# bupt-ai-cz/HIAST

Measured on AMD Instinct MI355X. Metric: self-training images/sec (fwd+bwd+pseudo-label) at 1024x512, higher is better.
Workload: dtype fp16

## Files before the change

### hiast_amd/_lib.py

```python
import ctypes
import os

import torch

_HERE = os.path.dirname(os.path.abspath(__file__))
LIB_PATH = os.environ.get("HIAST_LIB") or os.path.join(_HERE, "csrc", "libhiast_hip.so")

c_int, c_i64, c_f32, c_sz, c_vp = (ctypes.c_int, ctypes.c_int64, ctypes.c_float, ctypes.c_size_t,
                                   ctypes.c_void_p)

SIGNATURES = {
    "hiast_version": (c_int, []),
    "hiast_error_string": (ctypes.c_char_p, [c_int]),
    "hiast_upsample_bilinear_ac_fwd": (c_int, [c_vp, c_vp] + [c_int] * 6 + [c_vp]),
    "hiast_upsample_bilinear_ac_bwd": (c_int, [c_vp, c_vp] + [c_int] * 6 + [c_vp]),
    "hiast_plabel_pass1_workspace_bytes": (c_sz, [c_int]),
    "hiast_plabel_pass1": (c_int, [c_vp] + [c_int] * 6 + [c_vp, c_vp, c_vp, c_vp, c_sz, c_vp]),
    "hiast_plabel_pass2": (c_int, [c_vp, c_vp, c_vp, c_int, c_int, c_i64, c_vp, c_vp, c_vp, c_vp]),
    "hiast_plabel_strided_hist_workspace_bytes": (c_sz, [c_i64, c_int]),
    "hiast_plabel_strided_hist": (c_int, [c_vp, c_vp, c_i64, c_int, c_int, c_vp, c_vp, c_vp, c_vp, c_sz, c_vp]),
    "hiast_tta_fused": (c_int, [c_vp] * 6 + [c_int] * 5 + [c_vp, c_vp, c_vp]),
    "hiast_dinput_fwd": (c_int, [c_vp, c_int, c_vp] + [c_int] * 6 + [c_vp]),
    "hiast_dinput_bwd": (c_int, [c_vp, c_int, c_vp, c_vp, c_vp] + [c_int] * 6 + [c_vp]),
    "hiast_st_loss_workspace_bytes": (c_sz, [c_int] * 6),
    "hiast_st_loss_fwd": (c_int, [c_vp, c_vp, c_vp] + [c_int] * 8 + [c_vp, c_vp, c_sz, c_vp]),
    "hiast_st_loss_bwd": (c_int, [c_vp, c_vp, c_vp] + [c_int] * 8 + [c_vp, c_vp, c_vp, c_vp, c_sz, c_vp]),
    "hiast_st_loss_cst_fwd": (c_int, [c_vp, c_vp, c_vp] + [c_int] * 9 + [c_vp, c_vp, c_sz, c_vp]),
    "hiast_st_loss_cst_bwd": (c_int, [c_vp, c_vp, c_vp] + [c_int] * 9 + [c_vp, c_vp, c_vp, c_vp, c_sz, c_vp]),
    "hiast_aspp_wpack_bytes": (c_sz, [c_int, c_int]),
    "hiast_aspp_workspace_bytes": (c_sz, [c_int] * 5),
    "hiast_aspp_pack_weights": (c_int, [c_vp] * 8 + [c_int, c_int, c_vp, c_vp]),
    "hiast_aspp_fwd": (c_int, [c_vp, c_vp, c_vp] + [c_int] * 5 + [c_vp, c_vp, c_sz, c_vp]),
    "hiast_aspp_bwd_data": (c_int, [c_vp, c_vp, c_vp] + [c_int] * 5 + [c_vp, c_vp]),
    "hiast_aspp_bwd_weight": (c_int, [c_vp] * 7 + [c_int] * 5 + [c_vp, c_vp, c_sz, c_vp]),
    "hiast_aspp2_np": (c_int, [c_int]),
    "hiast_aspp2_workspace_bytes": (c_sz, [c_int] * 6),
    "hiast_aspp2_pack_weights": (c_int, [c_vp] * 8 + [c_int, c_int, c_vp, c_vp, c_vp, c_vp]),
    "hiast_aspp2_fwd": (c_int, [c_vp, c_int, c_vp, c_vp, c_vp] + [c_int] * 5 + [c_vp, c_vp, c_sz, c_vp]),
    "hiast_aspp2_bwd": (c_int, [c_vp] * 9 + [c_int] * 5 + [c_vp, c_int, c_vp, c_sz, c_vp]),
    "hiast_bn_workspace_bytes": (c_sz, [c_int, c_int]),
    "hiast_bn_stats": (c_int, [c_vp, c_int, c_int, c_i64, c_int, c_vp, c_vp]),
    "hiast_bn_act_apply": (c_int, [c_vp] * 8 + [c_int, ctypes.c_double, c_f32, c_f32, c_int, c_vp, c_vp,
                                   c_int, c_int, c_i64, c_int, c_vp]),
    "hiast_bn_act_bwd_stats": (c_int, [c_vp] * 5 + [c_int, c_int, c_int, c_i64, c_int, c_vp, c_vp]),
    "hiast_bn_act_bwd_apply": (c_int, [c_vp] * 7 + [c_int, ctypes.c_double, c_int, c_vp, c_vp, c_vp, c_vp,
                                       c_int, c_int, c_i64, c_int, c_vp]),
    "hiast_bn_act_nhwc_infer": (c_int, [c_vp] * 6 + [c_f32, c_int, c_i64, c_int, c_int, c_vp]),
    "hiast_igemm_bn_act": (c_int, [c_vp] * 6 + [c_f32, c_vp, c_int, c_vp] + [c_int] * 10 + [c_vp, c_int, c_vp, c_int, c_vp]),
    "hiast_igemm_set_cosched": (c_int, [c_int]),
    "hiast_igemm_set_half": (c_int, [c_int]),
    "hiast_device_cus": (c_int, []),
    "hiast_set_reserve_cus": (c_int, [c_int]),
    "hiast_get_reserve_cus": (c_int, []),
    "hiast_stream_create_reserved": (c_int, [c_vp, c_int]),
    "hiast_stream_destroy": (c_int, [c_vp]),
    "hiast_igemm_stats_rows": (c_int, [c_i64, c_int, c_int, c_int, c_int]),
    "hiast_igemm_dgrad_bn_stats": (c_int, [c_vp, c_vp, c_vp] + [c_int] * 7 + [c_vp] * 6 + [c_int, c_int, c_vp]),
    "hiast_xconv_dgrad_gated_bn_stats_rows": (c_int, [c_i64, c_int, c_int]),
    "hiast_xconv_dgrad_gated_bn_stats": (c_int, [c_vp] * 10 + [c_i64, c_int, c_int, c_int, c_vp]),
    "hiast_igemm_dgrad_s2": (c_int, [c_vp, c_vp, c_vp] + [c_int] * 6 + [c_vp]),
    "hiast_igemm_dgrad_bn_stats_rows": (c_int, [c_i64, c_int, c_int, c_int]),
    "hiast_bn_nhwc_stats_from_partial": (c_int, [c_vp, c_int, c_int, c_vp, c_vp]),
    "hiast_conv_wgrad_workspace_bytes": (c_sz, [c_int] * 6),
    "hiast_conv_wgrad_nhwc": (c_int, [c_vp, c_vp, c_vp] + [c_int] * 9 + [c_vp, c_sz, c_vp]),
    "hiast_conv_wgrad_group_workspace_bytes": (c_sz, [c_vp, c_int]),
    "hiast_conv_wgrad_group_nhwc": (c_int, [c_vp, c_int, c_int, c_vp, c_sz, c_vp]),
    "hiast_conv_wgrad_small_workspace_bytes": (c_sz, [c_int] * 6),
    "hiast_conv_wgrad_small_nhwc": (c_int, [c_vp, c_vp, c_vp] + [c_int] * 9 + [c_vp, c_sz, c_vp]),
    "hiast_pack_conv_weight": (c_int, [c_vp, c_int, c_int, c_int, c_int, c_int, c_vp, c_vp, c_vp]),
    "hiast_bn_nhwc_workspace_bytes": (c_sz, [c_int]),
    "hiast_bn_nhwc_stats": (c_int, [c_vp, c_i64, c_int, c_vp, c_vp, c_sz, c_int, c_vp]),
    "hiast_bn_nhwc_apply": (c_int, [c_vp] * 8 + [ctypes.c_double, c_f32, c_f32, c_int, c_vp, c_vp, c_i64, c_int, c_vp,
                                    c_int, c_vp]),
    "hiast_bn_nhwc_apply_partial": (c_int, [c_vp] * 8 + [c_int, ctypes.c_double, c_f32, c_f32, c_int, c_vp, c_vp, c_i64,
                                            c_int, c_vp, c_int, c_vp]),
    "hiast_bn_nhwc_bwd_stats": (c_int, [c_vp] * 7 + [c_int, c_i64, c_int, c_vp, c_vp, c_sz, c_int, c_vp]),
    "hiast_bn_nhwc_bwd_apply": (c_int, [c_vp] * 8 + [ctypes.c_double, c_int, c_vp, c_vp, c_vp, c_vp, c_i64, c_int, c_int,
                                        c_vp]),
    "hiast_pack_conv_weight_multi": (c_int, [c_vp, c_vp, c_vp, c_int, c_int, c_vp]),
    "hiast_split_planes": (c_int, [c_vp, c_vp, c_i64, c_int, c_int, c_vp]),
    "hiast_stem_tail": (c_int, [c_vp, c_int, c_vp, c_vp, c_vp, c_vp, c_f32, c_vp, c_int, c_int, c_int, c_int, c_int, c_vp]),
    "hiast_stem_eval": (c_int, [c_vp] * 6 + [c_f32, c_vp, c_int, c_int, c_int, c_int, c_vp]),
    "hiast_stem_train_blocks": (c_int, [c_int] * 3),
    "hiast_stem_train_fwd": (c_int, [c_vp, c_vp, c_vp, c_vp, c_int, c_int, c_int, c_int, c_vp]),
    "hiast_stem_wgrad_workspace_bytes": (c_sz, [c_int] * 3),
    "hiast_stem_wgrad": (c_int, [c_vp, c_vp, c_vp, c_int, c_int, c_int, c_int, c_vp, c_sz, c_vp]),
    "hiast_ema_update": (c_int, [c_vp, c_vp, c_vp, c_int, c_f32, c_f32, c_vp]),
    "hiast_normalize_u8": (c_int, [c_vp, c_vp, c_int, c_i64, c_vp, c_vp, c_vp]),
    "hiast_maxpool3x3s2_nhwc_fwd": (c_int, [c_vp, c_vp, c_vp, c_int, c_int, c_int, c_int, c_int, c_vp]),
    "hiast_maxpool3x3s2_nhwc_bwd": (c_int, [c_vp, c_vp, c_vp, c_int, c_int, c_int, c_int, c_int, c_vp]),
    "hiast_multi_copy": (c_int, [c_vp, c_int, c_vp]),
    "hiast_aug_geometry_u8": (c_int, [c_vp] * 6 + [c_int] * 4 + [c_vp]),
    "hiast_aug_hist_u8": (c_int, [c_vp] * 5 + [c_int, c_i64, c_vp]),
    "hiast_aug_colour_u8": (c_int, [c_vp] * 5 + [c_int, c_i64, c_vp]),
    "hiast_aug2_table_u8": (c_int, [c_vp] * 6 + [c_int, c_i64, c_vp]),
    "hiast_aug2_colour_u8": (c_int, [c_vp] * 6 + [c_int, c_i64, c_vp]),
    "hiast_aug2_blur_u8": (c_int, [c_vp] * 5 + [c_int] * 3 + [c_vp]),
    "hiast_adam_prepare": (c_int, [c_vp, c_vp, c_vp, c_vp]),
    "hiast_adam_step": (c_int, [c_vp, c_vp, c_vp, c_int, ctypes.c_double, ctypes.c_double, c_f32, c_f32, c_vp, c_vp]),
    "hiast_sgd_step": (c_int, [c_vp, c_vp, c_vp, c_int, c_f32, c_f32, c_vp, c_vp]),
    "hiast_adamw_step": (c_int, [c_vp, c_vp, c_vp, c_int, ctypes.c_double, ctypes.c_double, c_f32, c_vp, c_vp]),
    "hiast_disc_conv_workspace_bytes": (c_sz, [c_int] * 5),
    "hiast_disc_conv_fwd": (c_int, [c_vp] * 4 + [c_int] * 6 + [c_vp]),
    "hiast_disc_conv_dgrad": (c_int, [c_vp] * 4 + [c_int] * 6 + [c_vp, c_sz, c_vp]),
    "hiast_disc_conv_wgrad": (c_int, [c_vp] * 5 + [c_int] * 6 + [c_vp, c_sz, c_vp]),
    "hiast_disc_conv16_fwd": (c_int, [c_vp] * 4 + [c_int] * 7 + [c_vp]),
    "hiast_disc_conv16_dgrad": (c_int, [c_vp] * 4 + [c_int] * 7 + [c_vp, c_sz, c_vp]),
    "hiast_disc_conv16_wgrad": (c_int, [c_vp] * 5 + [c_int] * 7 + [c_vp, c_sz, c_vp]),
    "hiast_confusion_hist": (c_int, [c_vp, c_vp, c_i64, c_int, c_vp, c_vp, c_vp, c_vp]),
}



class WgradJob(ctypes.Structure):
    _fields_ = [("dy", c_vp), ("x", c_vp), ("dw", c_vp)] + [(n, ctypes.c_int32) for n in
                                                             ("B", "H", "W", "Cin", "Cout", "taps", "stride", "dil")]


NBINS = 15361
PROB_FX_SHIFT = 30
IGNORE = 255

_lib = None


class HiastLibraryError(RuntimeError):
    pass


def load():
    global _lib
    if _lib is not None:
        return _lib
    if not os.path.exists(LIB_PATH):
        raise HiastLibraryError(
            "libhiast_hip.so is not built (%s). Build it with `python -c 'import __graft_entry__ as g; "
            "g.build()'` or `make -C hiast_amd/csrc`; there is no fallback path." % LIB_PATH)
    lib = ctypes.CDLL(LIB_PATH)
    for name, (res, args) in SIGNATURES.items():
        try:
            fn = getattr(lib, name)
        except AttributeError as e:
            raise HiastLibraryError("libhiast_hip.so does not export %s" % name) from e
        fn.restype = res
        fn.argtypes = args
    if lib.hiast_version() != 6:
        raise HiastLibraryError("libhiast_hip.so ABI version mismatch")
    _lib = lib
    return lib


def kernel_sources_sha16():
    import glob
    import hashlib
    h = hashlib.sha256()
    files = sorted(glob.glob(os.path.join(_HERE, "csrc", "*.hip")) + glob.glob(os.path.join(_HERE, "csrc", "*.h")))
    files.append(os.path.join(os.path.dirname(_HERE), "include", "hiast_hip.h"))
    for f in files:
        h.update(os.path.basename(f).encode())
        h.update(open(f, "rb").read())
    return h.hexdigest()[:16]


def check(code, what):
    if code != 0:
        msg = load().hiast_error_string(int(code)).decode()
        raise HiastLibraryError("%s failed: %s (code %d)" % (what, msg, code))
```

### hiast_amd/csrc/bn_nhwc.hip

```cpp
#include <hip/hip_bf16.h>

#include "common.h"

namespace hiast {

constexpr int BNH_MAXBLK = 512;
#ifndef BNH_ROWS_PER_BLOCK_PASS
#define BNH_ROWS_PER_BLOCK_PASS 16
#endif
#ifndef BNH_APPLY_MAXBLK
#define BNH_APPLY_MAXBLK 65535
#endif
#ifndef BNH_CONTIG
#define BNH_CONTIG 0
#endif
#if BNH_CONTIG
#define BNH_ROW_WALK(CHUNK)                                                                                              \
    const long long step = (CHUNK);                                                                                      \
    const long long per_blk = ((M + gridDim.x - 1) / gridDim.x + (CHUNK) - 1) / (CHUNK) * (CHUNK);                       \
    const long long lim = (long long)(blockIdx.x + 1) * per_blk < M ? (long long)(blockIdx.x + 1) * per_blk : M;         \
    long long r0 = (long long)blockIdx.x * per_blk + rsub;
#else
#define BNH_ROW_WALK(CHUNK)                                                                                              \
    const long long step = (long long)gridDim.x * (CHUNK);                                                               \
    const long long lim = M;                                                                                             \
    long long r0 = (long long)blockIdx.x * (CHUNK) + rsub;
#endif
#ifndef BNH_UNR_PART
#define BNH_UNR_PART 8
#endif
#ifndef BNH_UNR_APPLY
#define BNH_UNR_APPLY 4
#endif
#ifndef BNH_UNR_BWD
#define BNH_UNR_BWD 4
#endif

template <bool F16>
__device__ __forceinline__ void bnh_unpack8(const uint4 r, float (&v)[8])
{
    const unsigned w[4] = {r.x, r.y, r.z, r.w};
#pragma unroll
    for (int i = 0; i < 4; ++i) {
        v[2 * i] = H16<F16>::lo(w[i]);
        v[2 * i + 1] = H16<F16>::hi(w[i]);
    }
}

#ifndef BNH_NT_LOADS
#define BNH_NT_LOADS 7
#endif
template <int WHICH>
__device__ __forceinline__ uint4 bnh_ld16(const unsigned short* p)
{
    if ((BNH_NT_LOADS >> WHICH) & 1) {
        const h_u32x4 v = __builtin_nontemporal_load(reinterpret_cast<const h_u32x4*>(p));
        return make_uint4(v.x, v.y, v.z, v.w);
    }
    return *reinterpret_cast<const uint4*>(p);
}

template <bool F16>
__device__ __forceinline__ void bnh_load8(const unsigned short* p, float (&v)[8])
{
    bnh_unpack8<F16>(*reinterpret_cast<const uint4*>(p), v);
}

__device__ __forceinline__ void bnh_param8(const float* p, const float* some_valid, int c0, float dflt, float (&v)[8])
{
    const float* q = (p ? p : some_valid) + c0;
    const float4 a = *reinterpret_cast<const float4*>(q), b = *reinterpret_cast<const float4*>(q + 4);
    const bool has = p != nullptr;
    v[0] = has ? a.x : dflt; v[1] = has ? a.y : dflt; v[2] = has ? a.z : dflt; v[3] = has ? a.w : dflt;
    v[4] = has ? b.x : dflt; v[5] = has ? b.y : dflt; v[6] = has ? b.z : dflt; v[7] = has ? b.w : dflt;
}

template <bool F16>
__device__ __forceinline__ void bnh_store8(unsigned short* p, const float (&v)[8], bool nt = false)
{
    unsigned w[4];
#pragma unroll
    for (int i = 0; i < 4; ++i) w[i] = H16<F16>::pack(v[2 * i], v[2 * i + 1]);
    h_store16(p, w[0], w[1], w[2], w[3], nt);
}

template <bool BWD, int GATE, bool F16 = false>
__global__ __launch_bounds__(256) void bnh_partial_kernel(const unsigned short* __restrict__ a,
                                                          const unsigned short* __restrict__ y,
                                                          const unsigned short* __restrict__ x,
                                                          const float* __restrict__ gamma,
                                                          const float* __restrict__ beta,
                                                          const float* __restrict__ save_mean,
                                                          const float* __restrict__ save_invstd, long long M, int C,
                                                          float* __restrict__ partial)
{
    __shared__ float s_red[256 * 16];
    const int G = C >> 3, RPP = 256 / G;
    const int cg = threadIdx.x % G, rsub = threadIdx.x / G;
    float s1[8], s2[8], mean[8], invstd[8], gsc[8], gsh[8];
#pragma unroll
    for (int k = 0; k < 8; ++k) { s1[k] = 0.f; s2[k] = 0.f; mean[k] = 0.f; invstd[k] = 0.f; gsc[k] = 0.f; gsh[k] = 0.f; }
    constexpr int UNR = BNH_UNR_PART;
    const long long stride = RPP;
    BNH_ROW_WALK(RPP * UNR)

    uint4 ra[UNR], ry[UNR], rx[UNR];
    unsigned rbits[UNR];
    auto load_rows = [&](long long rb) {
#pragma unroll
        for (int u = 0; u < UNR; ++u) {
            const long long r = rb + u * stride;
            const long long rc = r < lim ? r : (rb < lim ? rb : 0);
            const size_t off = (size_t)rc * C + cg * 8;
            ra[u] = bnh_ld16<0>(a + off);
            if (BWD) {
                if (GATE == 1) ry[u] = bnh_ld16<0>(y + off);
                rbits[u] = GATE == 3 ? reinterpret_cast<const unsigned char*>(y)[(size_t)rc * G + cg] : 0u;
                rx[u] = bnh_ld16<0>(x + off);
            }
        }
    };
    load_rows(r0);
    if (BWD) {
        float gm[8], bt[8];
        bnh_param8(save_mean, save_mean, cg * 8, 0.f, mean);
        bnh_param8(save_invstd, save_mean, cg * 8, 0.f, invstd);
        if (GATE == 2) {
            bnh_param8(gamma, save_mean, cg * 8, 1.0f, gm);
            bnh_param8(beta, save_mean, cg * 8, 0.0f, bt);
#pragma unroll
            for (int k = 0; k < 8; ++k) {
                gsc[k] = gm[k] * invstd[k];
                gsh[k] = fmaf(-mean[k], gsc[k], bt[k]);
            }
        }
    }
    while (r0 < lim) {
#pragma unroll
        for (int u = 0; u < UNR; ++u) {
            if (r0 + u * stride >= lim) break;
            float v[8];
            bnh_unpack8<F16>(ra[u], v);
            if (!BWD) {
#pragma unroll
                for (int k = 0; k < 8; ++k) { s1[k] += v[k]; s2[k] = fmaf(v[k], v[k], s2[k]); }
            } else {
                float yy[8], xx[8];
                if (GATE == 1) bnh_unpack8<F16>(ry[u], yy);
                const unsigned bits = rbits[u];
                bnh_unpack8<F16>(rx[u], xx);
#pragma unroll
                for (int k = 0; k < 8; ++k) {
                    const bool open = GATE == 0 || (GATE == 1 ? yy[k] > 0.f
                                                    : (GATE == 3 ? ((bits >> k) & 1u) != 0u : fmaf(xx[k], gsc[k], gsh[k]) > 0.f));
                    const float g = open ? v[k] : 0.f;
                    s1[k] += g;
                    s2[k] = fmaf(g, (xx[k] - mean[k]) * invstd[k], s2[k]);
                }
            }
        }
        r0 += step;
        if (r0 < lim) load_rows(r0);
    }
#pragma unroll
    for (int k = 0; k < 8; ++k) {
        s_red[threadIdx.x * 16 + k] = s1[k];
        s_red[threadIdx.x * 16 + 8 + k] = s2[k];
    }
    __syncthreads();
    if (rsub == 0) {
        float* dst = partial + ((size_t)blockIdx.x * C + cg * 8) * 2;
#pragma unroll
        for (int k = 0; k < 8; ++k) {
            float t1 = 0.f, t2 = 0.f;
            for (int j = 0; j < RPP; ++j) {
                t1 += s_red[(j * G + cg) * 16 + k];
                t2 += s_red[(j * G + cg) * 16 + 8 + k];
            }
            dst[2 * k] = t1;
            dst[2 * k + 1] = t2;
        }
    }
}

__global__ __launch_bounds__(256) void bnh_finalize_kernel(const float* __restrict__ partial, int nblk, int C,
                                                           double* __restrict__ sums)
{
    __shared__ double s[16][17];
    const int e = threadIdx.x & 15, j = threadIdx.x >> 4;
    const int i = blockIdx.x * 16 + e;
    double acc = 0.0;
    {
        int b = j;
        for (; b + 16 * 15 < nblk; b += 16 * 16) {
            float v[16];
#pragma unroll
            for (int u = 0; u < 16; ++u) v[u] = partial[(size_t)(b + 16 * u) * C * 2 + i];
#pragma unroll
            for (int u = 0; u < 16; ++u) acc += (double)v[u];
        }
        for (; b < nblk; b += 16) acc += (double)partial[(size_t)b * C * 2 + i];
    }
    s[j][e] = acc;
    __syncthreads();
    if (j == 0) {
        double t = 0.0;
#pragma unroll
        for (int q = 0; q < 16; ++q) t += s[q][e];
        sums[i] = t;
    }
}

__global__ __launch_bounds__(256) void bnh_prep_fwd_kernel(const double* __restrict__ sums, double count, float momentum,
                                                           float eps, float* __restrict__ run_mean,
                                                           float* __restrict__ run_var, float* __restrict__ save_mean,
                                                           float* __restrict__ save_invstd, int C)
{
    const int c = blockIdx.x * 256 + threadIdx.x;
    if (c >= C) return;
    const double m = sums[2 * c] / count;
    double var = sums[2 * c + 1] / count - m * m;
    var = var < 0.0 ? 0.0 : var;
    const float mean = (float)m;
    const float invstd = (float)(1.0 / sqrt(var + (double)eps));
    save_mean[c] = mean;
    save_invstd[c] = invstd;
    if (run_mean) {
        const double unb = count > 1.0 ? var * count / (count - 1.0) : var;
        run_mean[c] = (1.0f - momentum) * run_mean[c] + momentum * mean;
        run_var[c] = (1.0f - momentum) * run_var[c] + momentum * (float)unb;
    }
}

__global__ __launch_bounds__(256) void bnh_finalize_prep_kernel(const float* __restrict__ partial, int nblk, int C,
                                                                double count, float momentum, float eps,
                                                                float* __restrict__ run_mean, float* __restrict__ run_var,
                                                                float* __restrict__ save_mean,
                                                                float* __restrict__ save_invstd)
{
    __shared__ double s[64][5];
    const int e = threadIdx.x & 3, j = threadIdx.x >> 2;
    const int i = blockIdx.x * 4 + e;
    const int c = blockIdx.x * 2 + (int)threadIdx.x;
    float rm = 0.f, rv = 0.f;
    if (threadIdx.x < 2 && run_mean) { rm = run_mean[c]; rv = run_var[c]; }
    double acc = 0.0;
    {
        int b = j;
        for (; b + 64 * 3 < nblk; b += 64 * 4) {
            float v[4];
#pragma unroll
            for (int u = 0; u < 4; ++u) v[u] = partial[(size_t)(b + 64 * u) * C * 2 + i];
#pragma unroll
            for (int u = 0; u < 4; ++u) acc += (double)v[u];
        }
        for (; b < nblk; b += 64) acc += (double)partial[(size_t)b * C * 2 + i];
    }
    s[j][e] = acc;
    __syncthreads();
    if (threadIdx.x < 2) {
        double s1 = 0.0, s2 = 0.0;
#pragma unroll 8
        for (int q = 0; q < 64; ++q) { s1 += s[q][2 * threadIdx.x]; s2 += s[q][2 * threadIdx.x + 1]; }
        const double m = s1 / count;
        double var = s2 / count - m * m;
        var = var < 0.0 ? 0.0 : var;
        const float mean = (float)m;
        save_mean[c] = mean;
        save_invstd[c] = (float)(1.0 / sqrt(var + (double)eps));
        if (run_mean) {
            const double unb = count > 1.0 ? var * count / (count - 1.0) : var;
            run_mean[c] = (1.0f - momentum) * rm + momentum * mean;
            run_var[c] = (1.0f - momentum) * rv + momentum * (float)unb;
        }
    }
}

template <bool RES, bool RELU, bool F16 = false>
__global__ __launch_bounds__(256) void bnh_apply_kernel(const unsigned short* __restrict__ x,
                                                        const unsigned short* __restrict__ res,
                                                        unsigned short* __restrict__ y, const float* __restrict__ gamma,
                                                        const float* __restrict__ beta,
                                                        const float* __restrict__ save_mean,
                                                        const float* __restrict__ save_invstd, long long M, int C,
                                                        unsigned char* __restrict__ mask)
{
    const int G = C >> 3, RPP = 256 / G;
    const bool nt_out = (long long)M * C * 2 >= H_NT_MIN_BYTES;
    const int cg = threadIdx.x % G, rsub = threadIdx.x / G;
    constexpr int UNR = BNH_UNR_APPLY;
    const long long stride = RPP;
    BNH_ROW_WALK(RPP * UNR)

    uint4 rx[UNR], rres[UNR];
    auto load_rows = [&](long long rb) {
#pragma unroll
        for (int u = 0; u < UNR; ++u) {
            const long long r = rb + u * stride;
            const size_t off = (size_t)(r < lim ? r : (rb < lim ? rb : 0)) * C + cg * 8;
            rx[u] = bnh_ld16<1>(x + off);
            if (RES) rres[u] = bnh_ld16<1>(res + off);
        }
    };
    load_rows(r0);
    float scale[8], shift[8];
    {
        float gm[8], bt[8], mn[8], is[8];
        bnh_param8(gamma, save_mean, cg * 8, 1.0f, gm);
        bnh_param8(beta, save_mean, cg * 8, 0.0f, bt);
        bnh_param8(save_mean, save_mean, cg * 8, 0.f, mn);
        bnh_param8(save_invstd, save_mean, cg * 8, 0.f, is);
#pragma unroll
        for (int k = 0; k < 8; ++k) {
            scale[k] = gm[k] * is[k];
            shift[k] = fmaf(-mn[k], scale[k], bt[k]);
        }
    }
    while (r0 < lim) {
#pragma unroll
        for (int u = 0; u < UNR; ++u) {
            const long long r = r0 + u * stride;
            if (r >= lim) break;
            const size_t off = (size_t)r * C + cg * 8;
            float v[8], rr[8];
            bnh_unpack8<F16>(rx[u], v);
            if (RES) bnh_unpack8<F16>(rres[u], rr);
            unsigned bits = 0;
#pragma unroll
            for (int k = 0; k < 8; ++k) {
                float o = fmaf(v[k], scale[k], shift[k]);
                if (RES) o += rr[k];
                if (RELU) o = o > 0.f ? o : 0.f;
                bits |= (o > 0.f ? 1u : 0u) << k;
                v[k] = o;
            }
            bnh_store8<F16>(y + off, v, nt_out);
            if (mask) mask[(size_t)r * G + cg] = (unsigned char)bits;
        }
        r0 += step;
        if (r0 < lim) load_rows(r0);
    }
}

template <int GATE, bool DRES, bool F16 = false>
__global__ __launch_bounds__(256) void bnh_bwd_apply_kernel(
    const unsigned short* __restrict__ dy, const unsigned short* __restrict__ y, const unsigned short* __restrict__ x,
    const float* __restrict__ gamma, const float* __restrict__ beta, const float* __restrict__ save_mean,
    const float* __restrict__ save_invstd,
    const double* __restrict__ sums, double inv_count, unsigned short* __restrict__ dx,
    unsigned short* __restrict__ dres, float* __restrict__ dgamma, float* __restrict__ dbeta, long long M, int C)
{
    const int G = C >> 3, RPP = 256 / G;
    const bool nt_out = (long long)M * C * 2 >= H_NT_MIN_BYTES;
    const int cg = threadIdx.x % G, rsub = threadIdx.x / G;
    constexpr int UNR = BNH_UNR_BWD;
    const long long stride = RPP;
    BNH_ROW_WALK(RPP * UNR)

    uint4 rg[UNR], ry[UNR], rx[UNR];
    unsigned rbits[UNR];
    auto load_rows = [&](long long rb) {
#pragma unroll
        for (int u = 0; u < UNR; ++u) {
            const long long r = rb + u * stride;
            const long long rc = r < lim ? r : (rb < lim ? rb : 0);
            const size_t off = (size_t)rc * C + cg * 8;
            rg[u] = bnh_ld16<2>(dy + off);
            if (GATE == 1) ry[u] = bnh_ld16<2>(y + off);
            rbits[u] = GATE == 3 ? reinterpret_cast<const unsigned char*>(y)[(size_t)rc * G + cg] : 0u;
            rx[u] = bnh_ld16<2>(x + off);
        }
    };
    load_rows(r0);
    float mean[8], invstd[8], k0[8], mg[8], mgx[8], gsh[8];
    {
        float gm[8], bt[8];
        bnh_param8(save_mean, save_mean, cg * 8, 0.f, mean);
        bnh_param8(save_invstd, save_mean, cg * 8, 0.f, invstd);
        bnh_param8(gamma, save_mean, cg * 8, 1.0f, gm);
        bnh_param8(beta, save_mean, cg * 8, 0.0f, bt);
        const double2* sp = reinterpret_cast<const double2*>(sums) + cg * 8;
#pragma unroll
        for (int k = 0; k < 8; ++k) {
            const double2 ss = sp[k];
            if (blockIdx.x == 0 && rsub == 0) {
                if (dbeta) dbeta[cg * 8 + k] = (float)ss.x;
                if (dgamma) dgamma[cg * 8 + k] = (float)ss.y;
            }
            k0[k] = gm[k] * invstd[k];
            gsh[k] = GATE == 2 ? fmaf(-mean[k], k0[k], bt[k]) : 0.f;
            mg[k] = (float)(ss.x * inv_count);
            mgx[k] = (float)(ss.y * inv_count);
        }
    }
    while (r0 < lim) {
#pragma unroll
        for (int u = 0; u < UNR; ++u) {
            const long long r = r0 + u * stride;
            if (r >= lim) break;
            const size_t off = (size_t)r * C + cg * 8;
            float g[8], yy[8], xx[8];
            bnh_unpack8<F16>(rg[u], g);
            if (GATE == 1) bnh_unpack8<F16>(ry[u], yy);
            const unsigned bits = rbits[u];
            bnh_unpack8<F16>(rx[u], xx);
#pragma unroll
            for (int k = 0; k < 8; ++k) {
                const bool open = GATE == 0 || (GATE == 1 ? yy[k] > 0.f
                                                : (GATE == 3 ? ((bits >> k) & 1u) != 0u : fmaf(xx[k], k0[k], gsh[k]) > 0.f));
                const float gg = open ? g[k] : 0.f;
                g[k] = gg;
                xx[k] = k0[k] * (gg - mg[k] - (xx[k] - mean[k]) * invstd[k] * mgx[k]);
            }
            bnh_store8<F16>(dx + off, xx, nt_out);
            if (DRES) bnh_store8<F16>(dres + off, g, nt_out);
        }
        r0 += step;
        if (r0 < lim) load_rows(r0);
    }
}

static int bnh_nblk(long long M, int C)
{
    const int rpp = 256 / (C / 8);
    long long nb = (M + (long long)rpp * 16 - 1) / ((long long)rpp * 16);
    nb = nb < 1 ? 1 : (nb > BNH_MAXBLK ? BNH_MAXBLK : nb);
    return (int)nb;
}

}

static bool bnh_c_ok(int C) { return C >= 8 && C <= 2048 && (C & (C - 1)) == 0; }

static int bnh_check(const void* x, long long M, int C)
{
    if (!x) return HIAST_E_ARG;
    if (M <= 0) return HIAST_E_ARG;
    if (!bnh_c_ok(C) || (((uintptr_t)x) & 15)) return HIAST_E_RANGE;
    return 0;
}

extern "C" size_t hiast_bn_nhwc_workspace_bytes(int C) { return (size_t)hiast::BNH_MAXBLK * C * 2 * sizeof(float); }

#define BNH_FMT_CHECK()                                                             \
    if (fmt != HIAST_FMT_BF16 && fmt != HIAST_FMT_FP16) return HIAST_E_RANGE;          \
    const bool f16 = fmt == HIAST_FMT_FP16

extern "C" int hiast_bn_nhwc_stats(const void* x, int64_t M, int C, double* sums, void* workspace,
                                   size_t workspace_bytes, int fmt, hiast_stream_t stream)
{
    BNH_FMT_CHECK();
    int e = bnh_check(x, M, C);
    if (e) return e;
    if (!sums || !workspace) return HIAST_E_ARG;
    const int nblk = hiast::bnh_nblk(M, C);
    if (workspace_bytes < (size_t)nblk * C * 2 * sizeof(float)) return HIAST_E_WS;
    hipStream_t st = (hipStream_t)stream;
    if (f16)
        hipLaunchKernelGGL((hiast::bnh_partial_kernel<false, 0, true>), dim3(nblk), dim3(256), 0, st, (const unsigned short*)x,
                           nullptr, nullptr, nullptr, nullptr, nullptr, nullptr, (long long)M, C, (float*)workspace);
    else
        hipLaunchKernelGGL((hiast::bnh_partial_kernel<false, 0>), dim3(nblk), dim3(256), 0, st, (const unsigned short*)x,
                           nullptr, nullptr, nullptr, nullptr, nullptr, nullptr, (long long)M, C, (float*)workspace);
    HIAST_CHECK_LAUNCH();
    hipLaunchKernelGGL(hiast::bnh_finalize_kernel, dim3(C * 2 / 16), dim3(256), 0, st, (const float*)workspace, nblk, C,
                       sums);
    HIAST_CHECK_LAUNCH();
    return 0;
}

extern "C" int hiast_bn_nhwc_stats_from_partial(const float* partial, int nblk, int C, double* sums,
                                                hiast_stream_t stream)
{
    if (!partial || !sums) return HIAST_E_ARG;
    if (nblk <= 0) return HIAST_E_ARG;
    if (!bnh_c_ok(C)) return HIAST_E_RANGE;
    hipLaunchKernelGGL(hiast::bnh_finalize_kernel, dim3(C * 2 / 16), dim3(256), 0, (hipStream_t)stream, partial, nblk, C,
                       sums);
    HIAST_CHECK_LAUNCH();
    return 0;
}

extern "C" int hiast_bn_nhwc_apply(const void* x, const void* res, void* y, const float* gamma, const float* beta,
                                   float* running_mean, float* running_var, const double* sums, double count,
                                   float momentum, float eps, int relu, float* save_mean, float* save_invstd,
                                   int64_t M, int C, void* mask, int fmt, hiast_stream_t stream)
{
    BNH_FMT_CHECK();
    int e = bnh_check(x, M, C);
    if (e) return e;
    if (!y || !sums || !save_mean || !save_invstd || count <= 0) return HIAST_E_ARG;
    if ((((uintptr_t)y) | ((uintptr_t)res)) & 15) return HIAST_E_RANGE;
    const int rpp = 256 / (C / 8);
    long long nb = (M + (long long)rpp * BNH_ROWS_PER_BLOCK_PASS - 1) / ((long long)rpp * BNH_ROWS_PER_BLOCK_PASS);
    nb = nb < 1 ? 1 : (nb > BNH_APPLY_MAXBLK ? BNH_APPLY_MAXBLK : nb);
    hipStream_t st = (hipStream_t)stream;
    hipLaunchKernelGGL(hiast::bnh_prep_fwd_kernel, dim3((C + 255) / 256), dim3(256), 0, st, sums, count, momentum, eps,
                       running_mean, running_var, save_mean, save_invstd, C);
    HIAST_CHECK_LAUNCH();
#define L1(RES, RELU, F)                                                                                           \
    hipLaunchKernelGGL((hiast::bnh_apply_kernel<RES, RELU, F>), dim3((unsigned)nb), dim3(256), 0, st,              \
                       (const unsigned short*)x, (const unsigned short*)res, (unsigned short*)y, gamma, beta,      \
                       save_mean, save_invstd, (long long)M, C, (unsigned char*)mask)
#define L(RES, RELU) do { if (f16) L1(RES, RELU, true); else L1(RES, RELU, false); } while (0)
    if (res) { if (relu) L(true, true); else L(true, false); }
    else { if (relu) L(false, true); else L(false, false); }
#undef L
#undef L1
    HIAST_CHECK_LAUNCH();
    return 0;
}

extern "C" int hiast_bn_nhwc_apply_partial(const void* x, const void* res, void* y, const float* gamma, const float* beta,
                                           float* running_mean, float* running_var, const float* partial, int nblk,
                                           double count, float momentum, float eps, int relu, float* save_mean,
                                           float* save_invstd, int64_t M, int C, void* mask, int fmt,
                                           hiast_stream_t stream)
{
    BNH_FMT_CHECK();
    int e = bnh_check(x, M, C);
    if (e) return e;
    if (!y || !partial || !save_mean || !save_invstd || count <= 0 || nblk <= 0) return HIAST_E_ARG;
    if ((((uintptr_t)y) | ((uintptr_t)res)) & 15) return HIAST_E_RANGE;
    const int rpp = 256 / (C / 8);
    long long nb = (M + (long long)rpp * BNH_ROWS_PER_BLOCK_PASS - 1) / ((long long)rpp * BNH_ROWS_PER_BLOCK_PASS);
    nb = nb < 1 ? 1 : (nb > BNH_APPLY_MAXBLK ? BNH_APPLY_MAXBLK : nb);
    hipStream_t st = (hipStream_t)stream;
    hipLaunchKernelGGL(hiast::bnh_finalize_prep_kernel, dim3(C / 2), dim3(256), 0, st, partial, nblk, C, count,
                       momentum, eps, running_mean, running_var, save_mean, save_invstd);
    HIAST_CHECK_LAUNCH();
#define L1(RES, RELU, F)                                                                                           \
    hipLaunchKernelGGL((hiast::bnh_apply_kernel<RES, RELU, F>), dim3((unsigned)nb), dim3(256), 0, st,              \
                       (const unsigned short*)x, (const unsigned short*)res, (unsigned short*)y, gamma, beta,      \
                       save_mean, save_invstd, (long long)M, C, (unsigned char*)mask)
#define L(RES, RELU) do { if (f16) L1(RES, RELU, true); else L1(RES, RELU, false); } while (0)
    if (res) { if (relu) L(true, true); else L(true, false); }
    else { if (relu) L(false, true); else L(false, false); }
#undef L
#undef L1
    HIAST_CHECK_LAUNCH();
    return 0;
}

extern "C" int hiast_bn_nhwc_bwd_stats(const void* dy, const void* y, const void* x, const float* gamma,
                                       const float* beta, const float* save_mean, const float* save_invstd, int relu,
                                       int64_t M, int C, double* sums, void* workspace, size_t workspace_bytes, int fmt,
                                       hiast_stream_t stream)
{
    BNH_FMT_CHECK();
    int e = bnh_check(x, M, C);
    if (e) return e;
    if (!dy || !save_mean || !save_invstd || !sums || !workspace || ((relu == 1 || relu == 3) && !y)) return HIAST_E_ARG;
    if (relu < 0 || relu > 3 || (((uintptr_t)dy) & 15) || (relu == 1 && (((uintptr_t)y) & 15))) return HIAST_E_RANGE;
    const int nblk = hiast::bnh_nblk(M, C);
    if (workspace_bytes < (size_t)nblk * C * 2 * sizeof(float)) return HIAST_E_WS;
    hipStream_t st = (hipStream_t)stream;
#define L1(G, F)                                                                                                    \
    hipLaunchKernelGGL((hiast::bnh_partial_kernel<true, G, F>), dim3(nblk), dim3(256), 0, st, (const unsigned short*)dy, \
                       (const unsigned short*)y, (const unsigned short*)x, gamma, beta, save_mean, save_invstd,      \
                       (long long)M, C, (float*)workspace)
#define L(G) do { if (f16) L1(G, true); else L1(G, false); } while (0)
    if (relu == 1) L(1); else if (relu == 2) L(2); else if (relu == 3) L(3); else L(0);
#undef L
#undef L1
    HIAST_CHECK_LAUNCH();
    hipLaunchKernelGGL(hiast::bnh_finalize_kernel, dim3(C * 2 / 16), dim3(256), 0, st, (const float*)workspace, nblk, C,
                       sums);
    HIAST_CHECK_LAUNCH();
    return 0;
}

extern "C" int hiast_bn_nhwc_bwd_apply(const void* dy, const void* y, const void* x, const float* gamma,
                                       const float* beta, const float* save_mean, const float* save_invstd,
                                       const double* sums,
                                       double count, int relu, void* dx, void* dres, float* dgamma, float* dbeta,
                                       int64_t M, int C, int fmt, hiast_stream_t stream)
{
    BNH_FMT_CHECK();
    int e = bnh_check(x, M, C);
    if (e) return e;
    if (!dy || !save_mean || !save_invstd || !sums || !dx || ((relu == 1 || relu == 3) && !y) || count <= 0)
        return HIAST_E_ARG;
    if (relu < 0 || relu > 3 || ((((uintptr_t)dy) | ((uintptr_t)dx) | ((uintptr_t)dres)) & 15) ||
        (relu == 1 && (((uintptr_t)y) & 15)))
        return HIAST_E_RANGE;
    const int rpp = 256 / (C / 8);
    long long nb = (M + (long long)rpp * BNH_ROWS_PER_BLOCK_PASS - 1) / ((long long)rpp * BNH_ROWS_PER_BLOCK_PASS);
    nb = nb < 1 ? 1 : (nb > BNH_APPLY_MAXBLK ? BNH_APPLY_MAXBLK : nb);
    hipStream_t st = (hipStream_t)stream;
#define L1(G, DRES, F)                                                                                             \
    hipLaunchKernelGGL((hiast::bnh_bwd_apply_kernel<G, DRES, F>), dim3((unsigned)nb), dim3(256), 0, st,             \
                       (const unsigned short*)dy, (const unsigned short*)y, (const unsigned short*)x, gamma, beta,  \
                       save_mean, save_invstd, sums, 1.0 / count, (unsigned short*)dx, (unsigned short*)dres, dgamma, \
                       dbeta, (long long)M, C)
#define L(G, DRES) do { if (f16) L1(G, DRES, true); else L1(G, DRES, false); } while (0)
    if (relu == 1) { if (dres) L(1, true); else L(1, false); }
    else if (relu == 3) { if (dres) L(3, true); else L(3, false); }
    else if (relu == 2) { if (dres) L(2, true); else L(2, false); }
    else { if (dres) L(0, true); else L(0, false); }
#undef L
#undef L1
    HIAST_CHECK_LAUNCH();
    return 0;
}
```

### hiast_amd/csrc/common.h

```cpp
#pragma once
#include <hip/hip_runtime.h>
#include <hip/hip_bf16.h>
#include <hip/hip_fp16.h>
#include <stdint.h>

#include <type_traits>

#include "../../include/hiast_hip.h"

#define HIAST_WAVE 64

#define HIAST_CHECK_LAUNCH()                         \
    do {                                             \
        hipError_t e__ = hipGetLastError();          \
        if (e__ != hipSuccess) return (int)e__;      \
    } while (0)

static inline int hiast_fmt_planes(int fmt) { return fmt == HIAST_FMT_SPLIT_BF16 ? 2 : 1; }
static inline int hiast_fmt_ok(int fmt) { return fmt == HIAST_FMT_BF16 || fmt == HIAST_FMT_SPLIT_BF16 || fmt == HIAST_FMT_FP16; }

int hiast_cu_count();
int hiast_grid_cus();

namespace hiast {

template <class F>
static inline bool for_class_count(int C, F&& f)
{
    switch (C) {
        case 19: f(std::integral_constant<int, 19>{}); return true;
        case 16: f(std::integral_constant<int, 16>{}); return true;
        case 9:  f(std::integral_constant<int, 9>{});  return true;
        case 2:  f(std::integral_constant<int, 2>{});  return true;
        default: return false;
    }
}

typedef __attribute__((ext_vector_type(8))) __bf16 h_bf16x8;
typedef __attribute__((ext_vector_type(8))) _Float16 h_f16x8;
typedef __attribute__((ext_vector_type(4))) float h_f32x4;
typedef __attribute__((ext_vector_type(16))) float h_f32x16;

typedef __attribute__((address_space(3))) void* h_lds_ptr;
__device__ __forceinline__ void h_dma16(__amdgpu_buffer_rsrc_t rs, unsigned char* lds, int voff, int soff)
{
    __builtin_amdgcn_raw_ptr_buffer_load_lds(rs, (h_lds_ptr)lds, 16, voff, soff, 0, 0);
}
__device__ __forceinline__ int h_lds_off(int row, int chunk) { return row * 128 + ((chunk ^ ((row >> 1) & 7)) << 4); }

#ifndef HIAST_NT
#define HIAST_NT 1
#endif
__device__ __forceinline__ void h_store_f32(float* p, float v)
{
#if HIAST_NT
    __builtin_nontemporal_store(v, p);
#else
    *p = v;
#endif
}
typedef unsigned int h_u32x4 __attribute__((ext_vector_type(4)));
__device__ __forceinline__ void h_store16(void* p, unsigned a, unsigned b, unsigned c, unsigned d)
{
#if HIAST_NT
    __builtin_nontemporal_store((h_u32x4){a, b, c, d}, reinterpret_cast<h_u32x4*>(p));
#else
    *reinterpret_cast<uint4*>(p) = make_uint4(a, b, c, d);
#endif
}
__device__ __forceinline__ void h_store16(void* p, unsigned a, unsigned b, unsigned c, unsigned d, bool nt)
{
#if HIAST_NT
    if (nt) {
        __builtin_nontemporal_store((h_u32x4){a, b, c, d}, reinterpret_cast<h_u32x4*>(p));
        return;
    }
#endif
    *reinterpret_cast<uint4*>(p) = make_uint4(a, b, c, d);
}
#ifndef H_NT_MIN_MIB
#define H_NT_MIN_MIB 64
#endif
constexpr long long H_NT_MIN_BYTES = (long long)H_NT_MIN_MIB << 20;
#ifndef HIAST_NT_OUT
#define HIAST_NT_OUT 0
#endif
__device__ __forceinline__ void h_store16_out(void* p, unsigned a, unsigned b, unsigned c, unsigned d)
{
    h_store16(p, a, b, c, d, HIAST_NT_OUT != 0);
}
__device__ __forceinline__ void h_store_f32_out(float* p, float v)
{
#if HIAST_NT_OUT
    __builtin_nontemporal_store(v, p);
#else
    *p = v;
#endif
}
#ifndef HIAST_NT_RES
#define HIAST_NT_RES 0
#endif
__device__ __forceinline__ uint4 h_load16_once(const void* p)
{
#if HIAST_NT_RES
    const h_u32x4 v = __builtin_nontemporal_load(reinterpret_cast<const h_u32x4*>(p));
    return make_uint4(v.x, v.y, v.z, v.w);
#else
    return *reinterpret_cast<const uint4*>(p);
#endif
}

template <bool F16>
struct H16;

template <>
struct H16<false> {
    static __device__ __forceinline__ float lo(unsigned w) { return __uint_as_float(w << 16); }
    static __device__ __forceinline__ float hi(unsigned w) { return __uint_as_float(w & 0xFFFF0000u); }
    static __device__ __forceinline__ float dec(unsigned short h) { return __uint_as_float((unsigned)h << 16); }
    static __device__ __forceinline__ unsigned short enc(float v) { return __bfloat16_as_ushort(__float2bfloat16(v)); }
    static __device__ __forceinline__ unsigned pack(float a, float b) { return (unsigned)enc(a) | ((unsigned)enc(b) << 16); }
    template <class V>
    static __device__ __forceinline__ h_f32x4 mfma16(const V& a, const V& b, h_f32x4 c)
    {
        return __builtin_amdgcn_mfma_f32_16x16x32_bf16(__builtin_bit_cast(h_bf16x8, a), __builtin_bit_cast(h_bf16x8, b), c, 0, 0, 0);
    }
    template <class V>
    static __device__ __forceinline__ h_f32x16 mfma32(const V& a, const V& b, h_f32x16 c)
    {
        return __builtin_amdgcn_mfma_f32_32x32x16_bf16(__builtin_bit_cast(h_bf16x8, a), __builtin_bit_cast(h_bf16x8, b), c, 0, 0, 0);
    }
};

template <>
struct H16<true> {
    static __device__ __forceinline__ float dec(unsigned short h) { return __half2float(__ushort_as_half(h)); }
    static __device__ __forceinline__ float lo(unsigned w) { return dec((unsigned short)(w & 0xFFFFu)); }
    static __device__ __forceinline__ float hi(unsigned w) { return dec((unsigned short)(w >> 16)); }
    static __device__ __forceinline__ unsigned short enc(float v) { return __half_as_ushort(__float2half_rn(v)); }
    static __device__ __forceinline__ unsigned pack(float a, float b) { return (unsigned)enc(a) | ((unsigned)enc(b) << 16); }
    template <class V>
    static __device__ __forceinline__ h_f32x4 mfma16(const V& a, const V& b, h_f32x4 c)
    {
        return __builtin_amdgcn_mfma_f32_16x16x32_f16(__builtin_bit_cast(h_f16x8, a), __builtin_bit_cast(h_f16x8, b), c, 0, 0, 0);
    }
    template <class V>
    static __device__ __forceinline__ h_f32x16 mfma32(const V& a, const V& b, h_f32x16 c)
    {
        return __builtin_amdgcn_mfma_f32_32x32x16_f16(__builtin_bit_cast(h_f16x8, a), __builtin_bit_cast(h_f16x8, b), c, 0, 0, 0);
    }
};

__device__ __forceinline__ float a_expf(float x)
{
    const float LOG2E = 1.44269502162933349609375f;
    const float LN2_HI = 0.693145751953125f;
    const float LN2_LO = 1.428606765330187045037746429443359375e-06f;
    float n = rintf(x * LOG2E);
    float r = fmaf(-n, LN2_HI, x);
    r = fmaf(-n, LN2_LO, r);
    float p = 1.984127011382952332496643066406250e-04f;
    p = fmaf(p, r, 1.388888922519981861114501953125e-03f);
    p = fmaf(p, r, 8.33333376795053482055664062500e-03f);
    p = fmaf(p, r, 4.16666679084300994873046875000e-02f);
    p = fmaf(p, r, 1.66666671633720397949218750000e-01f);
    p = fmaf(p, r, 0.5f);
    p = fmaf(p, r, 1.0f);
    p = fmaf(p, r, 1.0f);
    float s = __int_as_float(((int)n + 127) << 23);
    float v = p * s;
    return x < -87.0f ? 0.0f : v;
}

struct Src {
    int i0, i1;
    float l0, l1;
};

__device__ __forceinline__ Src src_of(float scale, int dst, int in)
{
    Src s;
    float f = scale * (float)dst;
    int a = (int)f;
    a = a > in - 1 ? in - 1 : a;
    s.i0 = a;
    s.i1 = a + (a < in - 1 ? 1 : 0);
    s.l1 = f - (float)a;
    s.l0 = 1.0f - s.l1;
    return s;
}

__device__ __forceinline__ float lerp_h(float a, float b, float wl0, float wl1)
{
    return fmaf(wl1, b, wl0 * a);
}

__device__ __forceinline__ float lerp_v(float top, float bot, float hl0, float hl1)
{
    return fmaf(hl1, bot, hl0 * top);
}

__device__ __forceinline__ int band_start(float scale, int j, int in, int out)
{
    if (j <= 0) return 0;
    if (j > in - 1) return out;
    if (scale <= 0.0f) return out;
    int Y = (int)((float)j / scale);
    Y = Y < 0 ? 0 : (Y > out ? out : Y);
    while (Y > 0 && (int)(scale * (float)(Y - 1)) >= j) --Y;
    while (Y < out && (int)(scale * (float)Y) < j) ++Y;
    return Y;
}

__device__ __forceinline__ int lane_id() { return (int)(threadIdx.x & 63); }

__device__ __forceinline__ unsigned long long wave_sum_u64(unsigned long long v)
{
#pragma unroll
    for (int o = 32; o > 0; o >>= 1) v += __shfl_xor(v, o, 64);
    return v;
}

__device__ __forceinline__ double wave_sum_f64(double v)
{
#pragma unroll
    for (int o = 32; o > 0; o >>= 1) v += __shfl_xor(v, o, 64);
    return v;
}

}
```

### hiast_amd/functional.py

```python
import os

import torch

from . import kernels as K
from . import switches as SW

ASPP_DILATIONS = (6, 12, 18, 24)
H16 = (torch.bfloat16, torch.float16)


class _AsppFn(torch.autograd.Function):

    @staticmethod
    @torch.amp.custom_fwd(device_type="cuda", cast_inputs=torch.float32)
    def forward(ctx, x, w0, w1, w2, w3, b0, b1, b2, b3, dil):
        x = x.contiguous()
        ws = [w.contiguous() for w in (w0, w1, w2, w3)]
        bs = [b.contiguous() for b in (b0, b1, b2, b3)]
        wpack = K.aspp_pack_weights(ws, bs)
        Cout = ws[0].shape[0]
        y = K.aspp_fwd(x, wpack, Cout, dil)
        ctx.save_for_backward(x, wpack)
        ctx.dil = dil
        ctx.cin = x.shape[1]
        return y

    @staticmethod
    @torch.amp.custom_bwd(device_type="cuda")
    def backward(ctx, gy):
        x, wpack = ctx.saved_tensors
        gy = gy.contiguous().float()
        gx = None
        if ctx.needs_input_grad[0]:
            gx = K.aspp_bwd_data(gy, wpack, ctx.cin, ctx.dil)
        gws, gb = [None] * 4, None
        if any(ctx.needs_input_grad[1:9]):
            gws, gb = K.aspp_bwd_weight(x, gy, ctx.dil)
        return (gx, gws[0], gws[1], gws[2], gws[3], gb, gb, gb, gb, None)


def aspp(x, weights, biases, dil=ASPP_DILATIONS):
    return _AsppFn.apply(x, *weights, *biases, tuple(dil))


class _Aspp2Fn(torch.autograd.Function):

    @staticmethod
    @torch.amp.custom_fwd(device_type="cuda")
    def forward(ctx, x, w0, w1, w2, w3, b0, b1, b2, b3, dil, need_bwd):
        ws = [w.detach().float().contiguous() for w in (w0, w1, w2, w3)]
        bs = [b.detach().float().contiguous() for b in (b0, b1, b2, b3)]
        if need_bwd and x.dtype not in H16:
            raise TypeError("the channels-last ASPP backward is the 16-bit one; fp32 training uses hiast_amd.functional.aspp")
        wt, wd, bias = K.aspp2_pack_weights(ws, bs, need_dgrad=need_bwd and ctx.needs_input_grad[0])
        y = K.aspp2_fwd(x, wt, bias, dil)
        ctx.save_for_backward(x, wd)
        ctx.dil = dil
        return y

    @staticmethod
    @torch.amp.custom_bwd(device_type="cuda")
    def backward(ctx, gy):
        x, wd = ctx.saved_tensors
        gy = gy.contiguous().float()
        want_dx = ctx.needs_input_grad[0]
        want_dw = any(ctx.needs_input_grad[1:9])
        gx, gws, gb = K.aspp2_bwd(x, gy, wd, ctx.dil, want_dx, want_dw)
        if gws is None:
            gws = [None] * 4
        return (gx, gws[0], gws[1], gws[2], gws[3], gb, gb, gb, gb, None, None)


def aspp_nhwc(x, weights, biases, dil=ASPP_DILATIONS):
    need_bwd = torch.is_grad_enabled() and any(t.requires_grad for t in (x, *weights, *biases))
    return _Aspp2Fn.apply(x, *weights, *biases, tuple(dil), need_bwd)


class _UpsampleFn(torch.autograd.Function):

    @staticmethod
    @torch.amp.custom_fwd(device_type="cuda", cast_inputs=torch.float32)
    def forward(ctx, x, H, W):
        ctx.hw = x.shape[2:]
        return K.upsample_bilinear_ac_fwd(x.contiguous(), H, W)

    @staticmethod
    @torch.amp.custom_bwd(device_type="cuda")
    def backward(ctx, g):
        return K.upsample_bilinear_ac_bwd(g.contiguous().float(), ctx.hw[0], ctx.hw[1]), None, None


def upsample_bilinear_ac(x, size):
    return _UpsampleFn.apply(x, int(size[0]), int(size[1]))


class _StLossFn(torch.autograd.Function):

    @staticmethod
    @torch.amp.custom_fwd(device_type="cuda", cast_inputs=torch.float32)
    def forward(ctx, logits_lr, teacher_lr, plbl, H, W, region, w_t, w_k, w_e, w_c, cst_kind="SoftCE"):
        logits_lr = logits_lr.contiguous()
        if teacher_lr is not None:
            teacher_lr = teacher_lr.contiguous()
        plbl = plbl.contiguous()
        B, C, h, w = logits_lr.shape
        ws = K.st_loss_workspace(B, C, h, w, H, W, logits_lr.device)
        cst_kind = K.CST_KINDS[cst_kind] if teacher_lr is not None else 0
        sums = K.st_loss_fwd(logits_lr, teacher_lr, plbl, H, W, region, ws, cst_kind=cst_kind)
        ctx.save_for_backward(logits_lr, teacher_lr, plbl, sums)
        ctx.ws = ws
        ctx.args = (H, W, region, w_t, w_k, w_e, w_c, cst_kind)
        s = sums.float()
        ce = w_t * s[0] / s[4]
        kld = w_k * s[1] / (C * s[4])
        ent = w_e * s[2] / (C * s[5])
        cst = w_c * s[3] / s[6]
        ctx.mark_non_differentiable(sums)
        return ce, kld, ent, cst, sums

    @staticmethod
    @torch.amp.custom_bwd(device_type="cuda")
    def backward(ctx, g_ce, g_kld, g_ent, g_cst, _g_sums):
        logits_lr, teacher_lr, plbl, sums = ctx.saved_tensors
        H, W, region, w_t, w_k, w_e, w_c, cst_kind = ctx.args
        coef = torch.stack([g_ce * w_t, g_kld * w_k, g_ent * w_e, g_cst * w_c]).float().contiguous()
        d = K.st_loss_bwd(logits_lr, teacher_lr, plbl, H, W, region, sums, coef, ctx.ws, cst_kind=cst_kind)
        return (d,) + (None,) * 10


def st_loss(logits_lr, teacher_lr, plbl, size, region="ignored", w_t=1.0, w_k=0.1, w_e=1.0, w_c=0.5, cst_kind="SoftCE"):
    if cst_kind not in K.CST_KINDS:
        raise ValueError("cst_kind %r: one of %s" % (cst_kind, ", ".join(K.CST_KINDS)))
    ce, kld, ent, cst, _ = _StLossFn.apply(logits_lr, teacher_lr, plbl, int(size[0]), int(size[1]), region,
                                            float(w_t), float(w_k), float(w_e), float(w_c), cst_kind)
    return ce, kld, ent, cst


class _DInputFn(torch.autograd.Function):

    @staticmethod
    @torch.amp.custom_fwd(device_type="cuda", cast_inputs=torch.float32)
    def forward(ctx, logits_lr, H, W, entropy):
        logits_lr = logits_lr.contiguous()
        ctx.save_for_backward(logits_lr)
        ctx.entropy = entropy
        return K.dinput_fwd(logits_lr, H, W, entropy)

    @staticmethod
    @torch.amp.custom_bwd(device_type="cuda")
    def backward(ctx, g):
        (logits_lr,) = ctx.saved_tensors
        return K.dinput_bwd(logits_lr, g.float().contiguous(), ctx.entropy), None, None, None


def discriminator_input(logits_lr, size, entropy=False):
    return _DInputFn.apply(logits_lr, int(size[0]), int(size[1]), bool(entropy))


class _DiscConvFn(torch.autograd.Function):

    @staticmethod
    @torch.amp.custom_fwd(device_type="cuda", cast_inputs=torch.float32)
    def forward(ctx, x, weight, bias, leaky, fmt=None):
        x, weight = x.contiguous(), weight.contiguous()
        bias = bias.contiguous() if bias is not None else None
        y = K.disc_conv_fwd(x, weight, bias, leaky) if fmt is None else K.disc_conv16_fwd(x, weight, bias, leaky, fmt)
        ctx.save_for_backward(x, weight, y)
        ctx.leaky, ctx.has_bias, ctx.fmt = leaky, bias is not None, fmt
        return y

    @staticmethod
    @torch.amp.custom_bwd(device_type="cuda")
    def backward(ctx, dy):
        x, weight, y = ctx.saved_tensors
        dy = dy.float().contiguous()
        need_x, need_w, need_b = ctx.needs_input_grad[:3]
        fmt = ctx.fmt
        dx = None
        if need_x:
            dx = (K.disc_conv_dgrad(dy, y, weight, x.shape, ctx.leaky) if fmt is None
                  else K.disc_conv16_dgrad(dy, y, weight, x.shape, ctx.leaky, fmt))
        dw = db = None
        if need_w or (need_b and ctx.has_bias):
            want_bias = need_b and ctx.has_bias
            dw, db = (K.disc_conv_wgrad(x, dy, y, ctx.leaky, want_bias=want_bias) if fmt is None
                      else K.disc_conv16_wgrad(x, dy, y, ctx.leaky, fmt, want_bias=want_bias))
        return dx, (dw if need_w else None), (db if need_b else None), None, None


def disc_conv_shapes_ok(x_shape, w_shape):
    x_shape, w_shape = tuple(x_shape), tuple(w_shape)
    if len(x_shape) != 4 or len(w_shape) != 4 or w_shape[2:] != (4, 4) or w_shape[1] != x_shape[1]:
        return False
    B, Cin, H, W = x_shape
    Cout = w_shape[0]
    if B < 1 or not 1 <= Cin <= 4096 or not 1 <= Cout <= 4096 or H < 2 or W < 2 or max(B, H, W) >= 2 ** 31:
        return False
    return K.disc_conv_workspace_bytes(B, Cin, Cout, H, W) > 0


def disc_conv_ok(x, weight):
    return (isinstance(x, torch.Tensor) and isinstance(weight, torch.Tensor) and x.is_cuda and weight.is_cuda
            and x.dtype == torch.float32 and weight.dtype == torch.float32
            and disc_conv_shapes_ok(x.shape, weight.shape))


def disc_conv4x4s2(x, weight, bias, leaky, fmt=None):
    if fmt is None:
        return _DiscConvFn.apply(x, weight, bias, bool(leaky))
    if fmt not in (torch.float16, torch.bfloat16):
        raise TypeError("fmt must be None, torch.float16 or torch.bfloat16, got %r" % (fmt,))
    return _DiscConvFn.apply(x, weight, bias, bool(leaky), fmt)


def _sync_world(bn):
    import torch.distributed as dist
    if isinstance(bn, torch.nn.SyncBatchNorm) and dist.is_available() and dist.is_initialized():
        from hiast_amd.utils import comm
        w = dist.get_world_size()
        return 0 if (w == 1 and comm.rehearsal()) else w
    return 1


_BN3_FUSION = os.environ.get("HIAST_NO_BN3_FUSION", "0") != "1"
_OWN_S2_DGRAD = os.environ.get("HIAST_LIB_DGRAD_S2", "0") != "1"

_NO_ASYNC_STAT = os.environ.get("HIAST_NO_ASYNC_STAT", "0") == "1"


def _stat_all_reduce(t, async_op=False):
    from hiast_amd.utils import comm
    return comm.all_reduce(t, "stat", async_op=async_op)


def _stat_wait(work):
    from hiast_amd.utils import comm
    comm.wait(work, "stat")


class _BnActFn(torch.autograd.Function):

    @staticmethod
    def forward(ctx, x, res, gamma, beta, running_mean, running_var, training, momentum, eps, relu, world):
        x = x.contiguous()
        if res is not None:
            res = res.contiguous()
        ctx.training = training
        if not training:
            y, _, _ = K.bn_act_apply(x, res, gamma, beta, running_mean, running_var, None, 0.0, momentum, eps, relu)
            return y
        part = K.bn_stats(x)
        count = float(x.shape[0] * x.shape[2] * x.shape[3])
        if world != 1:
            _stat_all_reduce(part)
            count *= max(world, 1)
        y, sm, si = K.bn_act_apply(x, res, gamma, beta, running_mean, running_var, part, count, momentum, eps, relu)
        ctx.save_for_backward(x, y, gamma, sm, si)
        ctx.relu, ctx.has_res, ctx.world, ctx.count = relu, res is not None, world, count
        return y

    @staticmethod
    def backward(ctx, dy):
        if not ctx.training:
            raise NotImplementedError("backward through inference-mode fused BN is not needed by the hot path")
        x, y, gamma, sm, si = ctx.saved_tensors
        dy = dy.contiguous()
        if dy.dtype != x.dtype:
            dy = dy.to(x.dtype)
        part = K.bn_act_bwd_stats(dy, y, x, sm, si, ctx.relu)
        if ctx.world != 1:
            _stat_all_reduce(part)
        want_p = gamma is not None and (ctx.needs_input_grad[2] or ctx.needs_input_grad[3])
        dx, dres, dg, db = K.bn_act_bwd_apply(dy, y, x, gamma, sm, si, part, ctx.count, ctx.relu,
                                              ctx.has_res and ctx.needs_input_grad[1], want_p)
        return (dx, dres, dg if ctx.needs_input_grad[2] else None, db if ctx.needs_input_grad[3] else None,
                None, None, None, None, None, None, None)


def _is_cl(t):
    return t.dim() == 4 and t.permute(0, 2, 3, 1).is_contiguous()


class _BnActNhwcFn(torch.autograd.Function):

    @staticmethod
    def forward(ctx, x, res, gamma, beta, running_mean, running_var, momentum, eps, relu, world, partial, box,
                stat_box=None):
        count = float(x.shape[0] * x.shape[2] * x.shape[3])
        ctx.gate = 0 if not relu else (3 if res is not None else 2)
        if ctx.gate == 3 and SW.on("HIAST_NO_BN_MASK"):
            ctx.gate = 1
        want_mask = ctx.gate == 3
        if world == 1 and partial is not None:
            out = K.bn_nhwc_apply_partial(x, res, gamma, beta, running_mean, running_var, partial, count, momentum, eps,
                                          relu, want_mask)
        else:
            sums = K.bn_nhwc_stats_from_partial(partial) if partial is not None else K.bn_nhwc_stats(x)
            if world != 1:
                _stat_all_reduce(sums)
                count *= max(world, 1)
            out = K.bn_nhwc_apply(x, res, gamma, beta, running_mean, running_var, sums, count, momentum, eps, relu,
                                  want_mask)
        y, sm, si = out[:3]
        ctx.save_for_backward(x, out[3] if want_mask else (y if ctx.gate == 1 else None), gamma, beta, sm, si)
        ctx.has_res, ctx.world, ctx.count = res is not None, world, count
        ctx.box = box if (box is not None and box.get("armed") and ctx.gate in (1, 3)) else None
        ctx.stat_box = None
        if stat_box is not None:
            left = stat_box.pop("bwd_sums", None)
            if left is not None:
                _stat_wait(left[1])
            stat_box.pop("bwd_partial", None)
        if stat_box is not None and ctx.gate == 2:
            stat_box["bn"] = (x.detach(), sm, si, gamma, beta)
            stat_box["world"] = world
            ctx.stat_box = stat_box
        elif stat_box is not None and ctx.gate == 3:
            stat_box["bn3"] = (x.detach(), out[3], sm, si)
            stat_box["world"] = world
            ctx.stat_box = stat_box
        return y

    @staticmethod
    def backward(ctx, dy):
        x, y, gamma, beta, sm, si = ctx.saved_tensors
        if dy.dtype != x.dtype:
            dy = dy.to(x.dtype)
        dy = dy.contiguous(memory_format=torch.channels_last)
        fused = ctx.stat_box.pop("bwd_partial", None) if ctx.stat_box is not None else None
        early = ctx.stat_box.pop("bwd_sums", None) if ctx.stat_box is not None else None
        if early is not None:
            sums, work = early
            _stat_wait(work)
        else:
            if fused is not None:
                sums = K.bn_nhwc_stats_from_partial(fused)
            else:
                sums = K.bn_nhwc_bwd_stats(dy, y, x, gamma, beta, sm, si, ctx.gate)
            if ctx.world != 1:
                _stat_all_reduce(sums)
        want_p = gamma is not None and (ctx.needs_input_grad[2] or ctx.needs_input_grad[3])
        handoff = ctx.box is not None and ctx.needs_input_grad[1]
        dx, dres, dg, db = K.bn_nhwc_bwd_apply(dy, y, x, gamma, beta, sm, si, sums, ctx.count, ctx.gate,
                                               ctx.has_res and ctx.needs_input_grad[1] and not handoff, want_p)
        if handoff:
            ctx.box["gated"] = (dy, y)
        return (dx, dres, dg if ctx.needs_input_grad[2] else None, db if ctx.needs_input_grad[3] else None,
                None, None, None, None, None, None, None, None, None)


class _ConvNhwcFn(torch.autograd.Function):

    @staticmethod
    @torch.amp.custom_fwd(device_type="cuda")
    def forward(ctx, x, weight, stride, dil, want_stats, box, packed, in_bn=None, wgroup=None, xsum=None, in_bn3=None):
        xv = x.permute(0, 2, 3, 1)
        ctx.in_bn3 = None
        if (in_bn3 is not None and "bn3" in in_bn3 and box is not None and stride == 1 and weight.shape[2] == 1
                and ctx.needs_input_grad[0] and _BN3_FUSION
                and K.xconv_dgrad_gated_bn_stats_ok(x.shape[0] * x.shape[2] * x.shape[3], weight.shape[0], weight.shape[1])):
            ctx.in_bn3 = in_bn3
        ctx.wgroup = wgroup
        ctx.xsum = xsum if (xsum is not None and stride == 1 and ctx.needs_input_grad[0]) else None
        if ctx.xsum is not None:
            if ctx.xsum[1] == "take":
                ctx.xsum[0]["taker"] = True
            elif not ctx.xsum[0].get("taker"):
                ctx.xsum = None
        ctx.in_bn = in_bn if (in_bn is not None and "bn" in in_bn and stride == 1 and ctx.needs_input_grad[0]
                              and not SW.on("HIAST_NO_BN_BWD_FUSION")) else None
        ctx.set_materialize_grads(False)
        ctx.wpt = None
        ctx.box = None
        if box is not None and stride == 1 and ctx.needs_input_grad[0]:
            box["armed"] = True
            ctx.box = box
        need_adj = ctx.needs_input_grad[0] and (stride == 1 or (stride == 2 and weight.shape[2] == 3 and dil == 1 and _OWN_S2_DGRAD))
        if packed is not None and packed[0] is not None and (not need_adj or packed[1] is not None):
            wp, ctx.wpt = packed
        elif need_adj:
            wp, ctx.wpt = K.pack_conv_weight(weight, K.fmt_of(x), both=True)
        else:
            wp = K.pack_conv_weight(weight, K.fmt_of(x))
        ctx.save_for_backward(x, weight)
        ctx.geo = (stride, dil)
        if want_stats:
            y, partial = K.igemm_bn_act(xv, wp, 1, None, None, False, stride, dil, want_stats=True)
            ctx.mark_non_differentiable(partial)
            return y.permute(0, 3, 1, 2), partial
        return K.igemm_bn_act(xv, wp, 1, None, None, False, stride, dil).permute(0, 3, 1, 2)

    @staticmethod
    @torch.amp.custom_bwd(device_type="cuda")
    def backward(ctx, dy, _dpartial=None):
        if dy is None:
            return None, None, None, None, None, None, None, None, None, None, None
        x, weight = ctx.saved_tensors
        stride, dil = ctx.geo
        if dy.dtype != x.dtype:
            dy = dy.to(x.dtype)
        dy = dy.contiguous(memory_format=torch.channels_last)
        k = weight.shape[2]
        pad = dil if k == 3 else 0
        need_x, need_w = ctx.needs_input_grad[0], ctx.needs_input_grad[1]
        dx = dw = None
        own_s2 = need_x and stride == 2 and k == 3 and dil == 1 and _OWN_S2_DGRAD
        lib_x = need_x and stride != 1 and not own_s2
        if own_s2:
            wpt = ctx.wpt if ctx.wpt is not None else K.pack_conv_weight(weight, K.fmt_of(x), transpose=True)
            dx = K.igemm_dgrad_s2(dy.permute(0, 2, 3, 1), wpt, x.shape[2], x.shape[3]).permute(0, 3, 1, 2)
        if need_x and stride == 1:
            wpt = ctx.wpt if ctx.wpt is not None else K.pack_conv_weight(weight, K.fmt_of(x), transpose=True)
            gated = ctx.box.pop("gated", None) if ctx.box is not None else None
            if ctx.in_bn is not None and gated is None:
                bx, sm, si, gamma, beta = ctx.in_bn["bn"]
                dxv, bpartial = K.igemm_dgrad_bn_stats(dy.permute(0, 2, 3, 1), wpt, dil, bx.permute(0, 2, 3, 1), gamma, beta,
                                                       sm, si)
                if ctx.in_bn.get("world", 1) != 1 and not _NO_ASYNC_STAT:
                    bsums = K.bn_nhwc_stats_from_partial(bpartial)
                    ctx.in_bn["bwd_sums"] = (bsums, _stat_all_reduce(bsums, async_op=True))
                else:
                    ctx.in_bn["bwd_partial"] = bpartial
                dx = dxv.permute(0, 3, 1, 2)
            elif gated is not None and ctx.in_bn3 is not None and gated[1].dtype == torch.uint8:
                bx3, bmask, sm3, si3 = ctx.in_bn3["bn3"]
                dxv, bpartial = K.xconv_dgrad_gated_bn_stats(dy.permute(0, 2, 3, 1), wpt, gated[0].permute(0, 2, 3, 1), gated[1],
                                                             bx3.permute(0, 2, 3, 1), bmask, sm3, si3)
                if ctx.in_bn3.get("world", 1) != 1 and not _NO_ASYNC_STAT:
                    bsums = K.bn_nhwc_stats_from_partial(bpartial)
                    ctx.in_bn3["bwd_sums"] = (bsums, _stat_all_reduce(bsums, async_op=True))
                else:
                    ctx.in_bn3["bwd_partial"] = bpartial
                dx = dxv.permute(0, 3, 1, 2)
            elif gated is not None:
                dx = K.igemm_bn_act(dy.permute(0, 2, 3, 1), wpt, 1, None, gated[0].permute(0, 2, 3, 1), False, 1, dil,
                                    res_gate=(gated[1] if gated[1].dtype == torch.uint8
                                              else gated[1].permute(0, 2, 3, 1))).permute(0, 3, 1, 2)
            else:
                other = None
                if ctx.xsum is not None and ctx.xsum[1] == "take":
                    other = ctx.xsum[0].pop("dx", None)
                    ctx.xsum[0]["taken"] = True
                dx = K.igemm_bn_act(dy.permute(0, 2, 3, 1), wpt, 1, None, None if other is None else other.permute(0, 2, 3, 1),
                                    False, 1, dil).permute(0, 3, 1, 2)
        if ctx.xsum is not None and ctx.xsum[1] == "give" and dx is not None and not ctx.xsum[0].get("taken"):
            ctx.xsum[0]["dx"] = dx
            dx = None
        own_w = need_w and not SW.on("HIAST_LIB_WGRAD") and K.conv_wgrad_preferred(
            weight.shape[1], weight.shape[0], k, stride) and (k == 1 or dy.shape[3] >= 4)
        small_w = need_w and not own_w and not SW.on("HIAST_LIB_WGRAD") and K.conv_wgrad_small_supported(
            weight.shape[1], weight.shape[0], k, stride)
        if need_w and own_w and ctx.wgroup is not None:
            grp, slot = ctx.wgroup
            grp["jobs"][slot] = (dy.permute(0, 2, 3, 1), x.permute(0, 2, 3, 1), k, stride, dil)
            return dx, _wgrad_token(weight), None, None, None, None, None, None, None, None, None
        side = wgrad_side_stream(x.device) if (need_w and not lib_x) else None
        main = torch.cuda.current_stream()
        if side is not None:
            side.wait_stream(main)
            dy.record_stream(side)
            x.record_stream(side)
        with torch.cuda.stream(side if side is not None else main):
            if own_w:
                dw = K.conv_wgrad_nhwc(dy.permute(0, 2, 3, 1), x.permute(0, 2, 3, 1), k, stride, dil)
                need_w = False
            elif small_w:
                dw = K.conv_wgrad_small_nhwc(dy.permute(0, 2, 3, 1), x.permute(0, 2, 3, 1), k, stride, dil)
                need_w = False
            if need_w or lib_x:
                wl = torch.empty(weight.shape, dtype=x.dtype, device=weight.device)
                if lib_x:
                    wl = weight.to(x.dtype)
                gx, gw, _ = torch.ops.aten.convolution_backward(dy, x, wl, None, (stride, stride), (pad, pad), (dil, dil),
                                                                False, (0, 0), 1, (lib_x, need_w, False))
                if lib_x:
                    dx = gx
                if need_w:
                    dw = gw.to(dtype=weight.dtype, memory_format=torch.contiguous_format)
                    if dw.stride() != weight.stride() and dw.is_contiguous() and weight.is_contiguous():
                        dw = dw.view(-1).view(weight.shape)
        if side is not None and dw is not None:
            dw.record_stream(main)
        return dx, dw, None, None, None, None, None, None, None, None, None


_wgrad_tokens = {}


def _wgrad_token(weight):
    key = (weight.device, weight.dtype)
    z = _wgrad_tokens.get(key)
    if z is None:
        z = _wgrad_tokens[key] = torch.zeros((), dtype=weight.dtype, device=weight.device)
    return z.expand(weight.shape)


class _WGroupFn(torch.autograd.Function):

    @staticmethod
    def forward(ctx, grp, *ws):
        ctx.grp = grp
        ctx.set_materialize_grads(False)
        return tuple(w.view_as(w) for w in ws)

    @staticmethod
    def backward(ctx, *tokens):
        grp = ctx.grp
        jobs = grp["jobs"]
        live = [i for i, j in enumerate(jobs) if j is not None and tokens[i] is not None]
        out = [tokens[i] if jobs[i] is None else None for i in range(len(jobs))]
        if live:
            dev = jobs[live[0]][1].device
            side = wgrad_side_stream(dev)
            main = torch.cuda.current_stream()
            if side is not None:
                side.wait_stream(main)
                for i in live:
                    jobs[i][0].record_stream(side)
                    jobs[i][1].record_stream(side)
            with torch.cuda.stream(side if side is not None else main):
                dws = K.conv_wgrad_group([jobs[i] for i in live]) if len(live) > 1 else [K.conv_wgrad_nhwc(*jobs[live[0]])]
            for i, dw in zip(live, dws):
                if side is not None:
                    dw.record_stream(main)
                out[i] = dw
        for i in range(len(jobs)):
            jobs[i] = None
        return (None, *out)


def wgroup_weights(convs, x):
    if (len(convs) < 2 or len(convs) > 4 or SW.on("HIAST_NO_WGROUP")
            or SW.on("HIAST_LIB_WGRAD") or not torch.is_grad_enabled()):
        return None, None
    for c in convs:
        k = c.kernel_size[0]
        if (not c.weight.requires_grad or not conv_nhwc_ok(x, c) or c.stride[0] != 1
                or not K.conv_wgrad_preferred(c.in_channels, c.out_channels, k, 1)):
            return None, None
    tiles = [(c.in_channels // 256) * (c.out_channels // 256) * c.kernel_size[0] ** 2 for c in convs]

    cus = K.grid_cus()

    def fill(idx):
        t = sum(tiles[i] for i in idx)
        return t * (cus // t) / float(cus) if 0 < t <= cus else 0.0
    member = list(range(len(convs)))
    if fill(member) < 0.9:
        member = [i for i in member if convs[i].kernel_size[0] == 1]
        if len(member) < 2 or fill(member) < 0.9:
            return None, None
    grp = {"jobs": [None] * len(member)}
    views = _WGroupFn.apply(grp, *[convs[i].weight for i in member])
    wv = [None] * len(convs)
    slot = [None] * len(convs)
    for s_, i in enumerate(member):
        wv[i], slot[i] = views[s_], s_
    grp["slot"] = slot
    return grp, wv


class _StemConvFn(torch.autograd.Function):

    @staticmethod
    @torch.amp.custom_fwd(device_type="cuda")
    def forward(ctx, x, weight, fmt):
        x = x.contiguous()
        y, partial = K.stem_train_fwd(x, weight.detach(), fmt)
        ctx.save_for_backward(x)
        ctx.set_materialize_grads(False)
        ctx.mark_non_differentiable(partial)
        return y.permute(0, 3, 1, 2), partial

    @staticmethod
    @torch.amp.custom_bwd(device_type="cuda")
    def backward(ctx, dy, _dpartial=None):
        if dy is None or not ctx.needs_input_grad[1]:
            return None, None, None
        x, = ctx.saved_tensors
        dyv = dy.permute(0, 2, 3, 1)
        if not dyv.is_contiguous():
            dyv = dyv.contiguous()
        side = wgrad_side_stream(x.device)
        main = torch.cuda.current_stream()
        if side is not None:
            side.wait_stream(main)
            dyv.record_stream(side)
            x.record_stream(side)
        with torch.cuda.stream(side if side is not None else main):
            dw = K.stem_wgrad(x, dyv)
        if side is not None:
            dw.record_stream(main)
        return None, dw, None


def stem_conv_train(x, conv):
    dt = torch.get_autocast_dtype("cuda")
    return _StemConvFn.apply(x.float() if x.dtype != torch.float32 else x, conv.weight,
                             K.FMT_FP16 if dt == torch.float16 else K.FMT_BF16)


_wgrad_streams = {}
_wgrad_overlap = [False]
_eval_streams = {}


def new_stream(device):
    n = K.reserve_cus() if torch.device(device).type == "cuda" else 0
    return K.reserved_stream(n, device) if n > 0 else torch.cuda.Stream(device=device)
_eval_trunks = {}


def prepack_eval_trunks(model, x):
    trunks = _eval_trunks.get(id(model))
    if trunks is None or trunks[0]() is not model:
        import weakref
        trunks = _eval_trunks[id(model)] = (weakref.ref(model), [m for m in model.modules()
                                                                 if hasattr(m, "prepack") and hasattr(m, "fast_eval_planes")])
    used = []
    for m in trunks[1]:
        PL = m.fast_eval_planes(x)
        if PL:
            m.prepack(PL)
            ent = m.__dict__.get("_hiast_plans", {}).get((PL, False))
            if ent is not None:
                used.append(ent[0])
    return used


def eval_forward_split(model, x, parts=None):
    B = x.shape[0]
    if parts is None:
        parts = int(os.environ.get("HIAST_EVAL_SPLIT", "2" if B >= 8 else "1"))
    if parts <= 1 or B % parts != 0 or not x.is_cuda:
        return model(x, lowres=True)
    main = torch.cuda.current_stream()
    prepack_eval_trunks(model, x)
    key = (x.device, parts)
    side = _eval_streams.get(key)
    if side is None:
        side = _eval_streams[key] = [new_stream(x.device) for _ in range(parts - 1)]
    sub = B // parts
    outs = [None] * parts
    with K.cosched():
        for i, st in enumerate(side):
            st.wait_stream(main)
            with torch.cuda.stream(st):
                outs[i + 1] = model(x[(i + 1) * sub:(i + 2) * sub], lowres=True)
        outs[0] = model(x[:sub], lowres=True)
    for i, st in enumerate(side):
        main.wait_stream(st)
        outs[i + 1]["logits_lowres"].record_stream(main)
    out = dict(outs[0])
    out["logits_lowres"] = torch.cat([o["logits_lowres"] for o in outs], 0)
    return out


class GraphedEval:
    WARMUP = 2
    AUTO_MAX_BATCH = int(os.environ.get("HIAST_GRAPH_EVAL_MAX_BATCH", "0"))

    def __init__(self, model, amp_dtype=None, parts=None, graph=False, auto=True):
        self.model, self.amp_dtype, self.parts = model, amp_dtype, parts
        self.entries = {}
        env = os.environ.get("HIAST_GRAPH_EVAL", "1" if graph else "")
        self.enabled = (None if auto else False) if env == "" else env == "1"

    def wants_graph(self, x):
        return self.enabled if self.enabled is not None else x.shape[0] <= self.AUTO_MAX_BATCH

    def _autocast(self):
        return torch.autocast("cuda", dtype=self.amp_dtype or torch.bfloat16, enabled=self.amp_dtype is not None,
                              cache_enabled=False)

    def _eager(self, x, parts):
        with torch.no_grad(), self._autocast():
            return eval_forward_split(self.model, x, parts)["logits_lowres"].float()

    def _fingerprint(self):
        ps = self.model.__dict__.get("_hiast_fp_params")
        if ps is None:
            allp = list(self.model.parameters()) + list(self.model.buffers())
            ps = self.model.__dict__["_hiast_fp_params"] = [allp[0], allp[len(allp) // 2], allp[-1]]
        return tuple(p.data_ptr() for p in ps)

    def __call__(self, x, parts="ctor", eager=False):
        parts = self.parts if isinstance(parts, str) else parts
        if (eager or not x.is_cuda or self.model.training or not self.wants_graph(x)
                or torch.cuda.is_current_stream_capturing()):
            return self._eager(x, parts)
        key = (tuple(x.shape), x.dtype, x.device, self.amp_dtype, parts)
        e = self.entries.get(key)
        if e is None:
            e = self.entries[key] = {"calls": 0, "graph": None}
        if e["graph"] is not None:
            with torch.no_grad(), self._autocast():
                plans = prepack_eval_trunks(self.model, x)
            if self._fingerprint() == e["fp"] and len(plans) == len(e["plans"]) and all(a is b for a, b in zip(plans, e["plans"])):
                e["x"].copy_(x)
                e["graph"].replay()
                return e["y"]
            e["graph"], e["calls"] = None, 0
        e["calls"] += 1
        if e["calls"] <= self.WARMUP or e.get("failed"):
            return self._eager(x, parts)
        try:
            with torch.no_grad(), self._autocast():
                plans = prepack_eval_trunks(self.model, x)
            xs = torch.empty_like(x)
            xs.copy_(x)
            g = torch.cuda.CUDAGraph()
            cur = torch.cuda.current_stream()
            cap = torch.cuda.Stream(device=x.device)
            cap.wait_stream(cur)
            with torch.cuda.graph(g, stream=cap, capture_error_mode="thread_local"):
                y = self._eager(xs, parts)
            cur.wait_stream(cap)
        except Exception as err:
            import warnings
            warnings.warn("hiast_amd: graph capture of the inference forward failed (%s: %s); running it eagerly"
                          % (type(err).__name__, err))
            e["failed"] = True
            return self._eager(x, parts)
        e.update(graph=g, x=xs, y=y, plans=plans, fp=self._fingerprint())
        g.replay()
        return y


def enable_wgrad_overlap(on=True):
    _wgrad_overlap[0] = bool(on)


def wgrad_side_stream(device):
    if not _wgrad_overlap[0] or os.environ.get("HIAST_NO_WGRAD_STREAM", "0") == "1":
        return None
    from hiast_amd.utils import comm
    if comm.multi():
        return None
    st = _wgrad_streams.get(device)
    if st is None:
        st = new_stream(device)
        _wgrad_streams[device] = st
    return st


def wgrad_stream_join():
    for st in _wgrad_streams.values():
        torch.cuda.current_stream(st.device).wait_stream(st)


def conv_nhwc_ok(x, conv):
    if not (x.is_cuda and x.dtype in H16 and _is_cl(x)) or conv.bias is not None or conv.groups != 1:
        return False
    k = conv.kernel_size
    if k not in ((1, 1), (3, 3)) or conv.stride[0] != conv.stride[1] or conv.in_channels % 64 or conv.out_channels % 64:
        return False
    if k == (1, 1):
        return conv.stride[0] in (1, 2) and conv.padding == (0, 0)
    return conv.padding == conv.dilation and conv.dilation[0] == conv.dilation[1] and conv.stride[0] in (1, 2)


class _MaxPool3x3s2ClFn(torch.autograd.Function):

    @staticmethod
    def forward(ctx, x):
        y, idx = K.maxpool3x3s2_cl_fwd(x)
        ctx.save_for_backward(idx)
        ctx.hw, ctx.dtype = tuple(x.shape[2:]), x.dtype
        ctx.mark_non_differentiable(idx)
        return y

    @staticmethod
    def backward(ctx, dy):
        idx, = ctx.saved_tensors
        if dy.dtype != ctx.dtype:
            dy = dy.to(ctx.dtype)
        return K.maxpool3x3s2_cl_bwd(dy.contiguous(memory_format=torch.channels_last), idx, *ctx.hw)


def maxpool(x, pool):
    if (x.is_cuda and x.dtype in H16 and _is_cl(x) and x.shape[1] % 8 == 0
            and (pool.kernel_size, pool.stride, pool.padding, pool.dilation, pool.ceil_mode) == (3, 2, 1, 1, False)
            and not pool.return_indices and os.environ.get("HIAST_LIB_MAXPOOL", "0") != "1"):
        return _MaxPool3x3s2ClFn.apply(x)
    return pool(x)


class _SubsampleClFn(torch.autograd.Function):

    @staticmethod
    def forward(ctx, x, s):
        ctx.s, ctx.shape = s, x.shape
        return x[:, :, ::s, ::s].contiguous(memory_format=torch.channels_last)

    @staticmethod
    def backward(ctx, dy):
        g = torch.empty(ctx.shape, dtype=dy.dtype, device=dy.device, memory_format=torch.channels_last).zero_()
        g[:, :, ::ctx.s, ::ctx.s] = dy
        return g, None


def conv_nhwc(x, conv, want_stats=False, box=None, in_bn=None, wgroup=None, xsum=None, in_bn3=None):
    w = conv.weight
    wv = w if wgroup is None else wgroup[2]
    fmt = K.fmt_of(x)
    fwd = conv.__dict__.get("_hiast_packed", {}).get(fmt)
    adj = conv.__dict__.get("_hiast_packed_adj", {}).get(fmt)
    ok = lambda e: e is not None and e[0] == w._version and e[1] == w.data_ptr()
    packed = (fwd[2] if ok(fwd) else None, adj[2] if ok(adj) else None)
    stride = conv.stride[0]
    if conv.kernel_size == (1, 1) and stride != 1:
        x = _SubsampleClFn.apply(x, stride)
        stride = 1
    return _ConvNhwcFn.apply(x, wv, stride, conv.dilation[0], bool(want_stats), box, packed, in_bn,
                             None if wgroup is None else (wgroup[0], wgroup[1]), xsum, in_bn3)


_nbt_batched = [False]


def bn_act(x, bn, res=None, relu=True, partial=None, box=None, stat_box=None):
    training = bn.training or (bn.running_mean is None)
    if training and bn.track_running_stats and bn.num_batches_tracked is not None and not _nbt_batched[0]:
        bn.num_batches_tracked.add_(1)
    momentum = 0.1 if bn.momentum is None else bn.momentum
    if (training and x.dtype in H16 and _is_cl(x) and not x.is_contiguous()
            and K.bn_nhwc_supported(x.shape[1]) and (res is None or (res.dtype == x.dtype and _is_cl(res)))):
        return _BnActNhwcFn.apply(x, res, bn.weight, bn.bias, bn.running_mean, bn.running_var, momentum, bn.eps, relu,
                                  _sync_world(bn), partial, box, stat_box)
    return _BnActFn.apply(x, res, bn.weight, bn.bias, bn.running_mean, bn.running_var, training, momentum,
                          bn.eps, relu, _sync_world(bn) if training else 1)
```

### hiast_amd/kernels.py

```python
import ctypes

import numpy as np
import torch

from . import _lib
from . import switches as _SW
from ._lib import NBINS, check


def _stream():
    return ctypes.c_void_p(torch._C._cuda_getCurrentRawStream(torch._C._cuda_getDevice()))


def _ptr(t):
    return ctypes.c_void_p(t.data_ptr()) if t is not None else ctypes.c_void_p(0)


def h2d_async(host, device, out=None):
    stage = torch.from_numpy(np.ascontiguousarray(host)).pin_memory()
    if out is None:
        return stage.to(device, non_blocking=True)
    out.copy_(stage.view(out.dtype).reshape(out.shape) if stage.dtype != out.dtype else stage.reshape(out.shape),
              non_blocking=True)
    return out
# ... 891 lines not shown
                                         float(eps), int(bool(relu)), _ptr(sm), _ptr(si), B, C, HW, _bn_dtype(x),
                                         _stream()), "hiast_bn_act_apply")
    return y, sm, si


def bn_act_bwd_stats(dy, y, x, save_mean, save_invstd, relu):
    B, C, HW = _bn_dims(x)
    assert dy.shape == x.shape and dy.dtype == x.dtype and dy.is_contiguous()
    part = torch.empty((C, B, 2), dtype=torch.float64, device=x.device)
    check(_lib.load().hiast_bn_act_bwd_stats(_ptr(dy), _ptr(y), _ptr(x), _ptr(save_mean), _ptr(save_invstd),
                                             int(bool(relu)), B, C, HW, _bn_dtype(x), _ptr(part), _stream()),
          "hiast_bn_act_bwd_stats")
    return part


def bn_act_bwd_apply(dy, y, x, gamma, save_mean, save_invstd, part, count, relu, want_dres, want_dparam):
    B, C, HW = _bn_dims(x)
    dx = torch.empty_like(x)
    dres = torch.empty_like(x) if want_dres else None
    dg = torch.empty(C, dtype=torch.float32, device=x.device) if want_dparam else None
    db = torch.empty(C, dtype=torch.float32, device=x.device) if want_dparam else None
    check(_lib.load().hiast_bn_act_bwd_apply(_ptr(dy), _ptr(y), _ptr(x), _ptr(gamma), _ptr(save_mean),
                                             _ptr(save_invstd), _ptr(part), part.shape[1], float(count),
                                             int(bool(relu)), _ptr(dx), _ptr(dres), _ptr(dg), _ptr(db), B, C, HW,
                                             _bn_dtype(x), _stream()), "hiast_bn_act_bwd_apply")
    return dx, dres, dg, db


def _act_dtype(t):
    if t.dtype == torch.float32:
        return 0
    if t.dtype == torch.bfloat16:
        return 1
    raise TypeError("NHWC conv kernels take float32 or bfloat16 activations, got %s" % t.dtype)


def _act_dtype16(t):
    return 2 if t.dtype == torch.float16 else _act_dtype(t)


def _bn_params(bn):
    return (_ptr(bn.weight), _ptr(bn.bias), _ptr(bn.running_mean), _ptr(bn.running_var), float(bn.eps))


def bn_act_nhwc_infer(x2d, bn, relu=True):
    dt = _act_dtype(x2d)
    _req(x2d, x2d.dtype, 2, "x2d")
    M, C = x2d.shape
    y = torch.empty_like(x2d)
    g, b, mu, var, eps = _bn_params(bn)
    check(_lib.load().hiast_bn_act_nhwc_infer(_ptr(x2d), _ptr(y), g, b, mu, var, eps, int(bool(relu)), M, C, dt,
                                              _stream()), "hiast_bn_act_nhwc_infer")
    return y


def maxpool3x3s2_cl_fwd(x):
    if not (x.is_cuda and x.dtype in _H16 and x.dim() == 4 and x.permute(0, 2, 3, 1).is_contiguous()):
        raise ValueError("maxpool3x3s2_cl: x must be a channels-last bfloat16 / float16 HIP tensor [B,C,H,W]")
    B, C, H, W = x.shape
    Ho, Wo = (H - 1) // 2 + 1, (W - 1) // 2 + 1
    y = torch.empty((B, C, Ho, Wo), dtype=x.dtype, device=x.device, memory_format=torch.channels_last)
    idx = torch.empty((B, Ho, Wo, C), dtype=torch.uint8, device=x.device)
    check(_lib.load().hiast_maxpool3x3s2_nhwc_fwd(_ptr(x), _ptr(y), _ptr(idx), B, H, W, C, fmt_of(x), _stream()),
          "hiast_maxpool3x3s2_nhwc_fwd")
    return y, idx


def maxpool3x3s2_cl_bwd(dy, idx, H, W):
    if not (dy.is_cuda and dy.dtype in _H16 and dy.dim() == 4 and dy.permute(0, 2, 3, 1).is_contiguous()):
        raise ValueError("maxpool3x3s2_cl: dy must be a channels-last bfloat16 / float16 HIP tensor [B,C,Ho,Wo]")
    B, C, Ho, Wo = dy.shape
    assert tuple(idx.shape) == (B, Ho, Wo, C) and idx.dtype == torch.uint8
    dx = torch.empty((B, C, H, W), dtype=dy.dtype, device=dy.device, memory_format=torch.channels_last)
    check(_lib.load().hiast_maxpool3x3s2_nhwc_bwd(_ptr(dy), _ptr(idx), _ptr(dx), B, H, W, C, fmt_of(dy), _stream()),
          "hiast_maxpool3x3s2_nhwc_bwd")
    return dx


def stem_tail(x, bn, fmt):
    dt = _act_dtype16(x)
    fmt = int(fmt)
    B, C, H, W = x.shape
    assert x.permute(0, 2, 3, 1).is_contiguous(), "stem_tail: x must be channels-last"
    Ho, Wo = (H - 1) // 2 + 1, (W - 1) // 2 + 1
    out = torch.empty((B, Ho, Wo, (2 if fmt == FMT_SPLIT_BF16 else 1) * C), dtype=fmt_dtype(fmt), device=x.device)
    g, b, mu, var, eps = _bn_params(bn)
    check(_lib.load().hiast_stem_tail(_ptr(x), dt, g, b, mu, var, eps, _ptr(out), fmt, B, H, W, C, _stream()),
          "hiast_stem_tail")
    return out


def stem_eval_supported(conv, bn, pool):
    import os
    return (os.environ.get("HIAST_NO_STEM_FUSED", "0") != "1"
            and (conv.in_channels, conv.out_channels, conv.kernel_size, conv.stride, conv.padding, conv.dilation, conv.groups)
            == (3, 64, (7, 7), (2, 2), (3, 3), (1, 1), 1) and conv.bias is None and bn.num_features == 64 and not bn.training
            and (pool.kernel_size, pool.stride, pool.padding, pool.dilation, pool.ceil_mode) == (3, 2, 1, 1, False))


def stem_eval(x, weight, bn, fmt):
    x = x.contiguous()
    _req(x, torch.float32, 4, "x")
    _req(weight, torch.float32, 4, "stem weight")
    assert tuple(weight.shape) == (64, 3, 7, 7) and x.shape[1] == 3
    fmt = int(fmt)
    B, _, H, W = x.shape
    Hc, Wc = (H - 1) // 2 + 1, (W - 1) // 2 + 1
    Hp, Wp = (Hc - 1) // 2 + 1, (Wc - 1) // 2 + 1
    out = torch.empty((B, Hp, Wp, (2 if fmt == FMT_SPLIT_BF16 else 1) * 64), dtype=fmt_dtype(fmt), device=x.device)
    g, b, mu, var, eps = _bn_params(bn)
    check(_lib.load().hiast_stem_eval(_ptr(x), _ptr(weight), g, b, mu, var, eps, _ptr(out), fmt, B, H, W, _stream()),
          "hiast_stem_eval")
    return out


def stem_train_supported(conv):
    return (not _SW.on("HIAST_LIB_STEM")
            and (conv.in_channels, conv.out_channels, conv.kernel_size, conv.stride, conv.padding, conv.dilation, conv.groups)
            == (3, 64, (7, 7), (2, 2), (3, 3), (1, 1), 1) and conv.bias is None)


def stem_train_shape_ok(x):
    B, _, H, W = x.shape
    return x.dtype == torch.float32 and _lib.load().hiast_stem_train_blocks(int(B), int(H), int(W)) > 0


def stem_train_fwd(x, weight, fmt):
    _req(x, torch.float32, 4, "x")
    _req(weight, torch.float32, 4, "stem weight")
    assert tuple(weight.shape) == (64, 3, 7, 7) and x.shape[1] == 3
    fmt = int(fmt)
    B, _, H, W = x.shape
    Hc, Wc = (H - 1) // 2 + 1, (W - 1) // 2 + 1
    lib = _lib.load()
    nblk = lib.hiast_stem_train_blocks(B, H, W)
    if nblk <= 0:
        raise _lib.HiastLibraryError("hiast_stem_train_fwd: unsupported geometry B=%d H=%d W=%d" % (B, H, W))
    y = torch.empty((B, Hc, Wc, 64), dtype=fmt_dtype(fmt), device=x.device)
    partial = torch.empty((nblk, 64, 2), dtype=torch.float32, device=x.device)
    check(lib.hiast_stem_train_fwd(_ptr(x), _ptr(weight), _ptr(y), _ptr(partial), fmt, B, H, W, _stream()),
          "hiast_stem_train_fwd")
    return y, partial


_stem_ws = {}


def stem_wgrad(x, dy):
    _req(x, torch.float32, 4, "x")
    _req16(dy, 4, "dy")
    B, _, H, W = x.shape
    assert tuple(dy.shape) == (B, (H - 1) // 2 + 1, (W - 1) // 2 + 1, 64)
    lib = _lib.load()
    need = lib.hiast_stem_wgrad_workspace_bytes(B, H, W)
    if need == 0:
        raise _lib.HiastLibraryError("hiast_stem_wgrad: unsupported geometry B=%d H=%d W=%d" % (B, H, W))
    key = (x.device, torch.cuda.current_stream(x.device).cuda_stream)
    ws = _stem_ws.get(key)
    if ws is None or ws.numel() * 4 < need:
        ws = torch.empty((need + 3) // 4, dtype=torch.float32, device=x.device)
        _stem_ws[key] = ws
    dw = torch.empty((64, 3, 7, 7), dtype=torch.float32, device=x.device)
    check(lib.hiast_stem_wgrad(_ptr(x), _ptr(dy), _ptr(dw), fmt_of(dy), B, H, W, _ptr(ws), ws.numel() * 4, _stream()),
          "hiast_stem_wgrad")
    return dw


def split_planes(x2d):
    _req(x2d, torch.float32, 2, "x2d")
    M, C = x2d.shape
    p = torch.empty((M, 2 * C), dtype=torch.bfloat16, device=x2d.device)
    check(_lib.load().hiast_split_planes(_ptr(x2d), _ptr(p), M, C, 0, _stream()), "hiast_split_planes")
    return p


def merge_planes(p):
    _req(p, torch.bfloat16, 2, "planes")
    M, C2 = p.shape
    x = torch.empty((M, C2 // 2), dtype=torch.float32, device=p.device)
    check(_lib.load().hiast_split_planes(_ptr(x), _ptr(p), M, C2 // 2, 1, _stream()), "hiast_split_planes")
    return x


def pack_conv_weight(weight, fmt, transpose=False, both=False):
    fmt = int(fmt)
    planes, h16 = (2 if fmt == FMT_SPLIT_BF16 else 1), fmt_dtype(fmt)
    w = weight.detach()
    if w.dim() == 2:
        w = w.reshape(w.shape[0], w.shape[1], 1, 1)
    _req(w, torch.float32, 4, "weight")
    N, K_, kh, kw = w.shape
    fwd_shape, adj_shape = (N, kh * kw, planes * K_), (K_, kh * kw, planes * N)
    wpt = None
    if both:
        wp = torch.empty(fwd_shape, dtype=h16, device=w.device)
        wpt = torch.empty(adj_shape, dtype=h16, device=w.device)
        mode = 2
    else:
        wp = torch.empty(adj_shape if transpose else fwd_shape, dtype=h16, device=w.device)
        mode = 1 if transpose else 0
    check(_lib.load().hiast_pack_conv_weight(_ptr(w), N, K_, kh * kw, fmt, mode, _ptr(wp), _ptr(wpt), _stream()),
          "hiast_pack_conv_weight")
    return (wp, wpt) if both else wp


class PackPlan:
    CHUNK = 65536
    REC = np.dtype([("w", np.int64), ("wp", np.int64), ("wpt", np.int64), ("N", np.int32), ("K", np.int32),
                    ("taps", np.int32), ("planes", np.int32), ("mode", np.int32), ("pad", np.int32)])

    def __init__(self, weights, fmt, adjoint):
        assert len(weights) > 0 and len(weights) == len(adjoint)
        dev = weights[0].device
        fmt = int(fmt)
        planes, h16 = (2 if fmt == FMT_SPLIT_BF16 else 1), fmt_dtype(fmt)
        self.weights, self.fmt = list(weights), fmt
        self.wp, self.wpt = [], []
        host = np.zeros(len(weights), dtype=self.REC)
        lists = {}
        for i, (w, adj) in enumerate(zip(weights, adjoint)):
            _req(w.detach(), torch.float32, 4, "weight")
            N, K_, kh, kw = w.shape
            taps = kh * kw
            wp = torch.empty((N, taps, planes * K_), dtype=h16, device=dev)
            wpt = torch.empty((K_, taps, planes * N), dtype=h16, device=dev) if adj else None
            self.wp.append(wp)
            self.wpt.append(wpt)
            host[i] = (w.data_ptr(), wp.data_ptr(), wpt.data_ptr() if adj else 0, N, K_, taps, fmt, 2 if adj else 0, 0)
            if N % 64 or K_ % 64 or taps > 9:
                raise ValueError("PackPlan: channel counts must be multiples of 64 (got %d x %d)" % (N, K_))
            ct, cs = lists.setdefault(taps, ([], []))
            for tile in range((N // 64) * (K_ // 64)):
                ct.append(i)
                cs.append(tile)
        self.ptrs = [w.data_ptr() for w in weights]
        self.table = torch.from_numpy(host.view(np.uint8).reshape(-1).copy()).to(dev)
        self.launches = [(taps, torch.tensor(ct, dtype=torch.int32, device=dev), torch.tensor(cs, dtype=torch.int64, device=dev),
                          len(ct)) for taps, (ct, cs) in sorted(lists.items())]
        self.versions = None

    def still_valid(self):
        return all(w.data_ptr() == p for w, p in zip(self.weights, self.ptrs))

    def refresh(self):
        v = [w._version for w in self.weights]
        if v == self.versions:
            return False
        for taps, ct, cs, n in self.launches:
            check(_lib.load().hiast_pack_conv_weight_multi(_ptr(self.table), _ptr(ct), _ptr(cs), n, taps, _stream()),
                  "hiast_pack_conv_weight_multi")
        self.versions = v
        return True


def igemm_bn_act(x, wp, planes, bn, res, relu, stride=1, dil=1, out_f32=False, want_stats=False, res_gate=None):
    _req16(x, 4, "x")
    PL = 2 if int(planes) == 2 else 1
    fmt = fmt_of(x, PL)
    _req(wp, x.dtype, 3, "wp")
    B, H, W, CC = x.shape
    Cin = CC // PL
    N, taps, KK = wp.shape
    assert PL in (1, 2) and KK == PL * Cin and CC == PL * Cin and taps in (1, 9), (tuple(x.shape), tuple(wp.shape), PL)
    if taps == 1:
        assert stride == 1
        Ho, Wo = H, W
    else:
        Ho, Wo = (H - 1) // stride + 1, (W - 1) // stride + 1
    if out_f32:
        y = torch.empty((B, Ho, Wo, N), dtype=torch.float32, device=x.device)
        assert res is None
    else:
        y = torch.empty((B, Ho, Wo, PL * N), dtype=x.dtype, device=x.device)
    if res is not None:
        _req(res, x.dtype, 4, "res")
        assert tuple(res.shape) == tuple(y.shape)
    gate_mask = 0
    if res_gate is not None:
        assert PL == 1 and res is not None
        if res_gate.dtype == torch.uint8:
            _req(res_gate, torch.uint8, 2, "res_gate")
            assert tuple(res_gate.shape) == (B * Ho * Wo, N // 8)
            gate_mask = 1
        else:
            _req(res_gate, x.dtype, 4, "res_gate")
            assert tuple(res_gate.shape) == tuple(res.shape)
    if bn is not None:
        g, b, mu, var, eps = _bn_params(bn)
    else:
        g = b = mu = var = ctypes.c_void_p(0)
        eps = 0.0
    partial = None
    rows = 0
    if want_stats:
        assert PL == 1 and not out_f32
        rows = _lib.load().hiast_igemm_stats_rows(B * Ho * Wo, Cin, N, taps, fmt)
        partial = torch.empty((rows, N, 2), dtype=torch.float32, device=x.device)
    check(_lib.load().hiast_igemm_bn_act(_ptr(x), _ptr(wp), g, b, mu, var, eps, _ptr(res), int(bool(relu)), _ptr(y),
                                         B, H, W, Cin, N, taps, int(stride), int(dil), fmt, int(bool(out_f32)),
                                         _ptr(partial), rows, _ptr(res_gate), gate_mask, _stream()), "hiast_igemm_bn_act")
    return (y, partial) if want_stats else y


def igemm_dgrad_bn_stats(dy, wpt, dil, bn_x, gamma, beta, save_mean, save_invstd):
    _req16(dy, 4, "dy")
    _req(wpt, dy.dtype, 3, "wpt")
    _req(bn_x, dy.dtype, 4, "bn_x")
    B, H, W, Cin = dy.shape
    N, taps, KK = wpt.shape
    assert KK == Cin and taps in (1, 9) and tuple(bn_x.shape) == (B, H, W, N), (tuple(dy.shape), tuple(wpt.shape), tuple(bn_x.shape))
    _req(save_mean, torch.float32, 1, "save_mean")
    _req(save_invstd, torch.float32, 1, "save_invstd")
    lib = _lib.load()
    da = torch.empty((B, H, W, N), dtype=dy.dtype, device=dy.device)
    rows = lib.hiast_igemm_dgrad_bn_stats_rows(B * H * W, Cin, N, taps)
    partial = torch.empty((rows, N, 2), dtype=torch.float32, device=dy.device)
    check(lib.hiast_igemm_dgrad_bn_stats(_ptr(dy), _ptr(wpt), _ptr(da), B, H, W, Cin, N, taps, int(dil), _ptr(bn_x),
                                         _ptr(gamma), _ptr(beta), _ptr(save_mean), _ptr(save_invstd), _ptr(partial),
                                         rows, fmt_of(dy), _stream()), "hiast_igemm_dgrad_bn_stats")
    return da, partial


def xconv_dgrad_gated_bn_stats_ok(M, K, N):
    return _lib.load().hiast_xconv_dgrad_gated_bn_stats_rows(int(M), int(K), int(N)) > 0


def xconv_dgrad_gated_bn_stats(dy, wpt, res, res_gate, bn_x, bn_mask, save_mean, save_invstd):
    _req16(dy, 4, "dy")
    _req(wpt, dy.dtype, 3, "wpt")
    _req(res, dy.dtype, 4, "res")
    _req(bn_x, dy.dtype, 4, "bn_x")
    B, H, W, Kc = dy.shape
    N, taps, KK = wpt.shape
    M = B * H * W
    assert taps == 1 and KK == Kc and tuple(res.shape) == (B, H, W, N) and tuple(bn_x.shape) == (B, H, W, N)
    for t, nm in ((res_gate, "res_gate"), (bn_mask, "bn_mask")):
        _req(t, torch.uint8, 2, nm)
        assert tuple(t.shape) == (M, N // 8), nm
    _req(save_mean, torch.float32, 1, "save_mean")
    _req(save_invstd, torch.float32, 1, "save_invstd")
    lib = _lib.load()
    rows = lib.hiast_xconv_dgrad_gated_bn_stats_rows(M, Kc, N)
    if rows <= 0:
        raise _lib.HiastLibraryError("hiast_xconv_dgrad_gated_bn_stats: unsupported shape M=%d K=%d N=%d" % (M, Kc, N))
    dx = torch.empty((B, H, W, N), dtype=dy.dtype, device=dy.device)
    partial = torch.empty((rows, N, 2), dtype=torch.float32, device=dy.device)
    check(lib.hiast_xconv_dgrad_gated_bn_stats(_ptr(dy), _ptr(wpt), _ptr(res), _ptr(res_gate), _ptr(bn_x), _ptr(bn_mask),
                                               _ptr(save_mean), _ptr(save_invstd), _ptr(dx), _ptr(partial), M, Kc, N,
                                               fmt_of(dy), _stream()), "hiast_xconv_dgrad_gated_bn_stats")
    return dx, partial


def igemm_dgrad_s2(dy, wpt, H, W):
    _req16(dy, 4, "dy")
    _req(wpt, dy.dtype, 3, "wpt")
    B, Hs, Ws, Cout = dy.shape
    N, taps, KK = wpt.shape
    assert taps == 9 and KK == Cout and (Hs, Ws) == ((H - 1) // 2 + 1, (W - 1) // 2 + 1), (tuple(dy.shape), tuple(wpt.shape), H, W)
    dx = torch.empty((B, H, W, N), dtype=dy.dtype, device=dy.device)
    check(_lib.load().hiast_igemm_dgrad_s2(_ptr(dy), _ptr(wpt), _ptr(dx), B, H, W, N, Cout, fmt_of(dy), _stream()),
          "hiast_igemm_dgrad_s2")
    return dx


def _bnh_view(t, name):
    if not isinstance(t, torch.Tensor) or not t.is_cuda:
        raise _lib.HiastLibraryError("%s must be a CUDA(HIP) tensor: the HIP path has no CPU fallback" % name)
    if t.dtype not in _H16 or t.dim() != 4:
        raise TypeError("%s must be a 4-d bfloat16 / float16 tensor" % name)
    v = t.permute(0, 2, 3, 1)
    if not v.is_contiguous():
        raise ValueError("%s must be channels-last contiguous" % name)
    B, H, W, C = v.shape
    return v, B * H * W, C


_bnh_ws = {}


def _bnh_workspace(C, device):
    key = (C, device)
    ws = _bnh_ws.get(key)
    if ws is None:
        n = _lib.load().hiast_bn_nhwc_workspace_bytes(C)
        ws = torch.empty(n // 4, dtype=torch.float32, device=device)
        _bnh_ws[key] = ws
    return ws


def bn_nhwc_supported(C):
    return 8 <= C <= 2048 and (C & (C - 1)) == 0


def bn_nhwc_stats(x):
    xv, M, C = _bnh_view(x, "x")
    sums = torch.empty((C, 2), dtype=torch.float64, device=x.device)
    ws = _bnh_workspace(C, x.device)
    check(_lib.load().hiast_bn_nhwc_stats(_ptr(xv), M, C, _ptr(sums), _ptr(ws), ws.numel() * 4, fmt_of(x), _stream()),
          "hiast_bn_nhwc_stats")
    return sums


def bn_nhwc_stats_from_partial(partial):
    _req(partial, torch.float32, 3, "partial")
    nblk, C, two = partial.shape
    assert two == 2
    sums = torch.empty((C, 2), dtype=torch.float64, device=partial.device)
    check(_lib.load().hiast_bn_nhwc_stats_from_partial(_ptr(partial), nblk, C, _ptr(sums), _stream()),
          "hiast_bn_nhwc_stats_from_partial")
    return sums


def bn_nhwc_apply(x, res, gamma, beta, running_mean, running_var, sums, count, momentum, eps, relu, want_mask=False):
    xv, M, C = _bnh_view(x, "x")
    y = torch.empty_like(x, memory_format=torch.channels_last)
    mask = torch.empty((M, C // 8), dtype=torch.uint8, device=x.device) if want_mask else None
    rv = None
    if res is not None:
        rv, M2, C2 = _bnh_view(res, "res")
        assert (M2, C2) == (M, C)
    assert sums.dtype == torch.float64 and tuple(sums.shape) == (C, 2) and sums.is_contiguous()
    sm = torch.empty(C, dtype=torch.float32, device=x.device)
    si = torch.empty(C, dtype=torch.float32, device=x.device)
    check(_lib.load().hiast_bn_nhwc_apply(_ptr(xv), _ptr(rv), _ptr(y), _ptr(gamma), _ptr(beta), _ptr(running_mean),
                                          _ptr(running_var), _ptr(sums), float(count), float(momentum), float(eps),
                                          int(bool(relu)), _ptr(sm), _ptr(si), M, C, _ptr(mask), fmt_of(x), _stream()),
          "hiast_bn_nhwc_apply")
    return (y, sm, si, mask) if want_mask else (y, sm, si)


def bn_nhwc_apply_partial(x, res, gamma, beta, running_mean, running_var, partial, count, momentum, eps, relu,
                          want_mask=False):
    xv, M, C = _bnh_view(x, "x")
    mask = torch.empty((M, C // 8), dtype=torch.uint8, device=x.device) if want_mask else None
    _req(partial, torch.float32, 3, "partial")
    assert partial.shape[1] == C and partial.shape[2] == 2
    y = torch.empty_like(x, memory_format=torch.channels_last)
    rv = _bnh_view(res, "res")[0] if res is not None else None
    sm = torch.empty(C, dtype=torch.float32, device=x.device)
    si = torch.empty(C, dtype=torch.float32, device=x.device)
    check(_lib.load().hiast_bn_nhwc_apply_partial(_ptr(xv), _ptr(rv), _ptr(y), _ptr(gamma), _ptr(beta), _ptr(running_mean),
                                                  _ptr(running_var), _ptr(partial), partial.shape[0], float(count),
                                                  float(momentum), float(eps), int(bool(relu)), _ptr(sm), _ptr(si), M, C,
                                                  _ptr(mask), fmt_of(x), _stream()), "hiast_bn_nhwc_apply_partial")
    return (y, sm, si, mask) if want_mask else (y, sm, si)


def bn_nhwc_bwd_stats(dy, y, x, gamma, beta, save_mean, save_invstd, gate):
    xv, M, C = _bnh_view(x, "x")
    dv, M2, C2 = _bnh_view(dy, "dy")
    assert (M2, C2) == (M, C)
    yv = _bnh_view(y, "y")[0] if gate == 1 else (_req(y, torch.uint8, 2, "mask") if gate == 3 else None)
    sums = torch.empty((C, 2), dtype=torch.float64, device=x.device)
    ws = _bnh_workspace(C, x.device)
    check(_lib.load().hiast_bn_nhwc_bwd_stats(_ptr(dv), _ptr(yv), _ptr(xv), _ptr(gamma), _ptr(beta), _ptr(save_mean),
                                              _ptr(save_invstd), int(gate), M, C, _ptr(sums), _ptr(ws), ws.numel() * 4,
                                              fmt_of(x), _stream()), "hiast_bn_nhwc_bwd_stats")
    return sums


def bn_nhwc_bwd_apply(dy, y, x, gamma, beta, save_mean, save_invstd, sums, count, gate, want_dres, want_dparam):
    xv, M, C = _bnh_view(x, "x")
    dv = _bnh_view(dy, "dy")[0]
    yv = _bnh_view(y, "y")[0] if gate == 1 else (_req(y, torch.uint8, 2, "mask") if gate == 3 else None)
    dx = torch.empty_like(x, memory_format=torch.channels_last)
    dres = torch.empty_like(x, memory_format=torch.channels_last) if want_dres else None
    dg = torch.empty(C, dtype=torch.float32, device=x.device) if want_dparam else None
    db = torch.empty(C, dtype=torch.float32, device=x.device) if want_dparam else None
    check(_lib.load().hiast_bn_nhwc_bwd_apply(_ptr(dv), _ptr(yv), _ptr(xv), _ptr(gamma), _ptr(beta), _ptr(save_mean),
                                              _ptr(save_invstd), _ptr(sums), float(count), int(gate), _ptr(dx),
                                              _ptr(dres), _ptr(dg), _ptr(db), M, C, fmt_of(x), _stream()),
          "hiast_bn_nhwc_bwd_apply")
    return dx, dres, dg, db


_wgrad_ws = {}


def conv_wgrad_supported(Cin, Cout, k, stride):
    return Cin % 256 == 0 and Cout % 256 == 0 and k in (1, 3) and (k == 3 or stride == 1)


def conv_wgrad_preferred(Cin, Cout, k, stride):
    import os
    if not conv_wgrad_supported(Cin, Cout, k, stride):
        return False
    return k == 1 or os.environ.get("HIAST_LIB_WGRAD3", "0") != "1"


def conv_wgrad_small_supported(Cin, Cout, k, stride):
    import os

    def chan(c):
        return c == 64 or (c >= 128 and c % 128 == 0)
    if os.environ.get("HIAST_LIB_WGRAD_SMALL", "0") == "1" or conv_wgrad_supported(Cin, Cout, k, stride):
        return False
    return chan(Cin) and chan(Cout) and ((k == 1 and stride in (1, 2)) or k == 3)


def conv_wgrad_small_nhwc(dy, x, k, stride, dil):
    _req16(dy, 4, "dy")
    _req(x, dy.dtype, 4, "x")
    if stride != 1 and k == 1:
        x = x[:, ::stride, ::stride, :].contiguous()
        stride = 1
    B, H, W, Cin = x.shape
    Bo, Ho, Wo, Cout = dy.shape
    assert (Bo, Ho, Wo) == (B, (H - 1) // stride + 1, (W - 1) // stride + 1)
    taps = k * k
    lib = _lib.load()
    n = lib.hiast_conv_wgrad_small_workspace_bytes(B, Ho, Wo, Cin, Cout, taps)
    if n == 0:
        raise _lib.HiastLibraryError("hiast_conv_wgrad_small_nhwc: unsupported shape Cin=%d Cout=%d taps=%d" % (Cin, Cout, taps))
    key = ("small", x.device, torch.cuda.current_stream(x.device).cuda_stream)
    ws = _wgrad_ws.get(key)
    if ws is None or ws.numel() * 4 < n:
        ws = torch.empty((n + 3) // 4, dtype=torch.float32, device=x.device)
        _wgrad_ws[key] = ws
    dw = torch.empty((Cout, Cin, k, k), dtype=torch.float32, device=x.device)
    check(lib.hiast_conv_wgrad_small_nhwc(_ptr(dy), _ptr(x), _ptr(dw), B, H, W, Cin, Cout, taps, int(stride), int(dil), fmt_of(dy),
                                          _ptr(ws), ws.numel() * 4, _stream()), "hiast_conv_wgrad_small_nhwc")
    return dw


def conv_wgrad_nhwc(dy, x, k, stride, dil):
    _req16(dy, 4, "dy")
    _req(x, dy.dtype, 4, "x")
    B, H, W, Cin = x.shape
    Bo, Ho, Wo, Cout = dy.shape
    taps = k * k
    assert Bo == B and (Ho, Wo) == ((H, W) if k == 1 else ((H - 1) // stride + 1, (W - 1) // stride + 1))
    lib = _lib.load()
    n = lib.hiast_conv_wgrad_workspace_bytes(B, Ho, Wo, Cin, Cout, taps)
    if n == 0:
        raise _lib.HiastLibraryError("hiast_conv_wgrad_nhwc: unsupported shape Cin=%d Cout=%d taps=%d" % (Cin, Cout, taps))
    key = ("big", x.device, torch.cuda.current_stream(x.device).cuda_stream)
    ws = _wgrad_ws.get(key)
    if ws is None or ws.numel() * 4 < n:
        ws = torch.empty((n + 3) // 4, dtype=torch.float32, device=x.device)
        _wgrad_ws[key] = ws
    dw = torch.empty((Cout, Cin, k, k), dtype=torch.float32, device=x.device)
    check(lib.hiast_conv_wgrad_nhwc(_ptr(dy), _ptr(x), _ptr(dw), B, H, W, Cin, Cout, taps, int(stride), int(dil), fmt_of(dy),
                                    _ptr(ws), ws.numel() * 4, _stream()), "hiast_conv_wgrad_nhwc")
    return dw


def conv_wgrad_group(jobs):
    import ctypes
    lib = _lib.load()
    n = len(jobs)
    arr = (_lib.WgradJob * n)()
    outs = []
    fmt = None
    for i, (dy, x, k, stride, dil) in enumerate(jobs):
        _req16(dy, 4, "dy")
        _req(x, dy.dtype, 4, "x")
        B, H, W, Cin = x.shape
        Bo, Ho, Wo, Cout = dy.shape
        assert Bo == B and (Ho, Wo) == ((H, W) if k == 1 else ((H - 1) // stride + 1, (W - 1) // stride + 1))
        assert fmt is None or fmt == fmt_of(dy), "one operand type per grouped launch"
        fmt = fmt_of(dy)
        dw = torch.empty((Cout, Cin, k, k), dtype=torch.float32, device=x.device)
        outs.append(dw)
        arr[i] = _lib.WgradJob(_ptr(dy), _ptr(x), _ptr(dw), B, H, W, Cin, Cout, k * k, int(stride), int(dil))
    need = lib.hiast_conv_wgrad_group_workspace_bytes(ctypes.addressof(arr), n)
    if need == 0:
        raise _lib.HiastLibraryError("hiast_conv_wgrad_group_nhwc: unsupported shapes %s" %
                                     [(tuple(j[0].shape), tuple(j[1].shape), j[2]) for j in jobs])
    dev = jobs[0][1].device
    key = ("group", dev, torch.cuda.current_stream(dev).cuda_stream)
    ws = _wgrad_ws.get(key)
    if ws is None or ws.numel() * 4 < need:
        ws = torch.empty((need + 3) // 4, dtype=torch.float32, device=dev)
        _wgrad_ws[key] = ws
    check(lib.hiast_conv_wgrad_group_nhwc(ctypes.addressof(arr), n, fmt, _ptr(ws), ws.numel() * 4, _stream()),
          "hiast_conv_wgrad_group_nhwc")
    return outs


def disc_conv_workspace_bytes(B, Cin, Cout, H, W):
    return int(_lib.load().hiast_disc_conv_workspace_bytes(int(B), int(Cin), int(Cout), int(H), int(W)))


def _disc_conv_ws(x_shape, Cout, device):
    B, Cin, H, W = x_shape
    n = disc_conv_workspace_bytes(B, Cin, Cout, H, W)
    if n == 0:
        raise _lib.HiastLibraryError("hiast_disc_conv: unsupported shape x=%s Cout=%d" % (tuple(x_shape), Cout))
    key = ("disc", device, torch.cuda.current_stream(device).cuda_stream)
    ws = _wgrad_ws.get(key)
    if ws is None or ws.numel() * 4 < n:
        ws = torch.empty((n + 3) // 4, dtype=torch.float32, device=device)
        _wgrad_ws[key] = ws
    return ws


def _disc_conv_shapes(x, weight):
    B, Cin, H, W = x.shape
    Cout = weight.shape[0]
    if tuple(weight.shape) != (Cout, Cin, 4, 4):
        raise ValueError("weight must be [Cout, %d, 4, 4], got %s" % (Cin, tuple(weight.shape)))
    if H < 2 or W < 2:
        raise ValueError("a 4x4 stride-2 padding-1 convolution needs H, W >= 2, got %s" % (tuple(x.shape),))
    return B, Cin, Cout, H, W, (H - 2) // 2 + 1, (W - 2) // 2 + 1


def _disc_fmt(fmt):
    if isinstance(fmt, torch.dtype):
        if fmt not in _H16:
            raise TypeError("the 16-bit discriminator convolutions take float16 or bfloat16, got %s" % fmt)
        return FMT_FP16 if fmt == torch.float16 else FMT_BF16
    if fmt is None or int(fmt) not in (FMT_FP16, FMT_BF16):
        raise ValueError("fmt must be FMT_FP16 or FMT_BF16, got %r" % (fmt,))
    return int(fmt)


def _disc_conv_fwd(x, weight, bias, leaky, fmt):
    _req(x, torch.float32, 4, "x")
    _req(weight, torch.float32, 4, "weight")
    B, Cin, Cout, H, W, Ho, Wo = _disc_conv_shapes(x, weight)
    if bias is not None:
        _req(bias, torch.float32, 1, "bias")
        assert bias.numel() == Cout
    y = torch.empty((B, Cout, Ho, Wo), dtype=torch.float32, device=x.device)
    lib = _lib.load()
    args = (_ptr(x), _ptr(weight), _ptr(bias), _ptr(y), B, Cin, Cout, H, W, int(bool(leaky)))
    if fmt is None:
        check(lib.hiast_disc_conv_fwd(*args, _stream()), "hiast_disc_conv_fwd")
    else:
        check(lib.hiast_disc_conv16_fwd(*args, fmt, _stream()), "hiast_disc_conv16_fwd")
    return y


def _disc_conv_dgrad(dy, y, weight, x_shape, leaky, fmt):
    _req(dy, torch.float32, 4, "dy")
    _req(weight, torch.float32, 4, "weight")
    x_shape = tuple(int(s) for s in x_shape)
    B, Cin, Cout, H, W, Ho, Wo = _disc_conv_shapes(torch.empty(x_shape, device="meta"), weight)
    assert tuple(dy.shape) == (B, Cout, Ho, Wo), (tuple(dy.shape), (B, Cout, Ho, Wo))
    if leaky:
        _req(y, torch.float32, 4, "y")
        assert y.shape == dy.shape
    ws = _disc_conv_ws(x_shape, Cout, dy.device)
    dx = torch.empty(x_shape, dtype=torch.float32, device=dy.device)
    lib = _lib.load()
    args = (_ptr(dy), _ptr(y if leaky else None), _ptr(weight), _ptr(dx), B, Cin, Cout, H, W, int(bool(leaky)))
    tail = (_ptr(ws), ws.numel() * 4, _stream())
    if fmt is None:
        check(lib.hiast_disc_conv_dgrad(*args, *tail), "hiast_disc_conv_dgrad")
    else:
        check(lib.hiast_disc_conv16_dgrad(*args, fmt, *tail), "hiast_disc_conv16_dgrad")
    return dx


def _disc_conv_wgrad(x, dy, y, leaky, want_bias, fmt):
    _req(x, torch.float32, 4, "x")
    _req(dy, torch.float32, 4, "dy")
    B, Cin, H, W = x.shape
    Cout = dy.shape[1]
    assert H >= 2 and W >= 2 and tuple(dy.shape) == (B, Cout, (H - 2) // 2 + 1, (W - 2) // 2 + 1), (tuple(x.shape), tuple(dy.shape))
    if leaky:
        _req(y, torch.float32, 4, "y")
        assert y.shape == dy.shape
    ws = _disc_conv_ws(tuple(x.shape), Cout, x.device)
    dw = torch.empty((Cout, Cin, 4, 4), dtype=torch.float32, device=x.device)
    db = torch.empty((Cout,), dtype=torch.float32, device=x.device) if want_bias else None
    lib = _lib.load()
    args = (_ptr(x), _ptr(dy), _ptr(y if leaky else None), _ptr(dw), _ptr(db), B, Cin, Cout, H, W, int(bool(leaky)))
    tail = (_ptr(ws), ws.numel() * 4, _stream())
    if fmt is None:
        check(lib.hiast_disc_conv_wgrad(*args, *tail), "hiast_disc_conv_wgrad")
    else:
        check(lib.hiast_disc_conv16_wgrad(*args, fmt, *tail), "hiast_disc_conv16_wgrad")
    return dw, db


def disc_conv_fwd(x, weight, bias, leaky):
    return _disc_conv_fwd(x, weight, bias, leaky, None)


def disc_conv_dgrad(dy, y, weight, x_shape, leaky):
    return _disc_conv_dgrad(dy, y, weight, x_shape, leaky, None)


def disc_conv_wgrad(x, dy, y, leaky, want_bias=True):
    return _disc_conv_wgrad(x, dy, y, leaky, want_bias, None)


def disc_conv16_fwd(x, weight, bias, leaky, fmt):
    return _disc_conv_fwd(x, weight, bias, leaky, _disc_fmt(fmt))


def disc_conv16_dgrad(dy, y, weight, x_shape, leaky, fmt):
    return _disc_conv_dgrad(dy, y, weight, x_shape, leaky, _disc_fmt(fmt))


def disc_conv16_wgrad(x, dy, y, leaky, fmt, want_bias=True):
    return _disc_conv_wgrad(x, dy, y, leaky, want_bias, _disc_fmt(fmt))
```

### hiast_amd/sseg/models/modules/resnet.py

```python
import os

import torch
import torch.nn as nn
import torch.nn.functional as F

from hiast_amd import functional as HF


def bn_act(bn, x, res=None, relu=True, partial=None):
    if x.is_cuda:
        return HF.bn_act(x, bn, res, relu, partial=partial)
    y = bn(x)
    if res is not None:
        y = y + res
    return F.relu(y) if relu else y


def conv(m, x):
    if x.is_cuda and x.dtype in HF.H16 and HF.conv_nhwc_ok(x, m):
        return HF.conv_nhwc(x, m)
    return m(x)


def conv_bn_act(cv, bn, x, res=None, relu=True, conv_box=None, bn_box=None, in_bn=None, stat_box=None, wgroup=None, xsum=None,
                in_bn3=None):
    if x.is_cuda and x.dtype in HF.H16 and bn.training and HF.conv_nhwc_ok(x, cv):
        y, partial = HF.conv_nhwc(x, cv, want_stats=True, box=conv_box, in_bn=in_bn, wgroup=wgroup, xsum=xsum, in_bn3=in_bn3)
        return HF.bn_act(y, bn, res, relu, partial=partial, box=bn_box, stat_box=stat_box)
    return bn_act(bn, conv(cv, x), res, relu)


def _nhwc2d(t):
    B, C, H, W = t.shape
    return t.permute(0, 2, 3, 1).reshape(B * H * W, C)


def _from2d(y2d, B, H, W):
    return y2d.view(B, H, W, y2d.shape[1]).permute(0, 3, 1, 2)


def packed_weight(conv, fmt):
    from hiast_amd import kernels as K
    w = conv.weight
    cache = conv.__dict__.setdefault("_hiast_packed", {})
    ent = cache.get(fmt)
    if ent is not None and ent[0] == w._version and ent[1] == w.data_ptr():
        return ent[2]
    wp = K.pack_conv_weight(w, fmt)
    cache[fmt] = (w._version, w.data_ptr(), wp)
    return wp


class Bottleneck(nn.Module):
    expansion = 4

    def __init__(self, inplanes, planes, stride=1, dilation=1, downsample=None):
        super().__init__()
        self.conv1 = nn.Conv2d(inplanes, planes, 1, bias=False)
        self.bn1 = nn.BatchNorm2d(planes)
        self.conv2 = nn.Conv2d(planes, planes, 3, stride=stride, padding=dilation, dilation=dilation, bias=False)
        self.bn2 = nn.BatchNorm2d(planes)
        self.conv3 = nn.Conv2d(planes, planes * 4, 1, bias=False)
        self.bn3 = nn.BatchNorm2d(planes * 4)
        self.relu = nn.ReLU(inplace=True)
        self.downsample = downsample

    def forward(self, x):
        xs = None
        if (self.downsample is not None and self.downsample[0].stride == (1, 1) and x.is_cuda and x.dtype in HF.H16
                and self.bn1.training and x.requires_grad and not HF.SW.on("HIAST_NO_XSUM")):
            xs = {}
        idt = x if self.downsample is None else conv_bn_act(self.downsample[0], self.downsample[1], x, relu=False,
                                                            xsum=None if xs is None else (xs, "take"))
        box = {} if (self.downsample is None and not HF.SW.on("HIAST_NO_IDT_HANDOFF")) else None
        sb1, sb2 = {}, {}
        grp, wv = (None, None)
        if x.is_cuda and x.dtype in HF.H16 and self.bn1.training:
            grp, wv = HF.wgroup_weights((self.conv1, self.conv2, self.conv3), x)
        g = (lambda i: (grp, grp["slot"][i], wv[i]) if wv[i] is not None else None) if grp is not None else (lambda i: None)
        o = conv_bn_act(self.conv1, self.bn1, x, conv_box=box, stat_box=sb1, wgroup=g(0),
                        xsum=None if xs is None else (xs, "give"), in_bn3=getattr(x, "_hiast_bn3", None) if box is not None else None)
        o = conv_bn_act(self.conv2, self.bn2, o, in_bn=sb1, stat_box=sb2, wgroup=g(1))
        sb3 = {}
        y = conv_bn_act(self.conv3, self.bn3, o, res=idt, bn_box=box, in_bn=sb2, stat_box=sb3, wgroup=g(2))
        if "bn3" in sb3:
            y._hiast_bn3 = sb3
        return y

    def forward_eval_planes(self, x, fmt):
        from hiast_amd import kernels as K
        PL = 2 if fmt == K.FMT_SPLIT_BF16 else 1
        o = K.igemm_bn_act(x, packed_weight(self.conv1, fmt), PL, self.bn1, None, True)
        if self.downsample is None:
            idt = x
        else:
            dconv, dbn = self.downsample[0], self.downsample[1]
            xs = x if dconv.stride == (1, 1) else x[:, ::dconv.stride[0], ::dconv.stride[1]].contiguous()
            idt = K.igemm_bn_act(xs, packed_weight(dconv, fmt), PL, dbn, None, False)
        o = K.igemm_bn_act(o, packed_weight(self.conv2, fmt), PL, self.bn2, None, True, self.conv2.stride[0],
                           self.conv2.dilation[0])
        return K.igemm_bn_act(o, packed_weight(self.conv3, fmt), PL, self.bn3, idt, True)


class ResNet(nn.Module):

    def __init__(self, layers=(3, 4, 23, 3), strides=(1, 2, 2, 2), dilations=((1, 1), (1, 1), (1, 1), (1, 1))):
        super().__init__()
        self.inplanes = 64
        self.conv1 = nn.Conv2d(3, 64, 7, stride=2, padding=3, bias=False)
        self.bn1 = nn.BatchNorm2d(64)
        self.relu = nn.ReLU(inplace=True)
        self.maxpool = nn.MaxPool2d(3, stride=2, padding=1)
        for i, (planes, n) in enumerate(zip((64, 128, 256, 512), layers)):
            setattr(self, "layer%d" % (i + 1), self._stage(planes, n, strides[i], dilations[i]))
        for m in self.modules():
            if isinstance(m, nn.Conv2d):
                nn.init.kaiming_normal_(m.weight, mode="fan_out", nonlinearity="relu")
            elif isinstance(m, nn.BatchNorm2d):
                nn.init.constant_(m.weight, 1)
                nn.init.constant_(m.bias, 0)

    def _stage(self, planes, n, stride, dil):
        down = None
        if stride != 1 or self.inplanes != planes * 4:
            down = nn.Sequential(nn.Conv2d(self.inplanes, planes * 4, 1, stride=stride, bias=False),
                                 nn.BatchNorm2d(planes * 4))
        blocks = [Bottleneck(self.inplanes, planes, stride, dil[0], down)]
        self.inplanes = planes * 4
        blocks += [Bottleneck(self.inplanes, planes, 1, dil[1]) for _ in range(1, n)]
        return nn.Sequential(*blocks)

    def prepack(self, PL, adjoint=False):
        from hiast_amd import kernels as K
        plans = self.__dict__.setdefault("_hiast_plans", {})
        ent = plans.get((PL, adjoint))
        if ent is None or not ent[0].still_valid():
            convs = []
            for stage in (self.layer1, self.layer2, self.layer3, self.layer4):
                for blk in stage:
                    convs += [blk.conv1, blk.conv2, blk.conv3] + ([blk.downsample[0]] if blk.downsample is not None else [])
            convs = [c for c in convs if c.in_channels % 64 == 0 and c.out_channels % 64 == 0 and c.weight.is_cuda]
            if not convs:
                return
            plan = K.PackPlan([c.weight for c in convs], PL,
                              [adjoint and (c.stride == (1, 1) or c.kernel_size == (1, 1)
                                            or (c.kernel_size == (3, 3) and c.stride == (2, 2) and c.dilation == (1, 1)))
                               for c in convs])
            ent = (plan, convs)
            plans[(PL, adjoint)] = ent
        plan, convs = ent
        if plan.refresh() or not getattr(plan, "published", False):
            for i, c in enumerate(convs):
                w = c.weight
                c.__dict__.setdefault("_hiast_packed", {})[PL] = (w._version, w.data_ptr(), plan.wp[i])
                if plan.wpt[i] is not None:
                    c.__dict__.setdefault("_hiast_packed_adj", {})[PL] = (w._version, w.data_ptr(), plan.wpt[i])
            plan.published = True

    def fast_eval_planes(self, x):
        if self.training or not x.is_cuda or torch.is_grad_enabled() or x.dtype != torch.float32:
            return 0
        if os.environ.get("HIAST_NO_FAST_EVAL", "0") == "1":
            return 0
        if not torch.is_autocast_enabled():
            return 2
        amp = torch.get_autocast_dtype("cuda")
        return 1 if amp == torch.bfloat16 else (3 if amp == torch.float16 else 0)

    def forward_eval_planes(self, x, PL):
        from hiast_amd import kernels as K
        self.prepack(PL)
        if K.stem_eval_supported(self.conv1, self.bn1, self.maxpool) and x.dtype == torch.float32 and x.shape[1] == 3:
            o = K.stem_eval(x, self.conv1.weight.detach(), self.bn1, PL)
            for stage in (self.layer1, self.layer2, self.layer3, self.layer4):
                for blk in stage:
                    o = blk.forward_eval_planes(o, PL)
            return o
        x = x.contiguous(memory_format=torch.channels_last)
        o = self.conv1(x)
        o = o.contiguous(memory_format=torch.channels_last)
        mp = self.maxpool
        if ((mp.kernel_size, mp.stride, mp.padding, mp.dilation, mp.ceil_mode) == (3, 2, 1, 1, False)
                and o.shape[1] % 32 == 0 and o.dtype in (torch.float32, torch.bfloat16, torch.float16)
                and os.environ.get("HIAST_NO_STEM_TAIL", "0") != "1"):
            o = K.stem_tail(o, self.bn1, PL)
            for stage in (self.layer1, self.layer2, self.layer3, self.layer4):
                for blk in stage:
                    o = blk.forward_eval_planes(o, PL)
            return o
        B, _, H, W = o.shape
        o = _from2d(K.bn_act_nhwc_infer(_nhwc2d(o), self.bn1, True), B, H, W)
        o = self.maxpool(o)
        B, C, H, W = o.shape
        o2d = _nhwc2d(o.contiguous(memory_format=torch.channels_last))
        if PL == 2:
            o = K.split_planes(o2d.float()).view(B, H, W, 2 * C)
        else:
            o = o2d.to(K.fmt_dtype(PL)).view(B, H, W, C)
        for stage in (self.layer1, self.layer2, self.layer3, self.layer4):
            for blk in stage:
                o = blk.forward_eval_planes(o, PL)
        return o

    @staticmethod
    def planes_to_feature(p, PL):
        from hiast_amd import kernels as K
        B, h, w, CC = p.shape
        if PL == 2:
            return _from2d(K.merge_planes(p.view(B * h * w, CC)), B, h, w)
        return p.permute(0, 3, 1, 2)

    def forward(self, x, is_return_low=False):
        stem_partial = None
        if not is_return_low:
            PL = self.fast_eval_planes(x)
            if PL:
                return self.planes_to_feature(self.forward_eval_planes(x, PL), PL)
        if (x.is_cuda and torch.is_autocast_enabled() and torch.get_autocast_dtype("cuda") in HF.H16
                and os.environ.get("HIAST_TRAIN_NCHW", "0") != "1"):
            if self.training and torch.is_grad_enabled():
                self.prepack(3 if torch.get_autocast_dtype("cuda") == torch.float16 else 1, adjoint=True)
            from hiast_amd import kernels as K
            if (self.bn1.training and K.stem_train_supported(self.conv1) and not x.requires_grad
                    and K.stem_train_shape_ok(x)):
                x, stem_partial = HF.stem_conv_train(x, self.conv1)
            else:
                x = x.contiguous(memory_format=torch.channels_last)
                x = self.conv1(x).contiguous(memory_format=torch.channels_last)
        else:
            x = self.conv1(x)
        batched = False
        if self.training and x.is_cuda:
            nbt = self.__dict__.get("_hiast_nbt")
            if nbt is None or nbt[0].device != x.device:
                nbt = [m.num_batches_tracked for m in self.modules()
                       if isinstance(m, nn.modules.batchnorm._BatchNorm) and m.track_running_stats
                       and m.num_batches_tracked is not None]
                self.__dict__["_hiast_nbt"] = nbt
            if nbt:
                torch._foreach_add_(nbt, 1)
                batched = True
        prev = HF._nbt_batched[0]
        HF._nbt_batched[0] = batched or prev
        try:
            x = HF.maxpool(bn_act(self.bn1, x, partial=stem_partial), self.maxpool)
            low = self.layer1(x)
            x = self.layer4(self.layer3(self.layer2(low)))
        finally:
            HF._nbt_batched[0] = prev
        return (x, low) if is_return_low else x


def build_resnet101(pretrained=False, output_stride=32):
    if pretrained:
        raise RuntimeError("ImageNet weights cannot be downloaded here; pass pretrained=False and load a state dict")
    if output_stride == 8:
        return ResNet(strides=(1, 2, 1, 1), dilations=((1, 1), (1, 1), (1, 2), (2, 4)))
    return ResNet()
```

### include/hiast_hip.h

```cpp
#ifndef HIAST_HIP_H
#define HIAST_HIP_H

#include <stddef.h>
#include <stdint.h>

#ifdef __cplusplus
extern "C" {
#endif

#define HIAST_ABI_VERSION 6

#define HIAST_E_ARG   (-1)
#define HIAST_E_RANGE (-2)
#define HIAST_E_WS    (-3)

#define HIAST_NBINS 15361
#define HIAST_PROB_FX_SHIFT 30
#define HIAST_MAX_CLASSES 32
#define HIAST_FMT_BF16 1
#define HIAST_FMT_SPLIT_BF16 2
#define HIAST_FMT_FP16 3
#define HIAST_IGNORE 255

typedef void* hiast_stream_t;

int hiast_version(void);
const char* hiast_error_string(int code);

int hiast_device_cus(void);
int hiast_set_reserve_cus(int n);
int hiast_get_reserve_cus(void);
int hiast_stream_create_reserved(hiast_stream_t* out, int reserve);
int hiast_stream_destroy(hiast_stream_t s);

int hiast_upsample_bilinear_ac_fwd(const float* in, float* out, int B, int C, int h, int w,
                                   int H, int W, hiast_stream_t stream);
int hiast_upsample_bilinear_ac_bwd(const float* gout, float* gin, int B, int C, int h, int w,
                                   int H, int W, hiast_stream_t stream);

size_t hiast_plabel_pass1_workspace_bytes(int C);
int hiast_plabel_pass1(const float* logits_lr, int B, int C, int h, int w, int H, int W,
                       float* maxprob, uint8_t* argmax, uint32_t* hist, void* workspace,
                       size_t workspace_bytes, hiast_stream_t stream);

int hiast_plabel_pass2(const float* maxprob, const uint8_t* argmax, const float* thr_up,
                       int B, int C, int64_t HW, uint8_t* plbl, int64_t* count,
                       uint64_t* sumprob_fx, hiast_stream_t stream);

size_t hiast_plabel_strided_hist_workspace_bytes(int64_t N, int C);
int hiast_plabel_strided_hist(const float* maxprob, const uint8_t* argmax, int64_t N, int C, int interval,
                              const int64_t* rank_offset, int64_t* class_total, uint32_t* hist,
                              void* workspace, size_t workspace_bytes, hiast_stream_t stream);

#define HIAST_TTA_MAX_SCALES 8
int hiast_tta_fused(const float* const* z, const float* const* zf, const int* hs, const int* ws, const int* Hs,
                    const int* Ws, int n_scales, int B, int C, int H, int W, float* probsum, uint8_t* label,
                    hiast_stream_t stream);

#define HIAST_CST_SOFTCE 0
#define HIAST_CST_CE 1
#define HIAST_CST_KLDIV 2
#define HIAST_CST_MSE 3
size_t hiast_st_loss_workspace_bytes(int B, int C, int h, int w, int H, int W);
int hiast_st_loss_fwd(const float* logits_lr, const float* teacher_lr, const void* plbl,
                      int plbl_is_i64, int B, int C, int h, int w, int H, int W, int region,
                      double* sums, void* workspace, size_t workspace_bytes,
                      hiast_stream_t stream);
int hiast_st_loss_bwd(const float* logits_lr, const float* teacher_lr, const void* plbl,
                      int plbl_is_i64, int B, int C, int h, int w, int H, int W, int region,
                      const double* sums, const float* coef, float* dlogits_lr,
                      void* workspace, size_t workspace_bytes, hiast_stream_t stream);
int hiast_st_loss_cst_fwd(const float* logits_lr, const float* teacher_lr, const void* plbl,
                          int plbl_is_i64, int B, int C, int h, int w, int H, int W, int region, int cst_kind,
                          double* sums, void* workspace, size_t workspace_bytes, hiast_stream_t stream);
int hiast_st_loss_cst_bwd(const float* logits_lr, const float* teacher_lr, const void* plbl,
                          int plbl_is_i64, int B, int C, int h, int w, int H, int W, int region, int cst_kind,
                          const double* sums, const float* coef, float* dlogits_lr,
                          void* workspace, size_t workspace_bytes, hiast_stream_t stream);

size_t hiast_aspp_wpack_bytes(int Cin, int Cout);
size_t hiast_aspp_workspace_bytes(int B, int Cin, int h, int w, int Cout);
int hiast_aspp_pack_weights(const float* w0, const float* w1, const float* w2, const float* w3,
                            const float* b0, const float* b1, const float* b2, const float* b3,
                            int Cin, int Cout, float* wpack, hiast_stream_t stream);
int hiast_aspp_fwd(const float* x, const float* wpack, float* y, int B, int Cin, int h, int w,
                   int Cout, const int* dil, void* workspace, size_t workspace_bytes,
                   hiast_stream_t stream);
int hiast_aspp_bwd_data(const float* dy, const float* wpack, float* dx, int B, int Cin, int h,
                        int w, int Cout, const int* dil, hiast_stream_t stream);
int hiast_aspp_bwd_weight(const float* x, const float* dy, float* dw0, float* dw1, float* dw2,
                          float* dw3, float* db, int B, int Cin, int h, int w, int Cout,
                          const int* dil, void* workspace, size_t workspace_bytes,
                          hiast_stream_t stream);

int hiast_aspp2_np(int Cout);
size_t hiast_aspp2_workspace_bytes(int B, int Cin, int h, int w, int Cout, int backward);
int hiast_aspp2_pack_weights(const float* w0, const float* w1, const float* w2, const float* w3,
                             const float* b0, const float* b1, const float* b2, const float* b3, int Cin,
                             int Cout, float* wt, float* wd, float* bias, hiast_stream_t stream);
int hiast_aspp2_fwd(const void* x_nhwc, int dtype, const void* wt, const float* bias, float* y, int B, int Cin,
                    int h, int w, int Cout, const int* dil, void* workspace, size_t workspace_bytes,
                    hiast_stream_t stream);
int hiast_aspp2_bwd(const void* x_nhwc, const float* dy, const void* wd, void* dx_nhwc, float* dw0, float* dw1,
                    float* dw2, float* dw3, float* db, int B, int Cin, int h, int w, int Cout, const int* dil,
                    int fmt ,
                    void* workspace, size_t workspace_bytes, hiast_stream_t stream);

size_t hiast_bn_workspace_bytes(int B, int C);
int hiast_bn_stats(const void* x, int B, int C, int64_t HW, int dtype, double* part, hiast_stream_t stream);
int hiast_bn_act_apply(const void* x, const void* res, void* y, const float* gamma, const float* beta,
                       float* running_mean, float* running_var, const double* part, int npart, double count,
                       float momentum, float eps, int relu, float* save_mean, float* save_invstd, int B, int C,
                       int64_t HW, int dtype, hiast_stream_t stream);
int hiast_bn_act_bwd_stats(const void* dy, const void* y, const void* x, const float* save_mean,
                           const float* save_invstd, int relu, int B, int C, int64_t HW, int dtype,
                           double* part, hiast_stream_t stream);
int hiast_bn_act_bwd_apply(const void* dy, const void* y, const void* x, const float* gamma,
                           const float* save_mean, const float* save_invstd, const double* part, int npart,
                           double count, int relu, void* dx, void* dres, float* dgamma, float* dbeta, int B,
                           int C, int64_t HW, int dtype, hiast_stream_t stream);

int hiast_bn_act_nhwc_infer(const void* x, void* y, const float* gamma, const float* beta, const float* mean,
                            const float* var, float eps, int relu, int64_t M, int C, int dtype,
                            hiast_stream_t stream);

int hiast_igemm_bn_act(const void* x, const void* wp, const float* gamma, const float* beta, const float* mean,
                       const float* var, float eps, const void* res, int relu, void* y, int B, int H, int W, int Cin,
                       int Cout, int taps, int stride, int dil, int fmt , int out_f32, float* stats,
                       int stats_rows ,
                       const void* res_gate, int gate_mask, hiast_stream_t stream);
int hiast_igemm_set_cosched(int on);
int hiast_igemm_set_half(int v);
int hiast_igemm_stats_rows(int64_t M, int Cin, int Cout, int taps, int fmt);
int hiast_igemm_dgrad_bn_stats(const void* dy, const void* wpt, void* da, int B, int H, int W, int Cin, int Cout, int taps,
                               int dil, const void* bn_x, const float* gamma, const float* beta, const float* save_mean,
                               const float* save_invstd, float* partial, int partial_rows ,
                               int fmt , hiast_stream_t stream);
int hiast_igemm_dgrad_bn_stats_rows(int64_t M, int Cin, int Cout, int taps);
int hiast_igemm_dgrad_s2(const void* dy, const void* wpt, void* dx, int B, int H, int W, int Cin, int Cout, int fmt,
                         hiast_stream_t stream);
int hiast_xconv_dgrad_gated_bn_stats_rows(int64_t M, int K, int N);
int hiast_xconv_dgrad_gated_bn_stats(const void* dy, const void* wpt, const void* res, const void* res_gate, const void* bn_x,
                                     const void* bn_mask, const float* save_mean, const float* save_invstd, void* dx,
                                     float* partial, int64_t M, int K, int N, int fmt, hiast_stream_t stream);
int hiast_pack_conv_weight(const float* w, int N, int K, int taps, int fmt, int transpose, void* wp, void* wpt,
                           hiast_stream_t stream);
int hiast_split_planes(float* x, void* planes, int64_t M, int C, int inverse, hiast_stream_t stream);
int hiast_stem_tail(const void* x, int dtype , const float* gamma, const float* beta,
                    const float* mean, const float* var, float eps, void* out, int fmt , int B, int H,
                    int W, int C, hiast_stream_t stream);
int hiast_stem_eval(const float* x, const float* w, const float* gamma, const float* beta, const float* mean, const float* var,
                    float eps, void* out, int fmt, int B, int H, int W, hiast_stream_t stream);

int hiast_stem_train_blocks(int B, int H, int W);
int hiast_stem_train_fwd(const float* x, const float* w, void* y, float* partial, int fmt, int B, int H, int W,
                         hiast_stream_t stream);
size_t hiast_stem_wgrad_workspace_bytes(int B, int H, int W);
int hiast_stem_wgrad(const float* x, const void* dy, float* dw, int fmt, int B, int H, int W, void* workspace,
                     size_t workspace_bytes, hiast_stream_t stream);
typedef struct { const float* w; void* wp; void* wpt; int32_t N, K, taps, planes , mode, pad; } hiast_pack_rec;
int hiast_pack_conv_weight_multi(const hiast_pack_rec* table, const int32_t* chunk_tensor, const int64_t* chunk_start,
                                 int n_chunks, int max_taps, hiast_stream_t stream);

size_t hiast_conv_wgrad_workspace_bytes(int B, int Ho, int Wo, int Cin, int Cout, int taps);
int hiast_conv_wgrad_nhwc(const void* dy, const void* x, float* dw, int B, int H, int W, int Cin, int Cout, int taps,
                          int stride, int dil, int fmt ,
                          void* workspace, size_t workspace_bytes, hiast_stream_t stream);

typedef struct { const void* dy; const void* x; float* dw; int32_t B, H, W, Cin, Cout, taps, stride, dil; } hiast_wgrad_job;
size_t hiast_conv_wgrad_group_workspace_bytes(const hiast_wgrad_job* jobs, int njobs);
int hiast_conv_wgrad_group_nhwc(const hiast_wgrad_job* jobs, int njobs, int fmt, void* workspace, size_t workspace_bytes,
                                hiast_stream_t stream);

size_t hiast_conv_wgrad_small_workspace_bytes(int B, int H, int W, int Cin, int Cout, int taps);
int hiast_conv_wgrad_small_nhwc(const void* dy, const void* x, float* dw, int B, int H, int W, int Cin, int Cout, int taps,
                                int stride, int dil, int fmt, void* workspace, size_t workspace_bytes, hiast_stream_t stream);

size_t hiast_bn_nhwc_workspace_bytes(int C);
int hiast_bn_nhwc_stats(const void* x, int64_t M, int C, double* sums, void* workspace, size_t workspace_bytes, int fmt,
                        hiast_stream_t stream);
int hiast_bn_nhwc_stats_from_partial(const float* partial, int nblk, int C, double* sums, hiast_stream_t stream);
int hiast_bn_nhwc_apply_partial(const void* x, const void* res, void* y, const float* gamma, const float* beta,
                                float* running_mean, float* running_var, const float* partial, int nblk, double count,
                                float momentum, float eps, int relu, float* save_mean, float* save_invstd, int64_t M,
                                int C, void* mask, int fmt, hiast_stream_t stream);
int hiast_bn_nhwc_apply(const void* x, const void* res, void* y, const float* gamma, const float* beta,
                        float* running_mean, float* running_var, const double* sums, double count, float momentum,
                        float eps, int relu, float* save_mean, float* save_invstd, int64_t M, int C, void* mask, int fmt,
                        hiast_stream_t stream);
int hiast_bn_nhwc_bwd_stats(const void* dy, const void* y, const void* x, const float* gamma, const float* beta,
                            const float* save_mean, const float* save_invstd, int relu, int64_t M, int C, double* sums,
                            void* workspace, size_t workspace_bytes, int fmt, hiast_stream_t stream);
int hiast_bn_nhwc_bwd_apply(const void* dy, const void* y, const void* x, const float* gamma, const float* beta,
                            const float* save_mean, const float* save_invstd, const double* sums, double count, int relu,
                            void* dx, void* dres, float* dgamma, float* dbeta, int64_t M, int C, int fmt,
                            hiast_stream_t stream);

typedef struct { float* ema; const float* p; int64_t n; } hiast_ema_rec;
int hiast_ema_update(const hiast_ema_rec* table, const int32_t* chunk_tensor,
                     const int64_t* chunk_start, int n_chunks, float gamma,
                     float one_minus_gamma, hiast_stream_t stream);

int hiast_maxpool3x3s2_nhwc_fwd(const void* x, void* y, uint8_t* idx, int B, int H, int W, int C,
                                int fmt , hiast_stream_t stream);
int hiast_maxpool3x3s2_nhwc_bwd(const void* dy, const uint8_t* idx, void* dx, int B, int H, int W, int C, int fmt,
                                hiast_stream_t stream);

int hiast_normalize_u8(const uint8_t* img, float* out, int B, int64_t HW, const float* mean, const float* std,
                       hiast_stream_t stream);

#define HIAST_AUG_REC_WORDS 20
#define HIAST_AUG_MAX_OPS 8
#define HIAST_AUG_OPS_WORDS (4 + 2 * HIAST_AUG_MAX_OPS)
#define HIAST_AUG_OP_LUT 1
#define HIAST_AUG_OP_GRAY 2
#define HIAST_AUG_OP_EQUALIZE 3
int hiast_aug_geometry_u8(const int64_t* recs, const uint8_t* blob, const int32_t* tabs, uint8_t* tmp,
                          uint8_t* img_out, uint8_t* lbl_out, int B, int max_ch, int oh, int ow, hiast_stream_t stream);
int hiast_aug_hist_u8(const int64_t* ops, const uint8_t* blob, const uint8_t* in, uint32_t* hist, uint8_t* eq_lut,
                      int B, int64_t HW, hiast_stream_t stream);
int hiast_aug_colour_u8(const int64_t* ops, const uint8_t* blob, const uint8_t* eq_lut, const uint8_t* in,
                        uint8_t* out, int B, int64_t HW, hiast_stream_t stream);

#define HIAST_AUG_OP_CONTRAST 4
#define HIAST_AUG_OP_SAT 5
#define HIAST_AUG_OP_HUE 6
#define HIAST_AUG_OP_BLUR 7
#define HIAST_AUG_MAX_KSIZE 41
int hiast_aug2_table_u8(const int64_t* ops, const int32_t* seg, const uint8_t* blob, const uint8_t* in, uint32_t* hist,
                        uint8_t* table, int B, int64_t HW, hiast_stream_t stream);
int hiast_aug2_colour_u8(const int64_t* ops, const int32_t* seg, const uint8_t* blob, const uint8_t* table,
                         const uint8_t* in, uint8_t* out, int B, int64_t HW, hiast_stream_t stream);
int hiast_aug2_blur_u8(const int64_t* ops, const int32_t* seg, const int32_t* tabs, uint8_t* img, float* tmp, int B,
                       int H, int W, hiast_stream_t stream);

typedef struct { void* dst; const void* src; int64_t nbytes; } hiast_copy_rec;
int hiast_multi_copy(const hiast_copy_rec* table, int n_tensors, hiast_stream_t stream);

typedef struct { float* p; const float* g; float* m; float* v; int64_t n; float lr; float bc1; float bc2_sqrt; float step; } hiast_adam_rec;
typedef struct { float skipped; float skip; float inv_scale; float pad[5]; } hiast_adam_ctl;
int hiast_adam_prepare(hiast_adam_ctl* ctl, const float* grad_scale, const float* found_inf, hiast_stream_t stream);
int hiast_adam_step(const hiast_adam_rec* table, const int32_t* chunk_tensor, const int64_t* chunk_start,
                    int n_chunks, double beta1, double beta2, float eps, float weight_decay, const hiast_adam_ctl* ctl,
                    hiast_stream_t stream);

typedef struct { float* p; const float* g; float* buf; int64_t n; float lr; float pad; } hiast_sgd_rec;
int hiast_sgd_step(const hiast_sgd_rec* table, const int32_t* chunk_tensor, const int64_t* chunk_start, int n_chunks,
                   float momentum, float weight_decay, const hiast_adam_ctl* ctl, hiast_stream_t stream);

typedef struct { float* p; const float* g; float* m; float* v; int64_t n; float lr; float bc1; float bc2_sqrt; float step; float decay; float pad; } hiast_adamw_rec;
int hiast_adamw_step(const hiast_adamw_rec* table, const int32_t* chunk_tensor, const int64_t* chunk_start, int n_chunks,
                     double beta1, double beta2, float eps, const hiast_adam_ctl* ctl, hiast_stream_t stream);

int hiast_dinput_fwd(const float* logits_lr, int mode, float* out, int B, int C, int h, int w, int H, int W,
                     hiast_stream_t stream);
int hiast_dinput_bwd(const float* logits_lr, int mode, const float* gout, float* scratch, float* dlogits_lr,
                     int B, int C, int h, int w, int H, int W, hiast_stream_t stream);

size_t hiast_disc_conv_workspace_bytes(int B, int Cin, int Cout, int H, int W);
int hiast_disc_conv_fwd(const float* x, const float* w, const float* bias, float* y, int B, int Cin, int Cout, int H, int W,
                        int leaky, hiast_stream_t stream);
int hiast_disc_conv_dgrad(const float* dy, const float* y, const float* w, float* dx, int B, int Cin, int Cout, int H, int W,
                          int leaky, void* workspace, size_t workspace_bytes, hiast_stream_t stream);
int hiast_disc_conv_wgrad(const float* x, const float* dy, const float* y, float* dw, float* db, int B, int Cin, int Cout,
                          int H, int W, int leaky, void* workspace, size_t workspace_bytes, hiast_stream_t stream);
int hiast_disc_conv16_fwd(const float* x, const float* w, const float* bias, float* y, int B, int Cin, int Cout, int H, int W,
                          int leaky, int fmt, hiast_stream_t stream);
int hiast_disc_conv16_dgrad(const float* dy, const float* y, const float* w, float* dx, int B, int Cin, int Cout, int H, int W,
                            int leaky, int fmt, void* workspace, size_t workspace_bytes, hiast_stream_t stream);
int hiast_disc_conv16_wgrad(const float* x, const float* dy, const float* y, float* dw, float* db, int B, int Cin, int Cout,
                            int H, int W, int leaky, int fmt, void* workspace, size_t workspace_bytes, hiast_stream_t stream);

int hiast_confusion_hist(const int64_t* pred, const int64_t* target, int64_t N, int K,
                         int64_t* inter, int64_t* area_pred, int64_t* area_tgt,
                         hiast_stream_t stream);

#ifdef __cplusplus
}
#endif
#endif
```

Measured before the change: 141.9.

## Fuse bn3 backward apply into conv3 dgrad GEMM with bn2 stats epilogue

Adds a kernel that computes the bn3 backward input gradient (gated by the ReLU mask bits) on the fly while staging the A operand of the conv3 data-gradient GEMM. It also writes dx, runs the MFMA GEMM against packed weights, and in the epilogue applies the bn2 ReLU gate and accumulates bn2 backward partial statistics. Separately, dgamma/dbeta are now derived inside the stats-from-partial and bwd-stats kernels. The aim is to remove a full read/write pass over the bottleneck activations and several separate kernel launches per bottleneck block in backward. In exchange it adds a large, shape-restricted kernel (N=256, K up to 1024) with heavy LDS use, plus more Python plumbing that is only used when the bottleneck box is active.

```diff
diff --git a/hiast_amd/_lib.py b/hiast_amd/_lib.py
--- a/hiast_amd/_lib.py
+++ b/hiast_amd/_lib.py
@@ -61,6 +61,9 @@
     "hiast_igemm_dgrad_s2": (c_int, [c_vp, c_vp, c_vp] + [c_int] * 6 + [c_vp]),
     "hiast_igemm_dgrad_bn_stats_rows": (c_int, [c_i64, c_int, c_int, c_int]),
     "hiast_bn_nhwc_stats_from_partial": (c_int, [c_vp, c_int, c_int, c_vp, c_vp]),
+    "hiast_bn_nhwc_stats_from_partial_dparam": (c_int, [c_vp, c_int, c_int, c_vp, c_vp, c_vp, c_vp]),
+    "hiast_bn_bwd_dgrad_rows": (c_int, [c_i64, c_int, c_int]),
+    "hiast_bn_bwd_dgrad": (c_int, [c_vp] * 7 + [ctypes.c_double] + [c_vp] * 9 + [c_i64, c_int, c_int, c_int, c_vp]),
     "hiast_conv_wgrad_workspace_bytes": (c_sz, [c_int] * 6),
     "hiast_conv_wgrad_nhwc": (c_int, [c_vp, c_vp, c_vp] + [c_int] * 9 + [c_vp, c_sz, c_vp]),
     "hiast_conv_wgrad_group_workspace_bytes": (c_sz, [c_vp, c_int]),
@@ -75,6 +78,7 @@
     "hiast_bn_nhwc_apply_partial": (c_int, [c_vp] * 8 + [c_int, ctypes.c_double, c_f32, c_f32, c_int, c_vp, c_vp, c_i64,
                                             c_int, c_vp, c_int, c_vp]),
     "hiast_bn_nhwc_bwd_stats": (c_int, [c_vp] * 7 + [c_int, c_i64, c_int, c_vp, c_vp, c_sz, c_int, c_vp]),
+    "hiast_bn_nhwc_bwd_stats_dparam": (c_int, [c_vp] * 7 + [c_int, c_i64, c_int, c_vp, c_vp, c_sz, c_int, c_vp, c_vp, c_vp]),
     "hiast_bn_nhwc_bwd_apply": (c_int, [c_vp] * 8 + [ctypes.c_double, c_int, c_vp, c_vp, c_vp, c_vp, c_i64, c_int, c_int,
                                         c_vp]),
     "hiast_pack_conv_weight_multi": (c_int, [c_vp, c_vp, c_vp, c_int, c_int, c_vp]),
diff --git a/hiast_amd/csrc/bn_dgrad.hip b/hiast_amd/csrc/bn_dgrad.hip
--- /dev/null
+++ b/hiast_amd/csrc/bn_dgrad.hip
@@ -0,0 +1,314 @@
+#include "igemm_kernel.h"
+
+namespace hiast {
+
+constexpr int BD_A = 256 * 128, BD_B = 256 * 128;
+constexpr int BD_KMAX = 1024;
+constexpr int BD_PAR = 5 * BD_KMAX * 4;
+constexpr int BD_LDS = 2 * BD_A + 2 * BD_B + BD_PAR;
+
+template <bool F16>
+__global__ __launch_bounds__(512) void bn_bwd_dgrad_kernel(
+    const unsigned short* __restrict__ G, const unsigned char* __restrict__ bits, const unsigned short* __restrict__ X3,
+    const float* __restrict__ gamma3, const float* __restrict__ mean3, const float* __restrict__ invstd3,
+    const double* __restrict__ sums, double inv_count, const unsigned short* __restrict__ Wp,
+    const unsigned short* __restrict__ R, const float* __restrict__ gamma, const float* __restrict__ beta,
+    const float* __restrict__ mean, const float* __restrict__ var, unsigned short* __restrict__ dx,
+    unsigned short* __restrict__ Y, float* __restrict__ stats, int M, int K)
+{
+    using HT = H16<F16>;
+    constexpr int N = 256, WN = 4, WM = 2, TM = 4, NA = 8, EP = 68, NWV = 8;
+    static_assert(BD_LDS <= 160 * 1024 && 2 * BD_A + 2 * BD_B >= NWV * 32 * EP * 4, "LDS budget; the epilogue tiles fit in the operand stages");
+    __shared__ __attribute__((aligned(1024))) unsigned char smem[BD_LDS];
+    float* sP = reinterpret_cast<float*>(smem + 2 * BD_A + 2 * BD_B);
+
+    const int tid = threadIdx.x, lane = tid & 63;
+    const int wave = __builtin_amdgcn_readfirstlane(tid >> 6);
+    const int wm = wave / WN, wn = wave % WN;
+    int bm = blockIdx.x;
+    {
+        const int total = gridDim.x;
+        if ((total & 7) == 0) bm = (bm & 7) * (total >> 3) + (bm >> 3);
+    }
+    const int m0 = bm * 256;
+    const int nk = K >> 6;
+    const bool nt_dx = (long long)M * K * 2 >= H_NT_MIN_BYTES;
+
+    const int srow = lane >> 3, c8 = lane & 7;
+    const int rl0 = wave * 32 + srow;
+    const int mrow = m0 + rl0;
+    const unsigned eo0 = (unsigned)mrow * (unsigned)K + (unsigned)(c8 * 8);
+    const unsigned bo0 = (unsigned)mrow * (unsigned)(K >> 3) + (unsigned)c8;
+    const unsigned lo0 = (unsigned)h_lds_off(rl0, c8);
+    uint4 rg[4], rx[4];
+    unsigned rb[4];
+    auto load_rows = [&](int j, int g) {
+        if (mrow + 8 * g < M) {
+            rg[g] = *reinterpret_cast<const uint4*>(G + eo0 + (unsigned)(8 * g * K + j * 64));
+            rx[g] = *reinterpret_cast<const uint4*>(X3 + eo0 + (unsigned)(8 * g * K + j * 64));
+            rb[g] = bits[bo0 + (unsigned)(g * K + j * 8)];
+        }
+    };
+#pragma unroll
+    for (int g = 0; g < 4; ++g) load_rows(0, g);
+
+    constexpr int OOB = (int)0x80000000;
+    const __amdgpu_buffer_rsrc_t wrs = __builtin_amdgcn_make_buffer_rsrc((void*)Wp, 0, (int)((size_t)N * nk * 128), 0x00020000);
+    const int bv0 = rl0 * nk * 128 + ((lane & 7) ^ ((rl0 >> 1) & 7)) * 16;
+    auto dma_b = [&](int kt, int sb, int g, bool on) {
+        const int voff = ((g & 1) ? (bv0 ^ 64) : bv0) + g * 8 * nk * 128;
+        h_dma16(wrs, smem + 2 * BD_A + sb * BD_B + (4 * wave + g) * 1024, on ? voff : OOB, kt * 128);
+    };
+#pragma unroll
+    for (int g = 0; g < 4; ++g) dma_b(0, 0, g, true);
+
+    for (int c = tid; c < K; c += 512) {
+        const double2 ss = reinterpret_cast<const double2*>(sums)[c];
+        const float mu = mean3[c], is = invstd3[c];
+        float k0, mg, mgx;
+        bn_bwd_consts(gamma3 ? gamma3[c] : 1.0f, is, ss.x, ss.y, inv_count, k0, mg, mgx);
+        sP[c] = k0; sP[K + c] = mg; sP[2 * K + c] = mgx; sP[3 * K + c] = mu; sP[4 * K + c] = is;
+    }
+
+    h_f32x4 acc4[NA][4];
+#pragma unroll
+    for (int a = 0; a < NA; ++a)
+#pragma unroll
+        for (int b = 0; b < 4; ++b) acc4[a][b] = (h_f32x4){0.f, 0.f, 0.f, 0.f};
+
+    const int erow = lane >> 3, ec8 = lane & 7;
+    const int nc = wn * 64 + ec8 * 8;
+    constexpr int RD = 2;
+    uint4 rhA[TM][4];
+    auto load_res = [&](int a) {
+#pragma unroll
+        for (int ps = 0; ps < 4; ++ps) {
+            const int m = m0 + wm * (TM * 32) + a * 32 + ps * 8 + erow;
+            rhA[a][ps] = *reinterpret_cast<const uint4*>(R + (size_t)(m < M ? m : 0) * N + nc);
+        }
+    };
+
+    const int r16 = lane & 15, kq = lane >> 4;
+    const unsigned fswz = (unsigned)((kq ^ ((r16 >> 1) & 7)) << 4);
+    const unsigned lds_base = (unsigned)(size_t)smem;
+    const unsigned fa0 = lds_base + (unsigned)((wm * (TM * 32) + r16) * 128) + fswz;
+    const unsigned fb0 = lds_base + (unsigned)(2 * BD_A + (wn * 64 + r16) * 128) + fswz;
+
+    asm volatile("s_waitcnt lgkmcnt(0)\n\ts_barrier" ::: "memory");
+
+    for (int kt = 0; kt < nk; ++kt) {
+        const int st = kt & 1;
+        asm volatile("s_waitcnt vmcnt(0)" ::: "memory");
+        {
+            float k0[8], mg[8], mgx[8], mu[8], is[8];
+            const float* pp = sP + kt * 64 + c8 * 8;
+#pragma unroll
+            for (int h = 0; h < 2; ++h) {
+                const float4 a0 = *reinterpret_cast<const float4*>(pp + h * 4);
+                const float4 a1 = *reinterpret_cast<const float4*>(pp + K + h * 4);
+                const float4 a2 = *reinterpret_cast<const float4*>(pp + 2 * K + h * 4);
+                const float4 a3 = *reinterpret_cast<const float4*>(pp + 3 * K + h * 4);
+                const float4 a4 = *reinterpret_cast<const float4*>(pp + 4 * K + h * 4);
+                k0[4 * h] = a0.x; k0[4 * h + 1] = a0.y; k0[4 * h + 2] = a0.z; k0[4 * h + 3] = a0.w;
+                mg[4 * h] = a1.x; mg[4 * h + 1] = a1.y; mg[4 * h + 2] = a1.z; mg[4 * h + 3] = a1.w;
+                mgx[4 * h] = a2.x; mgx[4 * h + 1] = a2.y; mgx[4 * h + 2] = a2.z; mgx[4 * h + 3] = a2.w;
+                mu[4 * h] = a3.x; mu[4 * h + 1] = a3.y; mu[4 * h + 2] = a3.z; mu[4 * h + 3] = a3.w;
+                is[4 * h] = a4.x; is[4 * h + 1] = a4.y; is[4 * h + 2] = a4.z; is[4 * h + 3] = a4.w;
+            }
+            const bool more_a = kt + 1 < nk;
+#pragma unroll
+            for (int g = 0; g < 4; ++g) {
+                const bool ok = mrow + 8 * g < M;
+                const unsigned wg[4] = {rg[g].x, rg[g].y, rg[g].z, rg[g].w};
+                const unsigned wx[4] = {rx[g].x, rx[g].y, rx[g].z, rx[g].w};
+                const unsigned gb = rb[g];
+                unsigned w[4];
+#pragma unroll
+                for (int q = 0; q < 4; ++q) {
+                    const float g0 = ((gb >> (2 * q)) & 1u) != 0u ? HT::lo(wg[q]) : 0.f;
+                    const float g1 = ((gb >> (2 * q + 1)) & 1u) != 0u ? HT::hi(wg[q]) : 0.f;
+                    const float v0 = bn_bwd_dx(g0, HT::lo(wx[q]), mu[2 * q], is[2 * q], k0[2 * q], mg[2 * q], mgx[2 * q]);
+                    const float v1 = bn_bwd_dx(g1, HT::hi(wx[q]), mu[2 * q + 1], is[2 * q + 1], k0[2 * q + 1], mg[2 * q + 1],
+                                               mgx[2 * q + 1]);
+                    w[q] = ok ? HT::pack(v0, v1) : 0u;
+                }
+                if (more_a) load_rows(kt + 1, g);
+                *reinterpret_cast<uint4*>(smem + st * BD_A + (((g & 1) ? (lo0 ^ 64u) : lo0) + g * 1024)) =
+                    make_uint4(w[0], w[1], w[2], w[3]);
+                if (ok) h_store16(dx + eo0 + (unsigned)(8 * g * K + kt * 64), w[0], w[1], w[2], w[3], nt_dx);
+            }
+        }
+        asm volatile("s_waitcnt lgkmcnt(0)\n\ts_barrier" ::: "memory");
+        const bool more_b = kt + 1 < nk;
+        const unsigned ca = fa0 + (unsigned)(st * BD_A), cb = fb0 + (unsigned)(st * BD_B);
+        h_bf16x8 fb[4][2], fa[2][2];
+        fa[0][0] = ig_lds_read<0>(ca);
+        fa[0][1] = ig_lds_read<0>(ca ^ 64u);
+        ig_lds_read4(fb, cb);
+#pragma unroll
+        for (int a = 0; a < NA; ++a) {
+            const int cur = a & 1;
+            if (a == 0) ig_lds_wait_n<6>(fa[0], fb[0]);
+            else ig_lds_wait_n<0>(fa[cur]);
+            __builtin_amdgcn_sched_barrier(0);
+            acc4[a][0] = HT::mfma16(fa[cur][0], fb[0][0], acc4[a][0]);
+            acc4[a][0] = HT::mfma16(fa[cur][1], fb[0][1], acc4[a][0]);
+            __builtin_amdgcn_sched_barrier(0);
+            if (a + 1 < NA) ig_lds_read_a(fa[cur ^ 1], ca, a + 1);
+            if (a == 0) ig_lds_wait_n<6>(fb[1]);
+            __builtin_amdgcn_sched_barrier(0);
+            acc4[a][1] = HT::mfma16(fa[cur][0], fb[1][0], acc4[a][1]);
+            acc4[a][1] = HT::mfma16(fa[cur][1], fb[1][1], acc4[a][1]);
+            __builtin_amdgcn_sched_barrier(0);
+            if ((a & 1) == 0) dma_b(kt + 1, st ^ 1, a >> 1, more_b);
+            if (a == 0) ig_lds_wait_n<4>(fb[2]);
+            __builtin_amdgcn_sched_barrier(0);
+            acc4[a][2] = HT::mfma16(fa[cur][0], fb[2][0], acc4[a][2]);
+            acc4[a][2] = HT::mfma16(fa[cur][1], fb[2][1], acc4[a][2]);
+            if (a == 0) ig_lds_wait_n<2>(fb[3]);
+            __builtin_amdgcn_sched_barrier(0);
+            acc4[a][3] = HT::mfma16(fa[cur][0], fb[3][0], acc4[a][3]);
+            acc4[a][3] = HT::mfma16(fa[cur][1], fb[3][1], acc4[a][3]);
+            __builtin_amdgcn_sched_barrier(0);
+        }
+    }
+
+    asm volatile("s_waitcnt vmcnt(0)" ::: "memory");
+    __syncthreads();
+    float* sW = reinterpret_cast<float*>(smem) + wave * (32 * EP);
+#pragma unroll
+    for (int a = 0; a < RD; ++a) load_res(a);
+    float st1[8], st2[8];
+#pragma unroll
+    for (int q = 0; q < 8; ++q) { st1[q] = 0.f; st2[q] = 0.f; }
+    float bmean[8], binv[8], bgsc[8], bgsh[8];
+    {
+        const float4 m0_ = *reinterpret_cast<const float4*>(mean + nc), m1_ = *reinterpret_cast<const float4*>(mean + nc + 4);
+        const float4 i0_ = *reinterpret_cast<const float4*>(var + nc), i1_ = *reinterpret_cast<const float4*>(var + nc + 4);
+        const float* gp = gamma ? gamma : mean;
+        const float* bp = beta ? beta : mean;
+        const float4 g0_ = *reinterpret_cast<const float4*>(gp + nc), g1_ = *reinterpret_cast<const float4*>(gp + nc + 4);
+        const float4 b0_ = *reinterpret_cast<const float4*>(bp + nc), b1_ = *reinterpret_cast<const float4*>(bp + nc + 4);
+        const float mm[8] = {m0_.x, m0_.y, m0_.z, m0_.w, m1_.x, m1_.y, m1_.z, m1_.w};
+        const float ii[8] = {i0_.x, i0_.y, i0_.z, i0_.w, i1_.x, i1_.y, i1_.z, i1_.w};
+        const float gg[8] = {g0_.x, g0_.y, g0_.z, g0_.w, g1_.x, g1_.y, g1_.z, g1_.w};
+        const float bb[8] = {b0_.x, b0_.y, b0_.z, b0_.w, b1_.x, b1_.y, b1_.z, b1_.w};
+#pragma unroll
+        for (int q = 0; q < 8; ++q) {
+            bmean[q] = mm[q]; binv[q] = ii[q];
+            bgsc[q] = (gamma ? gg[q] : 1.0f) * ii[q];
+            bgsh[q] = fmaf(-mm[q], bgsc[q], beta ? bb[q] : 0.0f);
+        }
+    }
+#pragma unroll
+    for (int a = 0; a < TM; ++a) {
+        if (a + RD < TM) load_res(a + RD);
+        uint4 (&rh)[4] = rhA[a];
+#pragma unroll
+        for (int ta2 = 0; ta2 < 2; ++ta2)
+#pragma unroll
+            for (int b = 0; b < 4; ++b)
+#pragma unroll
+                for (int r = 0; r < 4; ++r)
+                    sW[(ta2 * 16 + 4 * (lane >> 4) + r) * EP + b * 16 + (lane & 15)] = fmaf(acc4[2 * a + ta2][b][r], 1.0f, 0.0f);
+        __builtin_amdgcn_fence(__ATOMIC_RELEASE, "wavefront");
+        __builtin_amdgcn_wave_barrier();
+        __builtin_amdgcn_fence(__ATOMIC_ACQUIRE, "wavefront");
+#pragma unroll
+        for (int ps = 0; ps < 4; ++ps) {
+            const int rl = ps * 8 + erow;
+            const int m = m0 + wm * (TM * 32) + a * 32 + rl;
+            float o[8];
+            const float4 o0 = *reinterpret_cast<const float4*>(sW + rl * EP + ec8 * 8);
+            const float4 o1 = *reinterpret_cast<const float4*>(sW + rl * EP + ec8 * 8 + 4);
+            o[0] = o0.x; o[1] = o0.y; o[2] = o0.z; o[3] = o0.w; o[4] = o1.x; o[5] = o1.y; o[6] = o1.z; o[7] = o1.w;
+            if (m < M) {
+                unsigned ph[4];
+#pragma unroll
+                for (int q = 0; q < 4; ++q) {
+                    const unsigned short h0 = HT::enc(o[2 * q]), h1 = HT::enc(o[2 * q + 1]);
+                    ph[q] = (unsigned)h0 | ((unsigned)h1 << 16);
+                    const unsigned xw = q == 0 ? rh[ps].x : (q == 1 ? rh[ps].y : (q == 2 ? rh[ps].z : rh[ps].w));
+                    const float x0 = HT::lo(xw), x1 = HT::hi(xw);
+                    const float v0 = HT::dec(h0), v1 = HT::dec(h1);
+                    const float g0 = fmaf(x0, bgsc[2 * q], bgsh[2 * q]) > 0.f ? v0 : 0.f;
+                    const float g1 = fmaf(x1, bgsc[2 * q + 1], bgsh[2 * q + 1]) > 0.f ? v1 : 0.f;
+                    st1[2 * q] += g0; st2[2 * q] = fmaf(g0, (x0 - bmean[2 * q]) * binv[2 * q], st2[2 * q]);
+                    st1[2 * q + 1] += g1;
+                    st2[2 * q + 1] = fmaf(g1, (x1 - bmean[2 * q + 1]) * binv[2 * q + 1], st2[2 * q + 1]);
+                }
+                h_store16(Y + (size_t)m * N + nc, ph[0], ph[1], ph[2], ph[3], true);
+            }
+        }
+        __builtin_amdgcn_fence(__ATOMIC_RELEASE, "wavefront");
+        __builtin_amdgcn_wave_barrier();
+        __builtin_amdgcn_fence(__ATOMIC_ACQUIRE, "wavefront");
+    }
+#pragma unroll
+    for (int q = 0; q < 8; ++q) {
+#pragma unroll
+        for (int o = 8; o < 64; o <<= 1) {
+            st1[q] += __shfl_xor(st1[q], o, 64);
+            st2[q] += __shfl_xor(st2[q], o, 64);
+        }
+    }
+    __syncthreads();
+    float* sS = reinterpret_cast<float*>(smem);
+    if (erow == 0) {
+#pragma unroll
+        for (int q = 0; q < 8; ++q) {
+            sS[(wave * 64 + ec8 * 8 + q) * 2] = st1[q];
+            sS[(wave * 64 + ec8 * 8 + q) * 2 + 1] = st2[q];
+        }
+    }
+    __syncthreads();
+    for (int e = tid; e < N * 2; e += NWV * 64) {
+        const int c = e >> 1, which = e & 1;
+        const int wnc = c >> 6, cl = c & 63;
+        float t = 0.f;
+#pragma unroll
+        for (int w = 0; w < WM; ++w) t += sS[((w * WN + wnc) * 64 + cl) * 2 + which];
+        stats[((size_t)bm * N + c) * 2 + which] = t;
+    }
+}
+
+}
+
+extern "C" int hiast_bn_bwd_dgrad_rows(int64_t M, int K, int N)
+{
+    if (M <= 0 || N != 256 || K < 64 || K > hiast::BD_KMAX || K % 64 != 0) return 0;
+    if (M > (1ll << 31) - 512 || (uint64_t)M * K * 2 >= (1ull << 31)) return 0;
+    ConvLaunch c;
+    c.M = M; c.K = K; c.N = N; c.taps = 1;
+    c.stats_mode = 2;
+    const ConvRoute r = ig_route(c);
+    if ((r.family != ConvFamily::TILE && r.family != ConvFamily::TILE_F16) || r.BM != 256 || r.BN != 256) return 0;
+    return r.rows;
+}
+
+extern "C" int hiast_bn_bwd_dgrad(const void* g, const void* gate_mask, const void* bn_x, const float* gamma,
+                                  const float* save_mean, const float* save_invstd, const double* sums, double count,
+                                  const void* wpt, const void* bn2_x, const float* bn2_gamma, const float* bn2_beta,
+                                  const float* bn2_mean, const float* bn2_invstd, void* dx, void* da, float* partial, int64_t M,
+                                  int K, int N, int fmt, hiast_stream_t stream)
+{
+    if (fmt != HIAST_FMT_BF16 && fmt != HIAST_FMT_FP16) return HIAST_E_RANGE;
+    if (!g || !gate_mask || !bn_x || !save_mean || !save_invstd || !sums || !wpt || !bn2_x || !bn2_mean || !bn2_invstd || !dx ||
+        !da || !partial)
+        return HIAST_E_ARG;
+    if (M <= 0 || K <= 0 || N <= 0 || count <= 0) return HIAST_E_ARG;
+    const int rows = hiast_bn_bwd_dgrad_rows(M, K, N);
+    if (rows <= 0) return HIAST_E_RANGE;
+    if ((((uintptr_t)g) | ((uintptr_t)bn_x) | ((uintptr_t)wpt) | ((uintptr_t)bn2_x) | ((uintptr_t)dx) | ((uintptr_t)da) |
+         ((uintptr_t)sums) | ((uintptr_t)bn2_mean) | ((uintptr_t)bn2_invstd) | ((uintptr_t)bn2_gamma) | ((uintptr_t)bn2_beta)) & 15)
+        return HIAST_E_RANGE;
+#define L(F)                                                                                                             \
+    hipLaunchKernelGGL((hiast::bn_bwd_dgrad_kernel<F>), dim3((unsigned)rows), dim3(512), 0, (hipStream_t)stream,        \
+                       (const unsigned short*)g, (const unsigned char*)gate_mask, (const unsigned short*)bn_x, gamma,    \
+                       save_mean, save_invstd, sums, 1.0 / count, (const unsigned short*)wpt, (const unsigned short*)bn2_x, \
+                       bn2_gamma, bn2_beta, bn2_mean, bn2_invstd, (unsigned short*)dx, (unsigned short*)da, partial, (int)M, K)
+    if (fmt == HIAST_FMT_FP16) L(true); else L(false);
+#undef L
+    HIAST_CHECK_LAUNCH();
+    return 0;
+}
diff --git a/hiast_amd/csrc/bn_nhwc.hip b/hiast_amd/csrc/bn_nhwc.hip
--- a/hiast_amd/csrc/bn_nhwc.hip
+++ b/hiast_amd/csrc/bn_nhwc.hip
@@ -184,7 +184,8 @@
 }
 
 __global__ __launch_bounds__(256) void bnh_finalize_kernel(const float* __restrict__ partial, int nblk, int C,
-                                                           double* __restrict__ sums)
+                                                           double* __restrict__ sums, float* __restrict__ dgamma = nullptr,
+                                                           float* __restrict__ dbeta = nullptr)
 {
     __shared__ double s[16][17];
     const int e = threadIdx.x & 15, j = threadIdx.x >> 4;
@@ -208,6 +209,7 @@
 #pragma unroll
         for (int q = 0; q < 16; ++q) t += s[q][e];
         sums[i] = t;
+        if (dbeta) ((i & 1) ? dgamma : dbeta)[i >> 1] = (float)t;
     }
 }
 
@@ -387,10 +389,8 @@
                 if (dbeta) dbeta[cg * 8 + k] = (float)ss.x;
                 if (dgamma) dgamma[cg * 8 + k] = (float)ss.y;
             }
-            k0[k] = gm[k] * invstd[k];
+            bn_bwd_consts(gm[k], invstd[k], ss.x, ss.y, inv_count, k0[k], mg[k], mgx[k]);
             gsh[k] = GATE == 2 ? fmaf(-mean[k], k0[k], bt[k]) : 0.f;
-            mg[k] = (float)(ss.x * inv_count);
-            mgx[k] = (float)(ss.y * inv_count);
         }
     }
     while (r0 < lim) {
@@ -410,7 +410,7 @@
                                                 : (GATE == 3 ? ((bits >> k) & 1u) != 0u : fmaf(xx[k], k0[k], gsh[k]) > 0.f));
                 const float gg = open ? g[k] : 0.f;
                 g[k] = gg;
-                xx[k] = k0[k] * (gg - mg[k] - (xx[k] - mean[k]) * invstd[k] * mgx[k]);
+                xx[k] = bn_bwd_dx(gg, xx[k], mean[k], invstd[k], k0[k], mg[k], mgx[k]);
             }
             bnh_store8<F16>(dx + off, xx, nt_out);
             if (DRES) bnh_store8<F16>(dres + off, g, nt_out);
@@ -481,6 +481,18 @@
     return 0;
 }
 
+extern "C" int hiast_bn_nhwc_stats_from_partial_dparam(const float* partial, int nblk, int C, double* sums, float* dgamma,
+                                                       float* dbeta, hiast_stream_t stream)
+{
+    if (!partial || !sums || !dgamma || !dbeta) return HIAST_E_ARG;
+    if (nblk <= 0) return HIAST_E_ARG;
+    if (!bnh_c_ok(C)) return HIAST_E_RANGE;
+    hipLaunchKernelGGL(hiast::bnh_finalize_kernel, dim3(C * 2 / 16), dim3(256), 0, (hipStream_t)stream, partial, nblk, C,
+                       sums, dgamma, dbeta);
+    HIAST_CHECK_LAUNCH();
+    return 0;
+}
+
 extern "C" int hiast_bn_nhwc_apply(const void* x, const void* res, void* y, const float* gamma, const float* beta,
                                    float* running_mean, float* running_var, const double* sums, double count,
                                    float momentum, float eps, int relu, float* save_mean, float* save_invstd,
@@ -542,10 +554,9 @@
     return 0;
 }
 
-extern "C" int hiast_bn_nhwc_bwd_stats(const void* dy, const void* y, const void* x, const float* gamma,
-                                       const float* beta, const float* save_mean, const float* save_invstd, int relu,
-                                       int64_t M, int C, double* sums, void* workspace, size_t workspace_bytes, int fmt,
-                                       hiast_stream_t stream)
+static int bnh_bwd_stats(const void* dy, const void* y, const void* x, const float* gamma, const float* beta,
+                         const float* save_mean, const float* save_invstd, int relu, int64_t M, int C, double* sums,
+                         void* workspace, size_t workspace_bytes, int fmt, hiast_stream_t stream, float* dgamma, float* dbeta)
 {
     BNH_FMT_CHECK();
     int e = bnh_check(x, M, C);
@@ -565,9 +576,28 @@
 #undef L1
     HIAST_CHECK_LAUNCH();
     hipLaunchKernelGGL(hiast::bnh_finalize_kernel, dim3(C * 2 / 16), dim3(256), 0, st, (const float*)workspace, nblk, C,
-                       sums);
-    HIAST_CHECK_LAUNCH();
-    return 0;
+                       sums, dgamma, dbeta);
+    HIAST_CHECK_LAUNCH();
+    return 0;
+}
+
+extern "C" int hiast_bn_nhwc_bwd_stats(const void* dy, const void* y, const void* x, const float* gamma,
+                                       const float* beta, const float* save_mean, const float* save_invstd, int relu,
+                                       int64_t M, int C, double* sums, void* workspace, size_t workspace_bytes, int fmt,
+                                       hiast_stream_t stream)
+{
+    return bnh_bwd_stats(dy, y, x, gamma, beta, save_mean, save_invstd, relu, M, C, sums, workspace, workspace_bytes, fmt, stream,
+                         nullptr, nullptr);
+}
+
+extern "C" int hiast_bn_nhwc_bwd_stats_dparam(const void* dy, const void* y, const void* x, const float* gamma,
+                                              const float* beta, const float* save_mean, const float* save_invstd, int relu,
+                                              int64_t M, int C, double* sums, void* workspace, size_t workspace_bytes, int fmt,
+                                              float* dgamma, float* dbeta, hiast_stream_t stream)
+{
+    if (!dgamma || !dbeta) return HIAST_E_ARG;
+    return bnh_bwd_stats(dy, y, x, gamma, beta, save_mean, save_invstd, relu, M, C, sums, workspace, workspace_bytes, fmt, stream,
+                         dgamma, dbeta);
 }
 
 extern "C" int hiast_bn_nhwc_bwd_apply(const void* dy, const void* y, const void* x, const float* gamma,
diff --git a/hiast_amd/csrc/common.h b/hiast_amd/csrc/common.h
--- a/hiast_amd/csrc/common.h
+++ b/hiast_amd/csrc/common.h
@@ -150,6 +150,18 @@
         return __builtin_amdgcn_mfma_f32_32x32x16_f16(__builtin_bit_cast(h_f16x8, a), __builtin_bit_cast(h_f16x8, b), c, 0, 0, 0);
     }
 };
+
+__device__ __forceinline__ void bn_bwd_consts(float gamma, float invstd, double sum_g, double sum_gx, double inv_count,
+                                              float& k0, float& mg, float& mgx)
+{
+    k0 = gamma * invstd;
+    mg = (float)(sum_g * inv_count);
+    mgx = (float)(sum_gx * inv_count);
+}
+__device__ __forceinline__ float bn_bwd_dx(float gg, float x, float mean, float invstd, float k0, float mg, float mgx)
+{
+    return k0 * (gg - mg - (x - mean) * invstd * mgx);
+}
 
 __device__ __forceinline__ float a_expf(float x)
 {
diff --git a/hiast_amd/functional.py b/hiast_amd/functional.py
--- a/hiast_amd/functional.py
+++ b/hiast_amd/functional.py
@@ -223,6 +223,7 @@
 
 
 _BN3_FUSION = os.environ.get("HIAST_NO_BN3_FUSION", "0") != "1"
+_BN3_DGRAD_FUSION = os.environ.get("HIAST_NO_BN3_DGRAD_FUSION", "0") != "1"
 _OWN_S2_DGRAD = os.environ.get("HIAST_LIB_DGRAD_S2", "0") != "1"
 
 _NO_ASYNC_STAT = os.environ.get("HIAST_NO_ASYNC_STAT", "0") == "1"
@@ -285,7 +286,7 @@
 
     @staticmethod
     def forward(ctx, x, res, gamma, beta, running_mean, running_var, momentum, eps, relu, world, partial, box,
-                stat_box=None):
+                stat_box=None, dgrad3=None):
         count = float(x.shape[0] * x.shape[2] * x.shape[3])
         ctx.gate = 0 if not relu else (3 if res is not None else 2)
         if ctx.gate == 3 and SW.on("HIAST_NO_BN_MASK"):
@@ -305,6 +306,9 @@
         ctx.save_for_backward(x, out[3] if want_mask else (y if ctx.gate == 1 else None), gamma, beta, sm, si)
         ctx.has_res, ctx.world, ctx.count = res is not None, world, count
         ctx.box = box if (box is not None and box.get("armed") and ctx.gate in (1, 3)) else None
+        ctx.dgrad3 = None
+        if dgrad3 is not None and dgrad3.get("conv") and ctx.gate == 3 and ctx.box is not None and world == 1:
+            ctx.dgrad3 = dgrad3
         ctx.stat_box = None
         if stat_box is not None:
             left = stat_box.pop("bwd_sums", None)
@@ -329,7 +333,15 @@
         dy = dy.contiguous(memory_format=torch.channels_last)
         fused = ctx.stat_box.pop("bwd_partial", None) if ctx.stat_box is not None else None
         early = ctx.stat_box.pop("bwd_sums", None) if ctx.stat_box is not None else None
-        if early is not None:
+        fuse3 = (ctx.dgrad3 is not None and ctx.needs_input_grad[0]
+                 and K.bn_bwd_dgrad_ok(x.shape[0] * x.shape[2] * x.shape[3], x.shape[1], ctx.dgrad3["conv"]))
+        dg3 = db3 = None
+        if fuse3:
+            if fused is not None:
+                sums, dg3, db3 = K.bn_nhwc_stats_from_partial(fused, want_dparam=True)
+            else:
+                sums, dg3, db3 = K.bn_nhwc_bwd_stats(dy, y, x, gamma, beta, sm, si, ctx.gate, want_dparam=True)
+        elif early is not None:
             sums, work = early
             _stat_wait(work)
         else:
@@ -341,19 +353,26 @@
                 _stat_all_reduce(sums)
         want_p = gamma is not None and (ctx.needs_input_grad[2] or ctx.needs_input_grad[3])
         handoff = ctx.box is not None and ctx.needs_input_grad[1]
+        if fuse3:
+            if handoff:
+                ctx.box["gated"] = (dy, y)
+            ctx.dgrad3["stash"] = (dy, y, x, gamma, sm, si, sums, ctx.count)
+            return (_wgrad_token(x), None, dg3 if ctx.needs_input_grad[2] else None, db3 if ctx.needs_input_grad[3] else None,
+                    None, None, None, None, None, None, None, None, None, None)
         dx, dres, dg, db = K.bn_nhwc_bwd_apply(dy, y, x, gamma, beta, sm, si, sums, ctx.count, ctx.gate,
                                                ctx.has_res and ctx.needs_input_grad[1] and not handoff, want_p)
         if handoff:
             ctx.box["gated"] = (dy, y)
         return (dx, dres, dg if ctx.needs_input_grad[2] else None, db if ctx.needs_input_grad[3] else None,
-                None, None, None, None, None, None, None, None, None)
+                None, None, None, None, None, None, None, None, None, None)
 
 
 class _ConvNhwcFn(torch.autograd.Function):
 
     @staticmethod
     @torch.amp.custom_fwd(device_type="cuda")
-    def forward(ctx, x, weight, stride, dil, want_stats, box, packed, in_bn=None, wgroup=None, xsum=None, in_bn3=None):
+    def forward(ctx, x, weight, stride, dil, want_stats, box, packed, in_bn=None, wgroup=None, xsum=None, in_bn3=None,
+                dgrad3=None):
         xv = x.permute(0, 2, 3, 1)
         ctx.in_bn3 = None
         if (in_bn3 is not None and "bn3" in in_bn3 and box is not None and stride == 1 and weight.shape[2] == 1
@@ -369,6 +388,11 @@
                 ctx.xsum = None
         ctx.in_bn = in_bn if (in_bn is not None and "bn" in in_bn and stride == 1 and ctx.needs_input_grad[0]
                               and not SW.on("HIAST_NO_BN_BWD_FUSION")) else None
+        ctx.dgrad3 = None
+        if (dgrad3 is not None and _BN3_DGRAD_FUSION and ctx.in_bn is not None and weight.shape[2] == 1
+                and K.bn_bwd_dgrad_ok(x.shape[0] * x.shape[2] * x.shape[3], weight.shape[0], weight.shape[1])):
+            dgrad3["conv"] = int(weight.shape[1])
+            ctx.dgrad3 = dgrad3
         ctx.set_materialize_grads(False)
         ctx.wpt = None
         ctx.box = None
@@ -394,9 +418,17 @@
     @torch.amp.custom_bwd(device_type="cuda")
     def backward(ctx, dy, _dpartial=None):
         if dy is None:
-            return None, None, None, None, None, None, None, None, None, None, None
+            return None, None, None, None, None, None, None, None, None, None, None, None
         x, weight = ctx.saved_tensors
         stride, dil = ctx.geo
+        stash3 = ctx.dgrad3.pop("stash", None) if ctx.dgrad3 is not None else None
+        if stash3 is not None:
+            g3, mask3, x3, gamma3, sm3, si3, sums3, count3 = stash3
+            bx, sm, si, gamma, beta = ctx.in_bn["bn"]
+            wpt = ctx.wpt if ctx.wpt is not None else K.pack_conv_weight(weight, K.fmt_of(x), transpose=True)
+            dxv, bpartial, dy3 = K.igemm_dgrad_bn_stats(g3.permute(0, 2, 3, 1), wpt, dil, bx.permute(0, 2, 3, 1), gamma, beta, sm, si,
+                                                        bn3=(mask3, x3.permute(0, 2, 3, 1), gamma3, sm3, si3, sums3, count3))
+            dy = dy3.permute(0, 3, 1, 2)
         if dy.dtype != x.dtype:
             dy = dy.to(x.dtype)
         dy = dy.contiguous(memory_format=torch.channels_last)
@@ -413,9 +445,10 @@
             wpt = ctx.wpt if ctx.wpt is not None else K.pack_conv_weight(weight, K.fmt_of(x), transpose=True)
             gated = ctx.box.pop("gated", None) if ctx.box is not None else None
             if ctx.in_bn is not None and gated is None:
-                bx, sm, si, gamma, beta = ctx.in_bn["bn"]
-                dxv, bpartial = K.igemm_dgrad_bn_stats(dy.permute(0, 2, 3, 1), wpt, dil, bx.permute(0, 2, 3, 1), gamma, beta,
-                                                       sm, si)
+                if stash3 is None:
+                    bx, sm, si, gamma, beta = ctx.in_bn["bn"]
+                    dxv, bpartial = K.igemm_dgrad_bn_stats(dy.permute(0, 2, 3, 1), wpt, dil, bx.permute(0, 2, 3, 1), gamma, beta,
+                                                           sm, si)
                 if ctx.in_bn.get("world", 1) != 1 and not _NO_ASYNC_STAT:
                     bsums = K.bn_nhwc_stats_from_partial(bpartial)
                     ctx.in_bn["bwd_sums"] = (bsums, _stat_all_reduce(bsums, async_op=True))
@@ -453,7 +486,7 @@
         if need_w and own_w and ctx.wgroup is not None:
             grp, slot = ctx.wgroup
             grp["jobs"][slot] = (dy.permute(0, 2, 3, 1), x.permute(0, 2, 3, 1), k, stride, dil)
-            return dx, _wgrad_token(weight), None, None, None, None, None, None, None, None, None
+            return dx, _wgrad_token(weight), None, None, None, None, None, None, None, None, None, None
         side = wgrad_side_stream(x.device) if (need_w and not lib_x) else None
         main = torch.cuda.current_stream()
         if side is not None:
@@ -481,7 +514,7 @@
                         dw = dw.view(-1).view(weight.shape)
         if side is not None and dw is not None:
             dw.record_stream(main)
-        return dx, dw, None, None, None, None, None, None, None, None, None
+        return dx, dw, None, None, None, None, None, None, None, None, None, None
 
 
 _wgrad_tokens = {}
@@ -800,7 +833,7 @@
         return g, None
 
 
-def conv_nhwc(x, conv, want_stats=False, box=None, in_bn=None, wgroup=None, xsum=None, in_bn3=None):
+def conv_nhwc(x, conv, want_stats=False, box=None, in_bn=None, wgroup=None, xsum=None, in_bn3=None, dgrad3=None):
     w = conv.weight
     wv = w if wgroup is None else wgroup[2]
     fmt = K.fmt_of(x)
@@ -813,13 +846,13 @@
         x = _SubsampleClFn.apply(x, stride)
         stride = 1
     return _ConvNhwcFn.apply(x, wv, stride, conv.dilation[0], bool(want_stats), box, packed, in_bn,
-                             None if wgroup is None else (wgroup[0], wgroup[1]), xsum, in_bn3)
+                             None if wgroup is None else (wgroup[0], wgroup[1]), xsum, in_bn3, dgrad3)
 
 
 _nbt_batched = [False]
 
 
-def bn_act(x, bn, res=None, relu=True, partial=None, box=None, stat_box=None):
+def bn_act(x, bn, res=None, relu=True, partial=None, box=None, stat_box=None, dgrad3=None):
     training = bn.training or (bn.running_mean is None)
     if training and bn.track_running_stats and bn.num_batches_tracked is not None and not _nbt_batched[0]:
         bn.num_batches_tracked.add_(1)
@@ -827,6 +860,6 @@
     if (training and x.dtype in H16 and _is_cl(x) and not x.is_contiguous()
             and K.bn_nhwc_supported(x.shape[1]) and (res is None or (res.dtype == x.dtype and _is_cl(res)))):
         return _BnActNhwcFn.apply(x, res, bn.weight, bn.bias, bn.running_mean, bn.running_var, momentum, bn.eps, relu,
-                                  _sync_world(bn), partial, box, stat_box)
+                                  _sync_world(bn), partial, box, stat_box, dgrad3)
     return _BnActFn.apply(x, res, bn.weight, bn.bias, bn.running_mean, bn.running_var, training, momentum,
                           bn.eps, relu, _sync_world(bn) if training else 1)
diff --git a/hiast_amd/kernels.py b/hiast_amd/kernels.py
--- a/hiast_amd/kernels.py
+++ b/hiast_amd/kernels.py
@@ -1217,7 +1217,11 @@
     return (y, partial) if want_stats else y
 
 
-def igemm_dgrad_bn_stats(dy, wpt, dil, bn_x, gamma, beta, save_mean, save_invstd):
+def bn_bwd_dgrad_ok(M, K, N):
+    return _lib.load().hiast_bn_bwd_dgrad_rows(int(M), int(K), int(N)) > 0
+
+
+def igemm_dgrad_bn_stats(dy, wpt, dil, bn_x, gamma, beta, save_mean, save_invstd, bn3=None):
     _req16(dy, 4, "dy")
     _req(wpt, dy.dtype, 3, "wpt")
     _req(bn_x, dy.dtype, 4, "bn_x")
@@ -1228,6 +1232,26 @@
     _req(save_invstd, torch.float32, 1, "save_invstd")
     lib = _lib.load()
     da = torch.empty((B, H, W, N), dtype=dy.dtype, device=dy.device)
+    if bn3 is not None:
+        mask, x3, gamma3, sm3, si3, sums3, count3 = bn3
+        M = B * H * W
+        assert taps == 1
+        _req(x3, dy.dtype, 4, "x3")
+        _req(mask, torch.uint8, 2, "mask")
+        assert tuple(x3.shape) == (B, H, W, Cin) and tuple(mask.shape) == (M, Cin // 8)
+        _req(sm3, torch.float32, 1, "save_mean3")
+        _req(si3, torch.float32, 1, "save_invstd3")
+        assert sums3.dtype == torch.float64 and tuple(sums3.shape) == (Cin, 2) and sums3.is_contiguous()
+        rows = lib.hiast_bn_bwd_dgrad_rows(M, Cin, N)
+        if rows <= 0:
+            raise _lib.HiastLibraryError("hiast_bn_bwd_dgrad: unsupported shape M=%d K=%d N=%d" % (M, Cin, N))
+        partial = torch.empty((rows, N, 2), dtype=torch.float32, device=dy.device)
+        dx = torch.empty((B, H, W, Cin), dtype=dy.dtype, device=dy.device)
+        check(lib.hiast_bn_bwd_dgrad(_ptr(dy), _ptr(mask), _ptr(x3), _ptr(gamma3), _ptr(sm3), _ptr(si3), _ptr(sums3),
+                                     float(count3), _ptr(wpt), _ptr(bn_x), _ptr(gamma), _ptr(beta), _ptr(save_mean),
+                                     _ptr(save_invstd), _ptr(dx), _ptr(da), _ptr(partial), M, Cin, N, fmt_of(dy), _stream()),
+              "hiast_bn_bwd_dgrad")
+        return da, partial, dx
     rows = lib.hiast_igemm_dgrad_bn_stats_rows(B * H * W, Cin, N, taps)
     partial = torch.empty((rows, N, 2), dtype=torch.float32, device=dy.device)
     check(lib.hiast_igemm_dgrad_bn_stats(_ptr(dy), _ptr(wpt), _ptr(da), B, H, W, Cin, N, taps, int(dil), _ptr(bn_x),
@@ -1316,11 +1340,17 @@
     return sums
 
 
-def bn_nhwc_stats_from_partial(partial):
+def bn_nhwc_stats_from_partial(partial, want_dparam=False):
     _req(partial, torch.float32, 3, "partial")
     nblk, C, two = partial.shape
     assert two == 2
     sums = torch.empty((C, 2), dtype=torch.float64, device=partial.device)
+    if want_dparam:
+        dg = torch.empty(C, dtype=torch.float32, device=partial.device)
+        db = torch.empty(C, dtype=torch.float32, device=partial.device)
+        check(_lib.load().hiast_bn_nhwc_stats_from_partial_dparam(_ptr(partial), nblk, C, _ptr(sums), _ptr(dg), _ptr(db),
+                                                                  _stream()), "hiast_bn_nhwc_stats_from_partial_dparam")
+        return sums, dg, db
     check(_lib.load().hiast_bn_nhwc_stats_from_partial(_ptr(partial), nblk, C, _ptr(sums), _stream()),
           "hiast_bn_nhwc_stats_from_partial")
     return sums
@@ -1361,13 +1391,21 @@
     return (y, sm, si, mask) if want_mask else (y, sm, si)
 
 
-def bn_nhwc_bwd_stats(dy, y, x, gamma, beta, save_mean, save_invstd, gate):
+def bn_nhwc_bwd_stats(dy, y, x, gamma, beta, save_mean, save_invstd, gate, want_dparam=False):
     xv, M, C = _bnh_view(x, "x")
     dv, M2, C2 = _bnh_view(dy, "dy")
     assert (M2, C2) == (M, C)
     yv = _bnh_view(y, "y")[0] if gate == 1 else (_req(y, torch.uint8, 2, "mask") if gate == 3 else None)
     sums = torch.empty((C, 2), dtype=torch.float64, device=x.device)
     ws = _bnh_workspace(C, x.device)
+    if want_dparam:
+        dg = torch.empty(C, dtype=torch.float32, device=x.device)
+        db = torch.empty(C, dtype=torch.float32, device=x.device)
+        check(_lib.load().hiast_bn_nhwc_bwd_stats_dparam(_ptr(dv), _ptr(yv), _ptr(xv), _ptr(gamma), _ptr(beta), _ptr(save_mean),
+                                                         _ptr(save_invstd), int(gate), M, C, _ptr(sums), _ptr(ws),
+                                                         ws.numel() * 4, fmt_of(x), _ptr(dg), _ptr(db), _stream()),
+              "hiast_bn_nhwc_bwd_stats_dparam")
+        return sums, dg, db
     check(_lib.load().hiast_bn_nhwc_bwd_stats(_ptr(dv), _ptr(yv), _ptr(xv), _ptr(gamma), _ptr(beta), _ptr(save_mean),
                                               _ptr(save_invstd), int(gate), M, C, _ptr(sums), _ptr(ws), ws.numel() * 4,
                                               fmt_of(x), _stream()), "hiast_bn_nhwc_bwd_stats")
diff --git a/hiast_amd/sseg/models/modules/resnet.py b/hiast_amd/sseg/models/modules/resnet.py
--- a/hiast_amd/sseg/models/modules/resnet.py
+++ b/hiast_amd/sseg/models/modules/resnet.py
@@ -23,10 +23,11 @@
 
 
 def conv_bn_act(cv, bn, x, res=None, relu=True, conv_box=None, bn_box=None, in_bn=None, stat_box=None, wgroup=None, xsum=None,
-                in_bn3=None):
+                in_bn3=None, dgrad3=None):
     if x.is_cuda and x.dtype in HF.H16 and bn.training and HF.conv_nhwc_ok(x, cv):
-        y, partial = HF.conv_nhwc(x, cv, want_stats=True, box=conv_box, in_bn=in_bn, wgroup=wgroup, xsum=xsum, in_bn3=in_bn3)
-        return HF.bn_act(y, bn, res, relu, partial=partial, box=bn_box, stat_box=stat_box)
+        y, partial = HF.conv_nhwc(x, cv, want_stats=True, box=conv_box, in_bn=in_bn, wgroup=wgroup, xsum=xsum, in_bn3=in_bn3,
+                                  dgrad3=dgrad3)
+        return HF.bn_act(y, bn, res, relu, partial=partial, box=bn_box, stat_box=stat_box, dgrad3=dgrad3)
     return bn_act(bn, conv(cv, x), res, relu)
 
 
@@ -82,7 +83,8 @@
                         xsum=None if xs is None else (xs, "give"), in_bn3=getattr(x, "_hiast_bn3", None) if box is not None else None)
         o = conv_bn_act(self.conv2, self.bn2, o, in_bn=sb1, stat_box=sb2, wgroup=g(1))
         sb3 = {}
-        y = conv_bn_act(self.conv3, self.bn3, o, res=idt, bn_box=box, in_bn=sb2, stat_box=sb3, wgroup=g(2))
+        y = conv_bn_act(self.conv3, self.bn3, o, res=idt, bn_box=box, in_bn=sb2, stat_box=sb3, wgroup=g(2),
+                        dgrad3={} if box is not None else None)
         if "bn3" in sb3:
             y._hiast_bn3 = sb3
         return y
diff --git a/include/hiast_hip.h b/include/hiast_hip.h
--- a/include/hiast_hip.h
+++ b/include/hiast_hip.h
@@ -137,6 +137,12 @@
                                const float* save_invstd, float* partial, int partial_rows ,
                                int fmt , hiast_stream_t stream);
 int hiast_igemm_dgrad_bn_stats_rows(int64_t M, int Cin, int Cout, int taps);
+int hiast_bn_bwd_dgrad_rows(int64_t M, int K, int N);
+int hiast_bn_bwd_dgrad(const void* g, const void* gate_mask, const void* bn_x, const float* gamma, const float* save_mean,
+                       const float* save_invstd, const double* sums, double count, const void* wpt, const void* bn2_x,
+                       const float* bn2_gamma, const float* bn2_beta, const float* bn2_mean, const float* bn2_invstd, void* dx,
+                       void* da, float* partial, int64_t M, int K, int N, int fmt ,
+                       hiast_stream_t stream);
 int hiast_igemm_dgrad_s2(const void* dy, const void* wpt, void* dx, int B, int H, int W, int Cin, int Cout, int fmt,
                          hiast_stream_t stream);
 int hiast_xconv_dgrad_gated_bn_stats_rows(int64_t M, int K, int N);
@@ -180,6 +186,12 @@
 int hiast_bn_nhwc_stats(const void* x, int64_t M, int C, double* sums, void* workspace, size_t workspace_bytes, int fmt,
                         hiast_stream_t stream);
 int hiast_bn_nhwc_stats_from_partial(const float* partial, int nblk, int C, double* sums, hiast_stream_t stream);
+int hiast_bn_nhwc_bwd_stats_dparam(const void* dy, const void* y, const void* x, const float* gamma, const float* beta,
+                                   const float* save_mean, const float* save_invstd, int relu, int64_t M, int C, double* sums,
+                                   void* workspace, size_t workspace_bytes, int fmt, float* dgamma, float* dbeta,
+                                   hiast_stream_t stream);
+int hiast_bn_nhwc_stats_from_partial_dparam(const float* partial, int nblk, int C, double* sums, float* dgamma, float* dbeta,
+                                            hiast_stream_t stream);
 int hiast_bn_nhwc_apply_partial(const void* x, const void* res, void* y, const float* gamma, const float* beta,
                                 float* running_mean, float* running_var, const float* partial, int nblk, double count,
                                 float momentum, float eps, int relu, float* save_mean, float* save_invstd, int64_t M,
```

Result: no change. 143.4 (median of 6 runs) (+1.1%).
